# lambdaclass/AES_zero_knowledge_proof_circuit

Hardware: AMD Instinct MI355X
Metric: AES-ECB blocks proven/sec (Marlin), proof verifies (higher is better)
Workload: dtype u32 limbs (253-bit Fr / 377-bit Fq modular integers)

## Files before the change

aes_zero_knowledge_proof_circuit_amd/csrc/capi_kernels.hip:

```cpp
#include "../../include/zkaes.h"
#include <cstring>
#include <string>
#include <vector>
#include "hip_util.hpp"
#include "marlin.hpp"
#include "te28.cuh"
#include <algorithm>
#include <chrono>

typedef unsigned int v4u __attribute__((ext_vector_type(4)));
__global__ void __launch_bounds__(256) k_stream_copy(uint4 *__restrict__ dst_, const uint4 *__restrict__ src_, size_t n16) {
    v4u *dst = (v4u *)dst_; const v4u *src = (const v4u *)src_;
    size_t base = (size_t)blockIdx.x * 1024 + threadIdx.x;
    if (base + 768 < n16) {
        v4u v0 = __builtin_nontemporal_load(src + base), v1 = __builtin_nontemporal_load(src + base + 256);
        v4u v2 = __builtin_nontemporal_load(src + base + 512), v3 = __builtin_nontemporal_load(src + base + 768);
        __builtin_nontemporal_store(v0, dst + base); __builtin_nontemporal_store(v1, dst + base + 256);
        __builtin_nontemporal_store(v2, dst + base + 512); __builtin_nontemporal_store(v3, dst + base + 768);
    } else {
        for (size_t i = base; i < n16; i += 256) dst[i] = src[i];
    }
}


// ... 307 lines not shown
        DevPtr<PF> dv = upload(v, n, s);
        {
            zk::gpu::ThroughputWaits as_between_overlapping_proofs(throughput_variant != 0);
            zk::gpu::batch_inverse(dv, n, post_or_null ? &post : nullptr, s);
            zk::gpu::sync(s);
        }
        zk::gpu::d2h(v, dv, n * sizeof(PF), s);
    });
}
int zkaes_poly_lincomb(const uint8_t *const *polys, const size_t *lens, const uint8_t *scalars, int count, size_t n, uint8_t *out) {
    return guardk([&] {
        const char *who = "zkaes_poly_lincomb";
        need(count >= 1 && count <= 8, who, "1..8 terms"); need(polys && lens && scalars && (out || !n), who, "null argument"); need(n <= POLY_MAX, who, "polynomial too long");
        for (int i = 0; i < count; i++) { need(lens[i] <= n, who, "a term longer than the result"); need(!lens[i] || polys[i], who, "null polynomial"); }
        if (!n) return;
        zk::gpu::require_device();
        StreamGuard s;
        DevPtr<PF> dp[8], dout(n);
        const PF *ptr[8];
        PF sc[8];
        for (int i = 0; i < count; i++) { dp[i] = upload(polys[i], lens[i], s); ptr[i] = dp[i]; sc[i] = load_f(scalars + 32 * i, who); }
        zk::gpu::poly_lincomb_n(dout, n, ptr, lens, sc, count, s);
        zk::gpu::d2h(out, dout, n * sizeof(PF), s);
    });
}
int zkaes_vanishing_quotient_evals(int lg_n, const uint8_t *g, int ncosets, const uint8_t a[32], const uint32_t *idx_or_null, size_t nidx, uint8_t *out) {
    return guardk([&] {
        const char *who = "zkaes_vanishing_quotient_evals";
        need(lg_n >= 0 && lg_n <= 24, who, "lg_n must be in [0, 24]"); need(ncosets >= 1 && ncosets <= 3, who, "1..3 cosets"); need(g && out, who, "null argument");
        const size_t n = (size_t)1 << lg_n;
        for (size_t i = 0; idx_or_null && i < nidx; i++) need(idx_or_null[i] < n, who, "index out of range");
        const PF af = load_f(a, who);
        PF gs[3];
        for (int c = 0; c < ncosets; c++) gs[c] = load_f(g + 32 * c, who);
        zk::gpu::require_device();
        StreamGuard s;
        const PF *elems = zk::gpu::domain_elements<zk::Fr377>(lg_n);
        const size_t scratch_len = zk::gpu::vanishing_quotient_scratch(lg_n, ncosets);
        DevPtr<PF> tabs[3], scratch(scratch_len);
        PF *outs[3] = {nullptr, nullptr, nullptr};
        for (int c = 0; c < ncosets; c++) { tabs[c].alloc(n); outs[c] = tabs[c]; }
        zk::gpu::vanishing_quotient_evals(outs, gs, ncosets, af, elems, (uint32_t)n, lg_n, scratch, scratch_len, s);
        if (!idx_or_null) { for (int c = 0; c < ncosets; c++) zk::gpu::d2h(out + (size_t)c * n * sizeof(PF), tabs[c], n * sizeof(PF), s); return; }
        std::vector<PF> host(n);
        for (int c = 0; c < ncosets; c++) {
            zk::gpu::d2h(host.data(), tabs[c], n * sizeof(PF), s);
            for (size_t i = 0; i < nidx; i++) memcpy(out + ((size_t)c * nidx + i) * sizeof(PF), &host[idx_or_null[i]], sizeof(PF));
        }
    });
}
int zkaes_q1_coset_pointwise(const uint8_t *r, const uint8_t *za, const uint8_t *zb, const uint8_t *t, const uint8_t *z, const uint8_t consts[192], size_t n, uint8_t *out) {
    return guardk([&] {
        const char *who = "zkaes_q1_coset_pointwise";
        need(r && za && zb && t && z && consts && out, who, "null argument"); need(n >= 1 && n <= POLY_MAX, who, "n out of range");
        PF c[6];
        for (int i = 0; i < 6; i++) c[i] = load_f(consts + 32 * i, who);
        zk::gpu::require_device();
        StreamGuard s;
        DevPtr<PF> dr = upload(r, n, s), dza = upload(za, n, s), dzb = upload(zb, n, s), dt = upload(t, n, s), dz = upload(z, n, s), dout(n);
        zk::gpu::q1_coset_pointwise(dout, dr, dza, dzb, dt, dz, c[0], c[1], c[2], c[3], c[4], c[5], n, s);
        zk::gpu::d2h(out, dout, n * sizeof(PF), s);
    });
}
int zkaes_h2_coset(const uint8_t *const arrays[7], const uint8_t consts[224], size_t k, uint8_t *out) {
    return guardk([&] {
        const char *who = "zkaes_h2_coset";
        need(arrays && consts && out, who, "null argument"); need(k >= 1 && k <= POLY_MAX, who, "k out of range");
        for (int i = 0; i < 7; i++) need(arrays[i], who, "null array");
        PF c[7];
        for (int i = 0; i < 7; i++) c[i] = load_f(consts + 32 * i, who);
        zk::gpu::require_device();
        StreamGuard s;
        DevPtr<PF> d[7], dout(k);
        for (int i = 0; i < 7; i++) d[i] = upload(arrays[i], k, s);
        zk::gpu::h2_coset(dout, d[0], d[1], d[2], d[3], d[4], d[5], d[6], c[0], c[1], c[2], c[3], c[4], c[5], c[6], k, s);
        zk::gpu::d2h(out, dout, k * sizeof(PF), s);
    });
}
int zkaes_q1_combine(const uint8_t *q0, const uint8_t *q1, const uint8_t *q3, const uint8_t *mask, const uint8_t inv2[32], const uint8_t inv2zeta[32], size_t n, uint8_t *h1, uint8_t *g1) {
    return guardk([&] {
        const char *who = "zkaes_q1_combine";
        need(q0 && q1 && q3 && mask && h1 && (g1 || n < 2), who, "null argument"); need(n >= 1 && n <= POLY_MAX / 4, who, "n out of range");
        const PF i2 = load_f(inv2, who), i2z = load_f(inv2zeta, who);
        zk::gpu::require_device();
        StreamGuard s;
        DevPtr<PF> d0 = upload(q0, n, s), d1 = upload(q1, n, s), d3 = upload(q3, n, s), dm = upload(mask, 3 * n, s), dh(2 * n), dg(n);
        zk::gpu::q1_combine(dh, dg, d0, d1, d3, dm, i2, i2z, n, s);
        zk::gpu::d2h(h1, dh, 2 * n * sizeof(PF), s);
        zk::gpu::d2h(g1, dg, (n - 1) * sizeof(PF), s);
    });
}
int zkaes_coset_scale(const uint8_t *in, size_t in_len, const uint8_t g[32], size_t n, uint8_t *out) {
    return guardk([&] {
        const char *who = "zkaes_coset_scale";
        need((in || !in_len) && (out || !n), who, "null argument"); need(n <= POLY_MAX && in_len <= POLY_MAX, who, "polynomial too long");
        const PF gf = load_f(g, who);
        if (!n) return;
        zk::gpu::require_device();
        StreamGuard s;
        DevPtr<PF> din = upload(in, in_len, s), dout(n);
        zk::gpu::coset_scale(dout, din, gf, in_len, n, s);
        zk::gpu::d2h(out, dout, n * sizeof(PF), s);
    });
}
int zkaes_z_poly_from_w(const uint8_t *w, size_t wlen, const uint8_t *x_poly, uint32_t m, size_t n, uint8_t *zp) {
    return guardk([&] {
        const char *who = "zkaes_z_poly_from_w";
        need((w || !wlen) && (x_poly || !m) && zp, who, "null argument"); need(n < POLY_MAX && wlen <= POLY_MAX, who, "polynomial too long");
        zk::gpu::require_device();
        StreamGuard s;
        DevPtr<PF> dw = upload(w, wlen, s), dx = upload(x_poly, m, s), dz(n + 1);
        zk::gpu::z_poly_from_w(dz, dw, wlen, dx, m, n, s);
        zk::gpu::d2h(zp, dz, (n + 1) * sizeof(PF), s);
    });
}
int zkaes_ntt_padded(int field_id, const uint8_t *in, size_t in_len, size_t n, int inverse, int coset_c, int lg_big, uint8_t *out) {
    return guardk([&] {
        if (field_id == 381) run_ntt_padded<zk::Fr381>(in, in_len, n, inverse, coset_c, lg_big, out); else if (field_id == 377) run_ntt_padded<zk::Fr377>(in, in_len, n, inverse, coset_c, lg_big, out);
        else throw std::invalid_argument("field_id must be 377 or 381");
    });
}
int zkaes_ntt_scaled(const uint8_t g[32], const uint8_t *in, size_t in_len, size_t n, int inverse, uint8_t *out) {
    return guardk([&] {
        const char *who = "zkaes_ntt_scaled";
        const int lg = exact_log2(n, who);
        need(lg >= 1 && lg <= 28, who, "n must be in [2, 2^28]"); need(in_len <= n, who, "in_len must not exceed n"); need(out && (in || !in_len), who, "null argument");
        const PF gf = load_f(g, who);
        need(!gf.is_zero(), who, "the coset generator must not be zero");
        zk::gpu::require_device();
        StreamGuard s;
        DevPtr<void> table = zk::gpu::coset_power_table<PF>(inverse ? gf.inverse() : gf, n, s);
        DevPtr<PF> a = upload(in, in_len, s), b(n);
        zk::gpu::ntt_scaled<PF>(b, a, in_len, lg, inverse != 0, table, s);
        zk::gpu::d2h(out, b, n * sizeof(PF), s);
    });
}
int zkaes_msm(int curve_id, const uint8_t *bases, const uint8_t *scalars, size_t n, uint8_t *out_xy, int *out_inf) {
    return guardk([&] { if (curve_id == 381) run_msm<zk::Bls381>(bases, scalars, n, out_xy, out_inf, 0, nullptr, nullptr); else if (curve_id == 377) run_msm<zk::Bls377>(bases, scalars, n, out_xy, out_inf, 0, nullptr, nullptr); else throw std::invalid_argument("curve_id must be 377 or 381"); });
}
int zkaes_msm_bench(int curve_id, const uint8_t *bases, const uint8_t *scalars, size_t n, int reps, double *ms_total, double *ms_accumulate) {
    return guardk([&] { if (curve_id == 381) run_msm<zk::Bls381>(bases, scalars, n, nullptr, nullptr, reps, ms_total, ms_accumulate); else run_msm<zk::Bls377>(bases, scalars, n, nullptr, nullptr, reps, ms_total, ms_accumulate); });
}
int zkaes_msm_bench_synth(size_t n, int window_bits, int reps, double *ms_total, double *ms_accumulate, uint8_t *out_xy) {
    return guardk([&] {
        using Fq = zk::Fq377; using Fr = zk::Fr377;
        if (!ms_total || !ms_accumulate || reps < 1 || n == 0 || window_bits > 22) throw std::invalid_argument("zkaes_msm_bench_synth: bad arguments");
        zk::gpu::require_device();
        const size_t nt = window_bits > 0 ? (size_t)zk::gpu::table_windows<zk::Bls377>(window_bits) : 1;
        if ((uint64_t)nt * n >= (1ull << 30)) throw std::invalid_argument("zkaes_msm_bench_synth: n x table copies exceeds the 2^30 base indices of one MSM");
        StreamGuard s;
        DevPtr<zk::Affine<Fq>> tab(nt * n);
        zk::Affine<Fq> g; for (int i = 0; i < 12; i++) { g.x.l[i] = G1_377_X_MONT[i]; g.y.l[i] = G1_377_Y_MONT[i]; }
        Fr beta = Fr::from_u64(0x9e3779b97f4a7c15ull) * Fr::from_u64(0xc2b2ae3d27d4eb4full);
        zk::gpu::fixed_base_powers<zk::Bls377>(tab, g, beta, 1, n, s);
        if (window_bits > 0) zk::gpu::build_window_tables<zk::Bls377>(tab, n, window_bits, s);
        const bool edwards = window_bits != 0;
        DevPtr<zk::Affine28<zk::Fq377P>> tab28;
        DevPtr<zk::Niels28<zk::Fq377P>> tabte;
        if (edwards) { tabte.alloc(nt * n); zk::gpu::convert_bases_te<zk::Bls377>(tabte, tab, nt * n, s); }
        else { tab28.alloc(nt * n); zk::gpu::convert_bases<zk::Bls377>(tab28, tab, nt * n, s); }
        std::vector<Fr> sc(n);
        uint64_t x = 88172645463325252ull;
        for (size_t i = 0; i < n; i++) { for (int k = 0; k < 8; k += 2) { x ^= x << 13; x ^= x >> 7; x ^= x << 17; sc[i].l[k] = (uint32_t)x; sc[i].l[k + 1] = (uint32_t)(x >> 32); } sc[i].l[7] &= 0x0fffffffu; }
        DevPtr<Fr> ds(n);
        zk::gpu::h2d(ds, sc.data(), n * 32, s);
        zk::gpu::sync(s);
        WorkspaceGuard ws;
        auto run = [&]() -> zk::XYZZ<Fq> {
            if (edwards) return window_bits > 0 ? zk::gpu::msm_table<zk::Bls377>(ws, tabte, n, 0, window_bits, ds, n, s) : zk::gpu::msm<zk::Bls377>(ws, tabte.get(), ds.get(), n, s);
            return window_bits > 0 ? zk::gpu::msm_table<zk::Bls377>(ws, tab28, n, 0, window_bits, ds, n, s) : zk::gpu::msm<zk::Bls377>(ws, tab28.get(), ds.get(), n, s);
        };
        give_affine(run().to_affine(), out_xy, nullptr);
        zk::gpu::MsmStats before = zk::gpu::msm_stats(false);
        EventGuard e0, e1;
        zk::gpu::event_record(e0, s);
        for (int i = 0; i < reps; i++) run();
        zk::gpu::event_record(e1, s);
        float ms = zk::gpu::event_elapsed_ms(e0, e1);
        zk::gpu::MsmStats after = zk::gpu::msm_stats(false);
        *ms_total = ms / reps; *ms_accumulate = (after.accumulate_ms - before.accumulate_ms) / reps;
    });
}

int zkaes_stream_copy_bench(size_t bytes, int reps, double *gb_per_s) {
    return guardk([&] {
        if (bytes < 4096 || reps < 1 || !gb_per_s) throw std::invalid_argument("zkaes_stream_copy_bench: bytes >= 4096, reps >= 1");
        zk::gpu::require_device();
        StreamGuard s;
        const size_t n16 = bytes / 16;
        DevPtr<uint4> a(n16), b(n16);
        zk::gpu::dzero(a, n16 * 16, s);
        hipStream_t hs = (hipStream_t)s.h;
        k_stream_copy<<<(unsigned)((n16 + 1023) / 1024), 256, 0, hs>>>(b, a, n16);
        EventGuard e0, e1;
        zk::gpu::event_record(e0, s);
        for (int i = 0; i < reps; i++) k_stream_copy<<<(unsigned)((n16 + 1023) / 1024), 256, 0, hs>>>(i & 1 ? a.get() : b.get(), i & 1 ? b.get() : a.get(), n16);
        zk::gpu::event_record(e1, s);
        float ms = zk::gpu::event_elapsed_ms(e0, e1);
        *gb_per_s = 2.0 * (double)(n16 * 16) * reps / 1e9 / (ms / 1e3);
    });
}
int zkaes_int_rate_bench(double seconds, double out[8]) {
    return guardk([&] {
        if (!out || !(seconds > 0.0) || seconds > 30.0) throw std::invalid_argument("zkaes_int_rate_bench: 0 < seconds <= 30, out != NULL");
        zk::gpu::require_device();
        using P = zk::Fq377P; using G = zk::FpMsm<P>;
        StreamGuard s;
        hipStream_t hs = (hipStream_t)s.h;
        const int GRID_A = 4096, ITERS_A = 300, GRID_B = 8192, ITERS_B = 83;
        const uint32_t NREC = 4096;
        DevPtr<CalStamp> st(GRID_B);
        DevPtr<G> sink_a((size_t)GRID_A * 64);
        DevPtr<zk::AccTE<P>> sink_b((size_t)GRID_B * 64);
        DevPtr<zk::Niels28<P>> tab(NREC);
        k_cal_fill<<<NREC / 256, 256, 0, hs>>>(tab, NREC);
        G ga; for (int k = 0; k < 14; k++) ga.l[k] = 0x0123457u + 977u * k;
        std::vector<double> rate_a, mhz_a, rate_b, mhz_b, cyc_b;
        std::vector<CalStamp> h(GRID_B);
        auto median = [](std::vector<double> &v) { std::sort(v.begin(), v.end()); return v.empty() ? 0.0 : v[v.size() / 2]; };
        auto stamps = [&](int grid, double per_wave_units, double *mhz, double *cyc_per_unit) {
            zk::gpu::d2h(h.data(), st, (size_t)grid * sizeof(CalStamp), s);
            std::vector<double> m(grid), c(grid);
            for (int i = 0; i < grid; i++) { m[i] = (double)h[i].cyc / ((double)h[i].rt / 1e8) / 1e6; c[i] = (double)h[i].cyc / per_wave_units; }
            *mhz = median(m); *cyc_per_unit = median(c);
        };
        EventGuard e0, e1;
        const auto t_begin = std::chrono::steady_clock::now();
        int rounds = 0;
        while (rounds < 3 || std::chrono::duration<double>(std::chrono::steady_clock::now() - t_begin).count() < seconds) {
            double mhz, cyc;
            zk::gpu::event_record(e0, s);
            k_cal_fqmul<<<GRID_A, 64, 0, hs>>>(st, sink_a, ga, ITERS_A);
            zk::gpu::event_record(e1, s);
            stamps(GRID_A, 2.0 * ITERS_A, &mhz, &cyc);
            rate_a.push_back(2.0 * ITERS_A * 64.0 * GRID_A / (zk::gpu::event_elapsed_ms(e0, e1) * 1e-3)); mhz_a.push_back(mhz);
            zk::gpu::event_record(e0, s);
            k_cal_hot_loop<<<GRID_B, 64, 0, hs>>>(st, sink_b, tab, NREC - 1, ITERS_B);
            zk::gpu::event_record(e1, s);
            stamps(GRID_B, (double)ITERS_B, &mhz, &cyc);
            rate_b.push_back((double)ITERS_B * 64.0 * GRID_B / (zk::gpu::event_elapsed_ms(e0, e1) * 1e-3)); mhz_b.push_back(mhz); cyc_b.push_back(cyc);
            rounds++;
        }
        out[0] = median(rate_a); out[1] = median(mhz_a); out[2] = median(rate_b); out[3] = median(mhz_b); out[4] = median(cyc_b); out[5] = (double)rounds; out[6] = 0; out[7] = 0;
    });
}
int zkaes_mem_info(uint64_t *free_bytes, uint64_t *total_bytes) {
    return guardk([&] {
        zk::gpu::require_device();
        size_t f = 0, t = 0;
        HIP_CHECK(hipMemGetInfo(&f, &t));
        if (free_bytes) *free_bytes = f;
        if (total_bytes) *total_bytes = t;
    });
}
}
```

aes_zero_knowledge_proof_circuit_amd/csrc/gpu.hpp:

```cpp
#pragma once
#include <cstddef>
#include <cstdint>
#include <stdexcept>
#include <string>
#include <utility>
#include <vector>
#include "ec.cuh"
#include "te28.cuh"

namespace zk {
namespace gpu {

struct GpuError : std::runtime_error { using std::runtime_error::runtime_error; };
typedef void *stream_t;

int device_count();
void require_device();
int current_device();
void set_device(int ordinal);
void *dmalloc(size_t bytes);
#ifdef ZKAES_MEASURE
int knockin();
#endif
size_t mem_free_bytes();
void dfree(void *p);
void h2d(void *dst, const void *src, size_t bytes, stream_t s);
void d2h(void *dst, const void *src, size_t bytes, stream_t s);
void d2d(void *dst, const void *src, size_t bytes, stream_t s);
void dzero(void *dst, size_t bytes, stream_t s);
void sync(stream_t s);
bool throughput_mode();
struct ThroughputWaits { explicit ThroughputWaits(bool on); ~ThroughputWaits(); ThroughputWaits(const ThroughputWaits &) = delete; ThroughputWaits &operator=(const ThroughputWaits &) = delete; private: bool on_; };
stream_t stream_create();
stream_t stream_create_background();
void stream_destroy(stream_t s);
void *event_create();
void event_record(void *ev, stream_t s);
void stream_wait_event(stream_t s, void *ev);
float event_elapsed_ms(void *start, void *stop);
void event_destroy(void *ev);

void *pinned_alloc(size_t bytes);
void *pinned_device_address(void *host);
void pinned_free(void *host);

template <class T> struct DevElem { static constexpr size_t bytes = sizeof(T); };
template <> struct DevElem<void> { static constexpr size_t bytes = 1; };
template <class T> struct DevPtr {
    T *p = nullptr;
    size_t n = 0;
    DevPtr() = default;
    explicit DevPtr(size_t count) { alloc(count); }
    DevPtr(const DevPtr &) = delete; DevPtr &operator=(const DevPtr &) = delete;
    DevPtr(DevPtr &&o) noexcept : p(o.p), n(o.n) { o.p = nullptr; o.n = 0; }
    DevPtr &operator=(DevPtr &&o) noexcept { if (this != &o) { reset(); p = o.p; n = o.n; o.p = nullptr; o.n = 0; } return *this; }
    ~DevPtr() { dfree(p); }
    void reset() { dfree(p); p = nullptr; n = 0; }
    void alloc(size_t count) { reset(); p = (T *)dmalloc(count * DevElem<T>::bytes); n = count; }
    void grow(size_t count) { if (!p || count > n) alloc(count); }
    T *get() const { return p; }
    operator T *() const { return p; }
};
template <class... T> void grow_together(const size_t (&counts)[sizeof...(T)], DevPtr<T> &...bufs) {
    size_t i = 0;
    if (((bufs.p && counts[i++] <= bufs.n) && ...)) return;
    (bufs.reset(), ...);
    i = 0;
    try { (bufs.alloc(counts[i++]), ...); } catch (...) { (bufs.reset(), ...); throw; }
}
template <class H, H (*Create)(), void (*Destroy)(H)> struct Handle {
    H h = nullptr;
    Handle() : h(Create()) {}
    explicit Handle(H adopt) : h(adopt) {}
    Handle(const Handle &) = delete; Handle &operator=(const Handle &) = delete;
    Handle(Handle &&o) noexcept : h(o.h) { o.h = nullptr; }
    Handle &operator=(Handle &&o) noexcept { if (this != &o) { Destroy(h); h = o.h; o.h = nullptr; } return *this; }
    ~Handle() { Destroy(h); }
    operator H() const { return h; }
};
using StreamGuard = Handle<stream_t, stream_create, stream_destroy>;
using EventGuard = Handle<void *, event_create, event_destroy>;
struct PinnedPtr {
    void *host = nullptr, *dev = nullptr;
    PinnedPtr() = default;
    PinnedPtr(const PinnedPtr &) = delete; PinnedPtr &operator=(const PinnedPtr &) = delete;
    ~PinnedPtr() { pinned_free(host); }
    void alloc(size_t bytes) { pinned_free(host); host = dev = nullptr; host = pinned_alloc(bytes); dev = pinned_device_address(host); }
};

enum : int { OP_MSM_BUCKETS = 0, OP_MSM_SECOND_BASES = 1, OP_MSM_CLASS_SUM = 2 };
struct OpRecord { std::vector<std::pair<uint64_t, int>> ntt , msm ; };
void oplog_begin();
OpRecord oplog_end();
void oplog_ntt(uint64_t n, int count);
void oplog_msm(uint64_t points, int kind);

template <class Fr> void ntt(Fr *dst, const Fr *src, size_t in_len, int lg, bool inverse, stream_t s);
template <class Fr> void ntt_coset(Fr *dst, const Fr *src, size_t in_len, int lg, bool inverse, int coset_c, int lg_big, stream_t s);
template <class Fr> struct NttJob { Fr *dst; const Fr *src; int coset_c; };
template <class Fr> void ntt_batch(const NttJob<Fr> *jobs, int count, size_t in_len, int lg, bool inverse, int lg_big, stream_t s);
template <class Fr> DevPtr<void> coset_power_table(const Fr &g, size_t n, stream_t s);
template <class Fr> void ntt_scaled(Fr *dst, const Fr *src, size_t in_len, int lg, bool inverse, const void *table, stream_t s);
template <class Fr> const Fr *domain_elements(int lg);

struct MsmWorkspace;
MsmWorkspace *msm_workspace_create();
void msm_workspace_destroy(MsmWorkspace *ws);
using WorkspaceGuard = Handle<MsmWorkspace *, msm_workspace_create, msm_workspace_destroy>;
template <class Curve> void convert_bases(Affine28<typename Curve::FqP> *dst, const Affine<typename Curve::Fq> *src, size_t n, stream_t s);
template <class Curve>
XYZZ<typename Curve::Fq> msm(MsmWorkspace *ws, const Affine28<typename Curve::FqP> *bases, const typename Curve::Fr *scalars, size_t n, stream_t s);
template <class Curve>
void msm_prepare(MsmWorkspace *ws, const typename Curve::Fr *scal1, size_t n1, const typename Curve::Fr *scal2, size_t n2, size_t val_off2, stream_t s, int force_c = 0);
template <class Curve>
XYZZ<typename Curve::Fq> msm_finish(MsmWorkspace *ws, const Affine28<typename Curve::FqP> *bases, stream_t s);
template <class Curve> void convert_bases_te(Niels28<typename Curve::FqP> *dst, const Affine<typename Curve::Fq> *src, size_t n, stream_t s);
template <class Curve>
XYZZ<typename Curve::Fq> msm(MsmWorkspace *ws, const Niels28<typename Curve::FqP> *bases, const typename Curve::Fr *scalars, size_t n, stream_t s);
template <class Curve>
XYZZ<typename Curve::Fq> msm_finish(MsmWorkspace *ws, const Niels28<typename Curve::FqP> *bases, stream_t s);
template <class Curve>
void msm_finish2(MsmWorkspace *ws, const Niels28<typename Curve::FqP> *bases, const Niels28<typename Curve::FqP> *bases2, XYZZ<typename Curve::Fq> *out, stream_t s);
template <class Curve>
XYZZ<typename Curve::Fq> msm_table(MsmWorkspace *ws, const Niels28<typename Curve::FqP> *tables, size_t stride, size_t off, int c, const typename Curve::Fr *scalars, size_t n, stream_t s);
template <class Curve>
bool class_sum(MsmWorkspace *ws, const Niels28<typename Curve::FqP> *bases, const int8_t *vals, size_t n, XYZZ<typename Curve::Fq> *out, stream_t s);
template <class Curve> void msm_sharded_plan(size_t n_total, int *window_bits, int *n_windows);
template <class Curve>
void msm_window_sums_device(MsmWorkspace *ws, const Affine28<typename Curve::FqP> *bases, const typename Curve::Fr *scalars, size_t n_local, size_t n_total,
                            XYZZ<typename Curve::Fq> *dev_out, stream_t s);
template <class Curve>
XYZZ<typename Curve::Fq> msm_fold_window_sums_device(const XYZZ<typename Curve::Fq> *dev_in, int world, size_t n_total, stream_t s);
template <class Curve>
void msm_table_sum_device(MsmWorkspace *ws, const Niels28<typename Curve::FqP> *tables, size_t stride, size_t off, int c, const typename Curve::Fr *scalars, size_t n,
                          XYZZ<typename Curve::Fq> *dev_out, stream_t s);
template <class Curve>
XYZZ<typename Curve::Fq> msm_fold_points_device(const XYZZ<typename Curve::Fq> *dev_in, int world, stream_t s);
template <class Curve> int table_windows(int c);
template <class Curve> void build_window_tables(Affine<typename Curve::Fq> *tables, size_t stride, int c, stream_t s);
template <class Curve> void table_next(Affine<typename Curve::Fq> *next, const Affine<typename Curve::Fq> *prev, size_t count, int c, int j, stream_t s);
template <class Curve>
void msm_prepare_table(MsmWorkspace *ws, const typename Curve::Fr *scal1, size_t n1, size_t off1, const typename Curve::Fr *scal2, size_t n2, size_t off2, int c, size_t stride, stream_t s);
template <class Curve>
XYZZ<typename Curve::Fq> msm_table(MsmWorkspace *ws, const Affine28<typename Curve::FqP> *tables, size_t stride, size_t off, int c, const typename Curve::Fr *scalars, size_t n, stream_t s);
template <class Curve>
void fixed_base_powers(Affine<typename Curve::Fq> *out, const Affine<typename Curve::Fq> &base, const typename Curve::Fr &beta, size_t from, size_t count, stream_t s);
template <class Curve>
void fixed_base_scalars(Affine<typename Curve::Fq> *out, const Affine<typename Curve::Fq> &base, const typename Curve::Fr *scalars, size_t count, stream_t s);
template <class Curve>
bool class_sum(MsmWorkspace *ws, const Affine28<typename Curve::FqP> *bases, const int8_t *vals, size_t n, XYZZ<typename Curve::Fq> *out, stream_t s);
struct MsmStats { double accumulate_ms = 0; double total_ms = 0; uint64_t points = 0; uint64_t launches = 0; uint64_t pairs = 0; };
MsmStats msm_stats(bool reset);

}
}

namespace zk {
namespace gpu {
using F = Fr377;

void poly_set_at(F *p, size_t idx, const F &val, stream_t s);
void poly_add_at(F *p, size_t idx, const F &val, stream_t s);
void poly_scale(F *p, const F &sc, size_t n, stream_t s);
void poly_lincomb_n(F *out, size_t n, const F *const *polys, const size_t *lens, const F *scalars, int count, stream_t s);
size_t divide_by_vanishing_scratch(size_t len, size_t m);
void divide_by_vanishing(F *q, F *rem, const F *p, size_t len, size_t m, stream_t s, F *scratch = nullptr, size_t scratch_len = 0);
void divide_by_linear(F *q, const F *p, size_t len, const F &z, F *scratch, size_t scratch_elems, stream_t s);
size_t divide_by_linear_scratch(size_t len);
F poly_eval(const F *p, size_t len, const F &x, F *scratch, stream_t s);
size_t poly_eval_scratch(size_t len);
void poly_eval_multi(const F *const *p, const size_t *len, const F *x, int count, F *out, F *scratch, size_t scratch_elems, stream_t s);
void batch_inverse(F *v, size_t n, const F *post_or_null, stream_t s);
size_t vanishing_quotient_scratch(int lg_n, int ncosets);
void vanishing_quotient_evals(F *const *out, const F *g, int ncosets, const F &a, const F *elems, uint32_t n, int lg_n, F *scratch, size_t scratch_elems, stream_t s);
void f_evals_from_tables(F *out, const F *va, const F *vb, const F *vc, const F &ea, const F &eb, const F &ec, const F *ra, const F *rb, const uint32_t *ri, const uint32_t *ci, size_t k,
                         stream_t s);

void upload_sbox(const uint8_t table[256]);
void aes_trace(uint8_t *trace, size_t trace_stride, const uint8_t *msgs, const uint8_t *keys, uint32_t nproofs, uint32_t nblocks, stream_t s);
void aes_trace_cbc(uint8_t *trace, size_t trace_stride, const uint8_t *msgs, const uint8_t *keys, const uint8_t *ivs, uint32_t nproofs, uint32_t nblocks, stream_t s);
void aes_trace_ctr(uint8_t *trace, size_t trace_stride, const uint8_t *msgs, const uint8_t *keys, const uint8_t *icbs, uint32_t nproofs, uint32_t msg_len, stream_t s);
void aes_trace_gcm(uint8_t *trace, size_t trace_stride, const uint8_t *msgs, const uint8_t *keys, const uint8_t *hdrs, uint32_t nproofs, uint32_t msg_len, uint32_t aad_len, stream_t s);
void ghash_trace(uint8_t *trace, size_t trace_stride, uint32_t nproofs, uint32_t msg_len, uint32_t aad_len, stream_t s);
void witness_expand(uint8_t *z, const uint32_t *desc, uint32_t ncols, const uint8_t *trace, const uint32_t *sbox_in_off, const uint32_t *sbox_tmpl, stream_t s);
void spmv_bits(F *out, int8_t *small_out, size_t rows_out, const uint32_t *rowptr, const uint32_t *col, const int64_t *coeff, size_t rows, const uint8_t *z, stream_t s);
void w_classes(int8_t *out, const uint8_t *z, uint32_t n, uint32_t m, uint32_t num_witness, stream_t s);
void lagrange_scalars(F *lag, F *lag_w, const F *elems, const F &beta, uint32_t n, uint32_t m, stream_t s);
void w_evals(F *out, const uint8_t *z, const F *x_evals, uint32_t n, uint32_t m, uint32_t num_witness, stream_t s);
void bits_to_field(F *out, const uint8_t *z, size_t n, stream_t s);
constexpr uint32_t T_SEG = 32, T_HEAVY_SEGMENTS = 256;
void t_evals(F *out, uint32_t n, F *partial, uint32_t nseg, const uint32_t *col_seg_ptr, const uint32_t *seg_start, const uint32_t *seg_end, const uint32_t *heavy, uint32_t n_heavy,
             const uint32_t *row, const uint8_t *mat, const int64_t *coeff, const F *r_alpha, const F &eta_a, const F &eta_b, const F &eta_c, stream_t s);
uint64_t chacha_field_stream(F *out, size_t count, const uint32_t key[8], int rounds, uint64_t word_pos, void *scratch, size_t scratch_bytes, stream_t s);
void mask_fixup(F *p, size_t n, stream_t s);
void q1_coset_pointwise(F *out, const F *r, const F *za, const F *zb, const F *t, const F *z, const F &ca, const F &cb, const F &cz, const F &eta_a, const F &eta_b, const F &eta_c,
                        size_t n, stream_t s);
void z_evals_h(F *out, const uint8_t *z, uint32_t n, uint32_t m, uint32_t num_witness, stream_t s);
void q1_combine(F *h1, F *g1, const F *q0, const F *q1, const F *q3, const F *mask, const F &inv2, const F &inv2zeta, size_t n, stream_t s);
void coset_scale(F *out, const F *in, const F &g, size_t in_len, size_t n, stream_t s);
void h2_coset(F *out, const F *row, const F *col, const F *va, const F *vb, const F *vc, const F *rc, const F *f, const F &alpha, const F &beta, const F &alpha_beta,
              const F &ea, const F &eb, const F &ec, const F &vinv, size_t k, stream_t s);
void index_evals(F *row, F *col, F *rowcol, F *va, F *vb, F *vc, F *tmp, const uint32_t *ci, const uint32_t *ri, const int64_t *ca, const int64_t *cb, const int64_t *cc, size_t cnt,
                 size_t k, const F *elems, uint32_t n, stream_t s);
void z_poly_from_w(F *zp, const F *w, size_t wlen, const F *x_poly, uint32_t m, size_t n, stream_t s);

}
}
```

aes_zero_knowledge_proof_circuit_amd/csrc/kernels_msm.hip:

```cpp
#include <cstring>
#include <rocprim/device/device_radix_sort.hpp>
#include <rocprim/device/device_scan.hpp>
#include <chrono>
#include <cstdio>
#include <cstdlib>
#include <mutex>
#include <vector>
#include "hip_util.hpp"
#include "te28.cuh"

namespace zk {
namespace gpu {

template <class P> struct WeierLaw { using Params = P; using Base = Affine28<P>; using Acc = Acc28<P>; static constexpr bool edwards = false; };
template <class P> struct EdwardsLaw { using Params = P; using Base = Niels28<P>; using Acc = AccTE<P>; static constexpr bool edwards = true; };

static MsmStats g_stats;
static std::mutex g_stats_mu;
MsmStats msm_stats(bool reset) {
    std::lock_guard<std::mutex> g(g_stats_mu);
    MsmStats s = g_stats;
    if (reset) g_stats = MsmStats();
    return s;
}

constexpr uint32_t VAL_SKIP = 1u << 30, VAL_INDEX = VAL_SKIP - 1;
template <class Fr>
__global__ void k_digits(const Fr *__restrict__ scalars, uint32_t n, uint32_t i_off, uint32_t ntot, uint32_t val_off, int c, int nwin, uint32_t nb,
                         uint32_t *__restrict__ keys, uint32_t *__restrict__ vals) {
    uint32_t i = blockIdx.x * blockDim.x + threadIdx.x;
    if (i >= n) return;
    uint32_t raw[Fr::N + 1];
    scalars[i].to_raw(raw);
    raw[Fr::N] = 0;
    const uint32_t mask = (1u << c) - 1, half = 1u << (c - 1);
    uint32_t carry = 0;
    for (int w = 0; w < nwin; w++) {
        int bit = w * c, limb = bit >> 5, sh = bit & 31;
        uint64_t two = limb <= Fr::N - 1 ? ((uint64_t)raw[limb] | ((uint64_t)raw[limb + 1] << 32)) : 0;
        uint32_t v = ((uint32_t)(two >> sh) & mask) + carry;
        uint32_t neg = 0;
        carry = 0;
        if (v > half) { v = (1u << c) - v; neg = 1u << 31; carry = 1; }
        keys[(size_t)w * ntot + i_off + i] = ((uint32_t)w << (c - 1)) | (v ? v - 1 : 0u);
        vals[(size_t)w * ntot + i_off + i] = v ? ((val_off + i) | neg) : VAL_SKIP;
    }
}

struct TableLayout {
    int nwin, c_hi, n_hi;
    __host__ __device__ int width(int j) const { return j < n_hi ? c_hi : c_hi - 1; }
    __host__ __device__ int offset(int j) const { return j < n_hi ? j * c_hi : n_hi * c_hi + (j - n_hi) * (c_hi - 1); }
};
static TableLayout table_layout(int total_bits, int c) {
    TableLayout L;
    L.nwin = (total_bits + c - 1) / c;
    int base = total_bits / L.nwin, rem = total_bits % L.nwin;
    L.c_hi = base + (rem ? 1 : 0);
    L.n_hi = rem ? rem : L.nwin;
    return L;
}
template <class Fr>
__global__ void k_digits_table(const Fr *__restrict__ scalars, uint32_t n, uint32_t i_off, uint32_t ntot, uint32_t val_off, TableLayout L, uint32_t stride,
                               uint32_t *__restrict__ keys, uint32_t *__restrict__ vals) {
    uint32_t i = blockIdx.x * blockDim.x + threadIdx.x;
    if (i >= n) return;
    uint32_t raw[Fr::N + 1];
    scalars[i].to_raw(raw);
    raw[Fr::N] = 0;
    uint32_t carry = 0;
    for (int w = 0; w < L.nwin; w++) {
        const int c = L.width(w), bit = L.offset(w), limb = bit >> 5, sh = bit & 31;
        const uint32_t mask = (1u << c) - 1, half = 1u << (c - 1);
        uint64_t two = limb <= Fr::N - 1 ? ((uint64_t)raw[limb] | ((uint64_t)raw[limb + 1] << 32)) : 0;
        uint32_t v = ((uint32_t)(two >> sh) & mask) + carry;
        uint32_t neg = 0;
        carry = 0;
        if (v > half) { v = (1u << c) - v; neg = 1u << 31; carry = 1; }
        keys[(size_t)w * ntot + i_off + i] = v ? v - 1 : 0u;
        vals[(size_t)w * ntot + i_off + i] = v ? (((uint32_t)w * stride + val_off + i) | neg) : VAL_SKIP;
    }
}
template <class Fq>
__global__ void __launch_bounds__(64) k_table_next(const Affine<Fq> *__restrict__ prev, Affine<Fq> *__restrict__ next, uint32_t count, int c) {
    constexpr int B = 8;
    uint32_t t = blockIdx.x * blockDim.x + threadIdx.x;
    uint32_t s0 = t * B;
    if (s0 >= count) return;
    uint32_t e = s0 + B < count ? s0 + B : count;
    Fq xs[B], ys[B], zz[B], zzz[B], pre[B];
    Fq acc = Fq::one();
    for (uint32_t i = s0; i < e; i++) {
        XYZZ<Fq> p = XYZZ<Fq>::from_affine(prev[i]);
        for (int k = 0; k < c; k++) p = p.dbl();
        xs[i - s0] = p.x; ys[i - s0] = p.y; zz[i - s0] = p.zz; zzz[i - s0] = p.zzz;
        pre[i - s0] = acc;
        if (!p.zzz.is_zero()) acc = acc * p.zzz;
    }
    acc = acc.inverse();
    for (uint32_t i = e; i-- > s0;) {
        uint32_t q = i - s0;
        if (zzz[q].is_zero()) { next[i] = Affine<Fq>::inf(); continue; }
        Fq zi3 = acc * pre[q];
        acc = acc * zzz[q];
        Fq zi2 = (zi3 * zz[q]).sqr();
        Affine<Fq> a; a.x = xs[q] * zi2; a.y = ys[q] * zi3;
        next[i] = a;
    }
}

__device__ __forceinline__ uint32_t bounds_rank(uint32_t key, int cbits, uint32_t nwin) { return nwin == 1 ? key : (key & ((1u << cbits) - 1)) * nwin + (key >> cbits); }
__device__ __forceinline__ uint32_t bounds_key(uint32_t rank, int cbits, uint32_t nwin) { return nwin == 1 ? rank : ((rank % nwin) << cbits) | (rank / nwin); }
__global__ void k_bounds(const uint32_t *__restrict__ keys, size_t total, int cbits, uint32_t nwin, uint32_t *__restrict__ start, uint32_t *__restrict__ end) {
    size_t i0 = ((size_t)blockIdx.x * blockDim.x + threadIdx.x) * 4;
    if (i0 >= total) return;
    const uint32_t nb = nwin << cbits;
    uint32_t k[6];
    if (i0 + 4 <= total) { uint4 v = *reinterpret_cast<const uint4 *>(keys + i0); k[1] = v.x; k[2] = v.y; k[3] = v.z; k[4] = v.w; }
    else { for (int j = 0; j < 4; j++) k[1 + j] = i0 + j < total ? keys[i0 + j] : 0u; }
    k[0] = i0 ? keys[i0 - 1] : 0u;
    k[5] = i0 + 4 < total ? keys[i0 + 4] : 0u;
#pragma unroll
    for (int j = 0; j < 4; j++) {
        size_t i = i0 + j;
        if (i >= total) break;
        const uint32_t key = k[1 + j];
        if (i == 0 || k[j] != key) {
            const uint32_t r1 = bounds_rank(key, cbits, nwin);
            uint32_t r0 = 0;
            if (i != 0) { end[k[j]] = (uint32_t)i; r0 = bounds_rank(k[j], cbits, nwin) + 1; }
            for (uint32_t r = r0; r < r1; r++) { const uint32_t g = bounds_key(r, cbits, nwin); start[g] = (uint32_t)i; end[g] = (uint32_t)i; }
            start[key] = (uint32_t)i;
        }
        if (i + 1 == total) {
            end[key] = (uint32_t)total;
            for (uint32_t r = bounds_rank(key, cbits, nwin) + 1; r < nb; r++) { const uint32_t g = bounds_key(r, cbits, nwin); start[g] = (uint32_t)total; end[g] = (uint32_t)total; }
        }
    }
}

template <class P>
__global__ void k_convert_bases(const Affine<Fp<P>> *__restrict__ src, Affine28<P> *__restrict__ dst, size_t n) {
    size_t i = (size_t)blockIdx.x * blockDim.x + threadIdx.x;
    if (i < n) dst[i] = Affine28<P>::from_std(src[i]);
}

constexpr uint32_t BUCKET_CAP = 2048, BUCKET_CAP_TABLE = 512;
constexpr uint32_t NO_SLOT = 0xffffffffu;

constexpr int ORD_BINS = 1024, ORD_THREADS = 256, ORD_MAX_BLOCKS = 128;
__device__ __forceinline__ uint32_t order_key(uint32_t sz) { return (ORD_BINS - 1) - (sz > ORD_BINS - 1 ? ORD_BINS - 1 : sz); }
__global__ void __launch_bounds__(ORD_THREADS) k_order_hist(const uint32_t *__restrict__ start, const uint32_t *__restrict__ end, uint32_t nb, uint32_t per_block, uint32_t cap,
                                                             uint32_t *__restrict__ ovf_slot, uint32_t *__restrict__ ovf_bucket, uint32_t *__restrict__ ovf_nseg, uint32_t ovf_cap,
                                                             uint32_t *__restrict__ ctrl, uint32_t *__restrict__ hist) {
    __shared__ uint32_t h[ORD_BINS];
    for (int b = threadIdx.x; b < ORD_BINS; b += ORD_THREADS) h[b] = 0;
    __syncthreads();
    const uint32_t lo = blockIdx.x * per_block, hi = lo + per_block < nb ? lo + per_block : nb;
    for (uint32_t k = lo + threadIdx.x; k < hi; k += ORD_THREADS) {
        const uint32_t sz = end[k] - start[k];
        uint32_t slot = NO_SLOT;
        if (sz > cap) {
            slot = atomicAdd(&ctrl[0], 1u);
            if (slot < ovf_cap) { ovf_bucket[slot] = k; ovf_nseg[slot] = (sz - 1) / cap; } else slot = NO_SLOT;
        }
        ovf_slot[k] = slot;
        atomicAdd(&h[order_key(sz)], 1u);
    }
    __syncthreads();
    for (int b = threadIdx.x; b < ORD_BINS; b += ORD_THREADS) hist[(size_t)blockIdx.x * ORD_BINS + b] = h[b];
}
__global__ void __launch_bounds__(ORD_BINS) k_order_scan(const uint32_t *__restrict__ hist, uint32_t *__restrict__ offs, uint32_t nblk, uint32_t *__restrict__ ctrl,
                                                          const uint32_t *__restrict__ ovf_nseg, uint32_t *__restrict__ ovf_off, uint32_t ovf_cap) {
    __shared__ uint32_t part[ORD_BINS];
    const uint32_t t = threadIdx.x;
    auto block_exclusive = [&](uint32_t v) {
        part[t] = v;
        __syncthreads();
        for (int d = 1; d < ORD_BINS; d <<= 1) {
            uint32_t add = t >= (unsigned)d ? part[t - d] : 0;
            __syncthreads();
            part[t] += add;
            __syncthreads();
        }
        return part[t] - v;
    };
    uint32_t sum = 0;
    uint32_t i0 = 0;
    for (; i0 + 8 <= nblk; i0 += 8) {
        uint32_t c[8];
#pragma unroll
        for (int u = 0; u < 8; u++) c[u] = hist[(size_t)(i0 + u) * ORD_BINS + t];
#pragma unroll
        for (int u = 0; u < 8; u++) sum += c[u];
    }
    for (; i0 < nblk; i0++) sum += hist[(size_t)i0 * ORD_BINS + t];
    uint32_t run = block_exclusive(sum);
    for (i0 = 0; i0 + 8 <= nblk; i0 += 8) {
        uint32_t c[8];
#pragma unroll
        for (int u = 0; u < 8; u++) c[u] = hist[(size_t)(i0 + u) * ORD_BINS + t];
#pragma unroll
        for (int u = 0; u < 8; u++) { offs[(size_t)(i0 + u) * ORD_BINS + t] = run; run += c[u]; }
    }
    for (; i0 < nblk; i0++) { const uint32_t c = hist[(size_t)i0 * ORD_BINS + t]; offs[(size_t)i0 * ORD_BINS + t] = run; run += c; }
    uint32_t n = ctrl[0];
    if (n > ovf_cap) n = ovf_cap;
    uint32_t base = 0;
    for (uint32_t c0 = 0; c0 < n; c0 += ORD_BINS) {
        __syncthreads();
        const uint32_t v = c0 + t < n ? ovf_nseg[c0 + t] : 0;
        const uint32_t ex = block_exclusive(v);
        if (c0 + t < n) ovf_off[c0 + t] = base + ex;
        base += part[ORD_BINS - 1];
    }
    __syncthreads();
    if (t == 0) { ovf_off[n] = base; ctrl[1] = n; ctrl[2] = base; ctrl[0] = 0; }
}
__global__ void __launch_bounds__(ORD_THREADS) k_order_scatter(const uint32_t *__restrict__ start, const uint32_t *__restrict__ end, uint32_t nb, uint32_t per_block,
                                                                const uint32_t *__restrict__ offs, uint32_t *__restrict__ order) {
    __shared__ uint32_t h[ORD_BINS];
    for (int b = threadIdx.x; b < ORD_BINS; b += ORD_THREADS) h[b] = 0;
// ... 494 lines not shown
    const int nrep = bases2 ? 2 : 1, nsets = nsets_one * nrep;
    if (bases2 && !Law::edwards) throw GpuError("msm: two base arrays per prepared state need the Edwards law");
    if (nsets > MAX_WSUMS) throw GpuError("msm: too many windows");
    const size_t nb = (size_t)nsets_one << c;
    ensure_result(S, nb * nrep);
    if constexpr (!Law::edwards) HIP_CHECK(hipMemsetAsync(S.deferred_count, 0, 8, s));
#ifdef ZKAES_MEASURE
    if (knockin() & 8) {
        hipLaunchKernelGGL((k_accumulate<Law>), dim3((unsigned)((nb + 63) / 64)), dim3(64), 0, s, bases, S.sorted_vals, S.start, S.end, S.order, (uint32_t)nb, cap,
                           (A *)S.buckets.p, S.deferred, DEFERRED_CAP, S.deferred_count);
        if constexpr (!Law::edwards) HIP_CHECK(hipMemsetAsync(S.deferred_count, 0, 8, s));
    }
#endif
    uint32_t max_seg = (uint32_t)(pairs / cap + 1);
    for (int rep = 0; rep < nrep; rep++) {
        const typename Law::Base *src = rep ? bases2 : bases;
        HIP_CHECK(hipEventRecord((hipEvent_t)S.ev[2 * rep].h, s));
        hipLaunchKernelGGL((k_accumulate<Law>), dim3((unsigned)((nb + 63) / 64)), dim3(64), 0, s, src, S.sorted_vals, S.start, S.end, S.order, (uint32_t)nb, cap,
                           (A *)S.buckets.p + rep * nb, S.deferred, DEFERRED_CAP, S.deferred_count);
        HIP_LAUNCH_CHECK();
        HIP_CHECK(hipEventRecord((hipEvent_t)S.ev[2 * rep + 1].h, s));
        hipLaunchKernelGGL((k_accumulate_tail<Law>), dim3((max_seg + 63) / 64), dim3(64), 0, s, src, S.sorted_vals, S.start, S.end, S.ctrl, S.ovf_bucket, S.ovf_off, max_seg, cap,
                           (A *)S.ovf_partial.p + rep * S.ovf_bucket.n, (A *)S.buckets.p + rep * nb, S.deferred, DEFERRED_CAP, S.deferred_count);
        HIP_LAUNCH_CHECK();
    }
    if constexpr (!Law::edwards) for (int rep = 0; rep < nrep; rep++) {
        hipLaunchKernelGGL((k_fold_overflow<A>), dim3((max_seg + 63) / 64), dim3(64), 0, s, (A *)S.buckets.p + rep * nb, S.ctrl, S.ovf_bucket, S.ovf_off, max_seg, (const A *)S.ovf_partial.p + rep * S.ovf_bucket.n);
        HIP_LAUNCH_CHECK();
    }
    XYZZ<Fq> *res = (XYZZ<Fq> *)S.h_res.dev;
    uint32_t segs = (1u << c) / RED_L1, groups = (segs + RED_L2 - 1) / RED_L2;
    [[maybe_unused]] int te_lgR = 0, te_lgC = 0;
    [[maybe_unused]] bool te_host_tail = false;
#ifdef ZKAES_MEASURE
    for (int rep = (knockin() & 2) ? 0 : 1; rep < 2; rep++)
#endif
    {
    if constexpr (Law::edwards)
        hipLaunchKernelGGL((k_reduce_l1_pair<A>), dim3((unsigned)((2 * segs * nsets + 63) / 64)), dim3(64), 0, s, (const A *)S.buckets.p, c, nsets, (A *)S.seg_s.p, (A *)S.seg_w.p);
    else
        hipLaunchKernelGGL((k_reduce_l1<A>), dim3((unsigned)((segs * nsets + 63) / 64)), dim3(64), 0, s, (const A *)S.buckets.p, c, nsets, (A *)S.seg_s.p, (A *)S.seg_w.p);
    HIP_LAUNCH_CHECK();
    if constexpr (Law::edwards) {
        const int lgG = c - 3 > 0 ? c - 3 : 0, lgC = (lgG + 1) / 2, lgR = lgG - lgC;
        if (lgC > 8) throw GpuError("msm: more than 2^19 buckets per set");
        const unsigned jobs = 2u * (1u << lgR) + (1u << lgC);
        A *rc = (A *)S.partial.p, *part = rc + (size_t)nsets * jobs;
        hipLaunchKernelGGL((k_reduce_rc<P>), dim3((unsigned)nsets * jobs), dim3(RQ_THREADS), 0, s, (const A *)S.seg_s.p, (const A *)S.seg_w.p, lgR, lgC, rc);
        HIP_LAUNCH_CHECK();
        te_host_tail = !dev_wsum_out && nsets <= 4;
        hipLaunchKernelGGL((k_reduce_terms<P>), dim3((unsigned)(RF_OUT * nsets)), dim3(RT_THREADS), 0, s, (const A *)rc, lgR, lgC, part, res, te_host_tail);
        HIP_LAUNCH_CHECK();
        if (!te_host_tail) {
            hipLaunchKernelGGL((k_reduce_combine<P>), dim3((unsigned)nsets), dim3(64), 0, s, (const A *)part, lgR, lgC, res, dev_wsum_out);
            HIP_LAUNCH_CHECK();
        }
        te_lgR = lgR; te_lgC = lgC;
    } else {
    hipLaunchKernelGGL((k_reduce_l2<A>), dim3(2u * (unsigned)((groups * nsets + 63) / 64)), dim3(64), 0, s, (const A *)S.seg_s.p, (const A *)S.seg_w.p, c, nsets, (A *)S.partial.p);
    HIP_LAUNCH_CHECK();
    const uint32_t parts = 2 * groups;
    if (nsets == 1 && parts > 2048) {
        uint32_t mid = (parts + 255) / 256;
        hipLaunchKernelGGL((k_sum_tree<A>), dim3(mid), dim3(256), 0, s, (const A *)S.partial.p, parts, 256u, (A *)S.seg_s.p, 0u, 0u);
        HIP_LAUNCH_CHECK();
        hipLaunchKernelGGL((k_reduce_window<A>), dim3(1), dim3(256), 0, s, (const A *)S.seg_s.p, mid, res, dev_wsum_out);
    } else {
        hipLaunchKernelGGL((k_reduce_window<A>), dim3((unsigned)nsets), dim3(256), 0, s, (const A *)S.partial.p, parts, res, dev_wsum_out);
    }
    HIP_LAUNCH_CHECK();
    }
    }
    std::vector<XYZZ<Fq>> ws(nsets);
    uint32_t n_deferred = 0;
    sync((stream_t)s);
    if (Law::edwards && te_host_tail) {
        std::vector<XYZZ<Fq>> terms((size_t)nsets * RF_OUT);
        memcpy(terms.data(), S.h_res.host, sizeof(XYZZ<Fq>) * terms.size());
        for (int i = 0; i < nsets; i++) ws[i] = reduce_host_tail<Fq>(terms.data() + (size_t)i * RF_OUT, te_lgR, te_lgC);
    } else memcpy(ws.data(), S.h_res.host, sizeof(XYZZ<Fq>) * nsets);
    if constexpr (!Law::edwards) {
        HIP_CHECK(hipMemcpyAsync(&n_deferred, S.deferred_count, 4, hipMemcpyDeviceToHost, s));
        sync((stream_t)s);
        if (n_deferred > DEFERRED_CAP) throw GpuError("msm: more than 2^20 degenerate additions (repeated base points); refusing to return a wrong sum");
    }
    for (int rep = 0; rep < nrep; rep++) HIP_CHECK(hipEventElapsedTime(acc_ms + rep, (hipEvent_t)S.ev[2 * rep].h, (hipEvent_t)S.ev[2 * rep + 1].h));
    (void)n_points;
    return ws;
}
static void add_stats(const float *acc_ms, int launches, size_t n, size_t pairs, std::chrono::steady_clock::time_point t_begin) {
    std::lock_guard<std::mutex> g(g_stats_mu);
    for (int i = 0; i < launches; i++) g_stats.accumulate_ms += acc_ms[i];
    g_stats.points += n * (size_t)launches;
    g_stats.pairs += pairs * (size_t)launches;
    g_stats.launches += (uint64_t)launches;
    g_stats.total_ms += std::chrono::duration<double, std::milli>(std::chrono::steady_clock::now() - t_begin).count();
}

__global__ void __launch_bounds__(64) k_convert_bases_te(const Affine<Fq377> *__restrict__ src, Niels28<Fq377P> *__restrict__ dst, size_t n, uint32_t *__restrict__ bad) {
    constexpr int B = 8;
    size_t s0 = ((size_t)blockIdx.x * blockDim.x + threadIdx.x) * B;
    if (s0 >= n) return;
    size_t e = s0 + B < n ? s0 + B : n;
    TeMapParts m[B];
    Fq377 pre[B];
    bool skip[B];
    Fq377 acc = Fq377::one();
    for (size_t i = s0; i < e; i++) {
        Affine<Fq377> p = src[i];
        int q = (int)(i - s0);
        skip[q] = p.is_inf();
        if (!skip[q]) {
            m[q] = te_map_parts(p);
            if (m[q].den.is_zero()) { skip[q] = true; atomicOr(bad, 1u); }
        }
        pre[q] = acc;
        if (!skip[q]) acc = acc * m[q].den;
    }
    acc = acc.inverse();
    for (size_t i = e; i-- > s0;) {
        int q = (int)(i - s0);
        if (skip[q]) { dst[i] = niels_identity<Fq377P>(); continue; }
        Fq377 inv = acc * pre[q];
        acc = acc * m[q].den;
        dst[i] = te_niels_finish(m[q], inv);
    }
}
template <class Curve>
void convert_bases_te(Niels28<typename Curve::FqP> *dst, const Affine<typename Curve::Fq> *src, size_t n, stream_t s_) {
    static_assert(Curve::ID == 377, "only BLS12-377's G1 has a twisted Edwards model");
    if (!n) return;
    hipStream_t s = (hipStream_t)s_;
    DevPtr<uint32_t> d_bad(1);
    uint32_t h_bad = 0;
    HIP_CHECK(hipMemsetAsync(d_bad, 0, 4, s));
    size_t lanes = (n + 7) / 8;
    hipLaunchKernelGGL(k_convert_bases_te, dim3((unsigned)((lanes + 63) / 64)), dim3(64), 0, s, src, dst, n, d_bad.get());
    HIP_LAUNCH_CHECK();
    sync((stream_t)s);
    HIP_CHECK(hipMemcpyAsync(&h_bad, d_bad, 4, hipMemcpyDeviceToHost, s));
    sync((stream_t)s);
    if (h_bad) throw GpuError("convert_bases_te: a base point has order 2 or 4 -- the Edwards path needs points of the prime-order subgroup");
}
template void convert_bases_te<Bls377>(Niels28<Fq377P> *, const Affine<Fq377> *, size_t, stream_t);

template <class Curve>
void convert_bases(Affine28<typename Curve::FqP> *dst, const Affine<typename Curve::Fq> *src, size_t n, stream_t s_) {
    if (!n) return;
    hipLaunchKernelGGL((k_convert_bases<typename Curve::FqP>), dim3((unsigned)((n + 255) / 256)), dim3(256), 0, (hipStream_t)s_, src, dst, n);
    HIP_LAUNCH_CHECK();
}

template <class Curve>
void msm_prepare(MsmWorkspace *ws_, const typename Curve::Fr *scal1, size_t n1, const typename Curve::Fr *scal2, size_t n2, size_t val_off2, stream_t s_, int force_c) {
    using Fr = typename Curve::Fr;
    hipStream_t s = (hipStream_t)s_;
    if (!ws_) throw GpuError("msm: null workspace");
    MsmWorkspace &S = *ws_;
    size_t n = n1 + n2;
    S.plan_n = n;
    if (n == 0) return;
    if (n >= (1u << 30) || val_off2 + n2 >= (1u << 30)) throw GpuError("msm: too many points");
    int lg = 0;
    while (((size_t)1 << lg) < n) lg++;
    int c = lg - 2;
    if (c < 7) c = 7;
    if (c > 17) c = 17;
    if (force_c >= 4 && force_c <= 22) c = force_c;
    const int nwin = (Fr::BITS + 1 + c - 1) / c;
    size_t pairs = n * (size_t)nwin;
    if (pairs >= ((size_t)1 << 31)) throw GpuError("msm: n x windows exceeds the 2^31 pairs the sort indexes with int");
    const size_t nb = (size_t)nwin << (c - 1);
    S.plan_c = c; S.plan_nwin = nwin; S.plan_pairs = pairs; S.plan_table = false; S.plan_cap = BUCKET_CAP;
    ensure_scratch(S, pairs, nb, BUCKET_CAP);
    if (n1) { hipLaunchKernelGGL((k_digits<Fr>), dim3((unsigned)((n1 + 255) / 256)), dim3(256), 0, s, scal1, (uint32_t)n1, 0u, (uint32_t)n, 0u, c, nwin, (uint32_t)nb, S.keys_a, S.vals_a); HIP_LAUNCH_CHECK(); }
    if (n2) { hipLaunchKernelGGL((k_digits<Fr>), dim3((unsigned)((n2 + 255) / 256)), dim3(256), 0, s, scal2, (uint32_t)n2, (uint32_t)n1, (uint32_t)n, (uint32_t)val_off2, c, nwin, (uint32_t)nb, S.keys_a, S.vals_a); HIP_LAUNCH_CHECK(); }
    prepare_buckets<typename Curve::FqP>(S, pairs, c - 1, nwin, c - 1, BUCKET_CAP, s);
}
template <class Curve, class Law>
static XYZZ<typename Curve::Fq> msm_finish_impl(MsmWorkspace *ws_, const typename Law::Base *bases, stream_t s_, const typename Law::Base *bases2 = nullptr,
                                                XYZZ<typename Curve::Fq> *out2 = nullptr) {
    using Fq = typename Curve::Fq;
    static_assert(sizeof(XYZZ<Fq>) == 192, "XYZZ layout");
    hipStream_t s = (hipStream_t)s_;
    if (!ws_) throw GpuError("msm: null workspace");
    MsmWorkspace &S = *ws_;
    if (out2) *out2 = XYZZ<Fq>::inf();
    if (S.plan_n == 0) return XYZZ<Fq>::inf();
    auto t_begin = std::chrono::steady_clock::now();
    const int c = S.plan_c, nwin = S.plan_nwin;
    oplog_msm(S.plan_n, OP_MSM_BUCKETS);
    if (bases2) oplog_msm(S.plan_n, OP_MSM_SECOND_BASES);
    float ms[2] = {0, 0};
    if (S.plan_table) {
        std::vector<XYZZ<Fq>> one = run_buckets<Law>(S, bases, S.plan_pairs, c - 1, 1, S.plan_n, S.plan_cap, s, ms, nullptr, bases2);
        add_stats(ms, bases2 ? 2 : 1, S.plan_n, S.plan_pairs, t_begin);
        if (bases2) *out2 = one[1];
        return one[0];
    }
    if (bases2 && 2 * nwin > MAX_WSUMS) {
        *out2 = msm_finish_impl<Curve, Law>(ws_, bases2, s_);
        bases2 = nullptr;
    }
    std::vector<XYZZ<Fq>> ws = run_buckets<Law>(S, bases, S.plan_pairs, c - 1, nwin, S.plan_n, S.plan_cap, s, ms, nullptr, bases2);
    static const bool msm_debug = getenv("ZKAES_MSM_DEBUG") != nullptr;
    if (msm_debug) {
        for (int w = 0; w < nwin; w++) {
            Affine<Fq> a = ws[w].to_affine();
            fprintf(stderr, "window %d inf=%d x0=%08x y0=%08x\n", w, (int)a.is_inf(), a.x.l[0], a.y.l[0]);
        }
    }
    XYZZ<Fq> total[2];
    for (int rep = 0; rep < (bases2 ? 2 : 1); rep++) {
        XYZZ<Fq> t = XYZZ<Fq>::inf();
        for (int w = nwin - 1; w >= 1; w--) {
            t.add(ws[rep * nwin + w]);
            for (int k = 0; k < c; k++) t = t.dbl();
        }
        t.add(ws[rep * nwin]);
        total[rep] = t;
    }
    if (bases2) *out2 = total[1];
    add_stats(ms, bases2 ? 2 : 1, S.plan_n, S.plan_pairs, t_begin);
    return total[0];
}
template <class Curve>
void msm_finish2(MsmWorkspace *ws_, const Niels28<typename Curve::FqP> *bases, const Niels28<typename Curve::FqP> *bases2, XYZZ<typename Curve::Fq> *out, stream_t s_) {
    out[0] = msm_finish_impl<Curve, EdwardsLaw<typename Curve::FqP>>(ws_, bases, s_, bases2, out + 1);
}
template <class Curve>
XYZZ<typename Curve::Fq> msm_finish(MsmWorkspace *ws_, const Affine28<typename Curve::FqP> *bases, stream_t s_) { return msm_finish_impl<Curve, WeierLaw<typename Curve::FqP>>(ws_, bases, s_); }
template <class Curve>
XYZZ<typename Curve::Fq> msm(MsmWorkspace *ws_, const Affine28<typename Curve::FqP> *bases, const typename Curve::Fr *scalars, size_t n, stream_t s_) {
    if (n == 0) return XYZZ<typename Curve::Fq>::inf();
    msm_prepare<Curve>(ws_, scalars, n, nullptr, 0, 0, s_);
    return msm_finish<Curve>(ws_, bases, s_);
}
template <class Curve>
XYZZ<typename Curve::Fq> msm_finish(MsmWorkspace *ws_, const Niels28<typename Curve::FqP> *bases, stream_t s_) { return msm_finish_impl<Curve, EdwardsLaw<typename Curve::FqP>>(ws_, bases, s_); }
template <class Curve>
XYZZ<typename Curve::Fq> msm(MsmWorkspace *ws_, const Niels28<typename Curve::FqP> *bases, const typename Curve::Fr *scalars, size_t n, stream_t s_) {
    if (n == 0) return XYZZ<typename Curve::Fq>::inf();
    msm_prepare<Curve>(ws_, scalars, n, nullptr, 0, 0, s_);
    return msm_finish<Curve>(ws_, bases, s_);
}

template <class Curve>
void msm_sharded_plan(size_t n_total, int *c_out, int *nwin_out) {
    int lg = 0;
    while (((size_t)1 << lg) < n_total) lg++;
    int c = lg - 2;
    if (c < 7) c = 7;
    if (c > 17) c = 17;
    *c_out = c;
    *nwin_out = (Curve::Fr::BITS + 1 + c - 1) / c;
}
template <class Curve>
void msm_window_sums_device(MsmWorkspace *ws_, const Affine28<typename Curve::FqP> *bases, const typename Curve::Fr *scalars, size_t n_local, size_t n_total,
                            XYZZ<typename Curve::Fq> *dev_out, stream_t s_) {
    using Fq = typename Curve::Fq;
    hipStream_t s = (hipStream_t)s_;
    int c, nwin;
    msm_sharded_plan<Curve>(n_total, &c, &nwin);
    if (n_local == 0) {
        HIP_CHECK(hipMemsetAsync(dev_out, 0, sizeof(XYZZ<Fq>) * nwin, s));
        sync((stream_t)s);
        return;
    }
    msm_prepare<Curve>(ws_, scalars, n_local, nullptr, 0, 0, s_, c);
    MsmWorkspace &S = *ws_;
    if (S.plan_nwin != nwin) throw GpuError("msm_window_sums_device: window plan mismatch");
    float ms = 0;
    auto t_begin = std::chrono::steady_clock::now();
    oplog_msm(n_local, OP_MSM_BUCKETS);
    run_buckets<WeierLaw<typename Curve::FqP>>(S, bases, S.plan_pairs, c - 1, nwin, n_local, S.plan_cap, s, &ms, dev_out);
    add_stats(&ms, 1, n_local, S.plan_pairs, t_begin);
}
template <class Fq>
__global__ void k_fold_ranks(const XYZZ<Fq> *__restrict__ in, int world, int nwin, XYZZ<Fq> *__restrict__ out) {
    int w = blockIdx.x * blockDim.x + threadIdx.x;
    if (w >= nwin) return;
    XYZZ<Fq> acc = in[w];
    for (int r = 1; r < world; r++) acc.add(in[(size_t)r * nwin + w]);
    out[w] = acc;
}
template <class Curve>
XYZZ<typename Curve::Fq> msm_fold_window_sums_device(const XYZZ<typename Curve::Fq> *dev_in, int world, size_t n_total, stream_t s_) {
    using Fq = typename Curve::Fq;
    hipStream_t s = (hipStream_t)s_;
    int c, nwin;
    msm_sharded_plan<Curve>(n_total, &c, &nwin);
    DevPtr<XYZZ<Fq>> d_out((size_t)nwin);
    hipLaunchKernelGGL((k_fold_ranks<Fq>), dim3(1), dim3(64), 0, s, dev_in, world, nwin, d_out.get());
    HIP_LAUNCH_CHECK();
    std::vector<XYZZ<Fq>> ws(nwin);
    sync((stream_t)s);
    HIP_CHECK(hipMemcpyAsync(ws.data(), d_out, sizeof(XYZZ<Fq>) * nwin, hipMemcpyDeviceToHost, s));
    sync((stream_t)s);
    XYZZ<Fq> total = XYZZ<Fq>::inf();
    for (int w = nwin - 1; w >= 1; w--) {
        total.add(ws[w]);
        for (int k = 0; k < c; k++) total = total.dbl();
    }
    total.add(ws[0]);
    return total;
}

template <class Curve>
void msm_table_sum_device(MsmWorkspace *ws_, const Niels28<typename Curve::FqP> *tables, size_t stride, size_t off, int c, const typename Curve::Fr *scalars, size_t n,
                          XYZZ<typename Curve::Fq> *dev_out, stream_t s_) {
    using Fq = typename Curve::Fq;
    hipStream_t s = (hipStream_t)s_;
    if (n == 0) {
        HIP_CHECK(hipMemsetAsync(dev_out, 0, sizeof(XYZZ<Fq>), s));
        sync((stream_t)s);
        return;
    }
    msm_prepare_table<Curve>(ws_, scalars, n, off, nullptr, 0, 0, c, stride, s_);
    MsmWorkspace &S = *ws_;
    float ms = 0;
    auto t_begin = std::chrono::steady_clock::now();
    oplog_msm(n, OP_MSM_BUCKETS);
    run_buckets<EdwardsLaw<typename Curve::FqP>>(S, tables, S.plan_pairs, S.plan_c - 1, 1, n, S.plan_cap, s, &ms, dev_out);
    add_stats(&ms, 1, n, S.plan_pairs, t_begin);
}
template <class Curve>
XYZZ<typename Curve::Fq> msm_fold_points_device(const XYZZ<typename Curve::Fq> *dev_in, int world, stream_t s_) {
    using Fq = typename Curve::Fq;
    hipStream_t s = (hipStream_t)s_;
    DevPtr<XYZZ<Fq>> d_out(1);
    hipLaunchKernelGGL((k_fold_ranks<Fq>), dim3(1), dim3(64), 0, s, dev_in, world, 1, d_out.get());
    HIP_LAUNCH_CHECK();
    XYZZ<Fq> r;
    sync((stream_t)s);
    HIP_CHECK(hipMemcpyAsync(&r, d_out, sizeof r, hipMemcpyDeviceToHost, s));
    sync((stream_t)s);
    return r;
}

template <class Curve>
int table_windows(int c) { return table_layout(Curve::Fr::BITS + 1, c).nwin; }

template <class Curve>
void build_window_tables(Affine<typename Curve::Fq> *tables, size_t stride, int c, stream_t s_) {
    using Fq = typename Curve::Fq;
    hipStream_t s = (hipStream_t)s_;
    const TableLayout L = table_layout(Curve::Fr::BITS + 1, c);
    for (int j = 1; j < L.nwin; j++) {
        uint32_t lanes = (uint32_t)((stride + 7) / 8);
        hipLaunchKernelGGL((k_table_next<Fq>), dim3((lanes + 63) / 64), dim3(64), 0, s, tables + (size_t)(j - 1) * stride, tables + (size_t)j * stride, (uint32_t)stride, L.width(j - 1));
        HIP_LAUNCH_CHECK();
    }
    sync((stream_t)s);
}

template <class Curve>
void table_next(Affine<typename Curve::Fq> *next, const Affine<typename Curve::Fq> *prev, size_t count, int c, int j, stream_t s_) {
    const TableLayout L = table_layout(Curve::Fr::BITS + 1, c);
    if (j < 1 || j >= L.nwin) throw GpuError("table_next: window index out of range");
    uint32_t lanes = (uint32_t)((count + 7) / 8);
    hipLaunchKernelGGL((k_table_next<typename Curve::Fq>), dim3((lanes + 63) / 64), dim3(64), 0, (hipStream_t)s_, prev, next, (uint32_t)count, L.width(j - 1));
    HIP_LAUNCH_CHECK();
}

constexpr int PART_FINE_BITS = 9, PART_FINE = 1 << PART_FINE_BITS, PART_WBITS = 4, PART_KEYS = PART_FINE << PART_WBITS;
constexpr int PART_THREADS = 512, PART_SPT = 2, PART_TILE = PART_THREADS * PART_SPT;
constexpr int PART_MAXW = 1 << PART_WBITS;
constexpr int PART_STAGE = PART_TILE * PART_MAXW;
constexpr uint32_t PART_NBIN_MAX = 1024;
constexpr uint32_t PART_GRID = 512, PART_NONE = 0xffffffffu;
constexpr int PART_FINE_THREADS = 1024, PART_FINE_UNROLL = 8;

template <int NW>
__device__ __forceinline__ void part_digits(const uint32_t (&raw)[NW + 1], const TableLayout &L, uint32_t d[PART_MAXW]) {
    uint32_t carry = 0;
#pragma unroll
    for (int w = 0; w < PART_MAXW; w++) {
        d[w] = PART_NONE;
        if (w < L.nwin) {
            const int c = L.width(w), bit = L.offset(w), limb = bit >> 5, sh = bit & 31;
            const uint32_t mask = (1u << c) - 1, half = 1u << (c - 1);
            uint64_t two = limb <= NW - 1 ? ((uint64_t)raw[limb] | ((uint64_t)raw[limb + 1] << 32)) : 0;
            uint32_t v = ((uint32_t)(two >> sh) & mask) + carry;
            uint32_t neg = 0;
            carry = 0;
            if (v > half) { v = (1u << c) - v; neg = 1u << 31; carry = 1; }
            if (v) d[w] = (v - 1) | neg;
        }
    }
}
template <int THREADS>
__device__ __forceinline__ void part_block_scan(uint32_t *cnt, uint32_t len, uint32_t *wave_sums, uint32_t *total_out) {
    const uint32_t per = len / THREADS, t = threadIdx.x, base = t * per;
    uint32_t sum = 0;
    for (uint32_t i = 0; i < per; i++) sum += cnt[base + i];
    uint32_t incl = sum;
    for (int d = 1; d < 64; d <<= 1) { uint32_t v = __shfl_up(incl, d, 64); if ((int)(t & 63) >= d) incl += v; }
    if ((t & 63) == 63) wave_sums[t >> 6] = incl;
    __syncthreads();
    uint32_t run = incl - sum;
    for (uint32_t w = 0; w < (t >> 6); w++) run += wave_sums[w];
    for (uint32_t i = 0; i < per; i++) { const uint32_t c = cnt[base + i]; cnt[base + i] = run; run += c; }
    if (t == THREADS - 1) *total_out = run;
    __syncthreads();
}
template <class Fr>
__global__ void __launch_bounds__(PART_THREADS) k_part_hist(const Fr *__restrict__ s1, uint32_t n1, const Fr *__restrict__ s2, uint32_t n2, TableLayout L, uint32_t nbin,
                                                            uint32_t *__restrict__ canon, uint32_t *__restrict__ hist) {
    __shared__ uint32_t sh[PART_NBIN_MAX];
    for (uint32_t b = threadIdx.x; b < nbin; b += PART_THREADS) sh[b] = 0;
    __syncthreads();
    const uint32_t n = n1 + n2, ntiles = (n + PART_TILE - 1) / PART_TILE, per_wg = (ntiles + gridDim.x - 1) / gridDim.x;
    const uint32_t tile_lo = blockIdx.x * per_wg, tile_hi = tile_lo + per_wg < ntiles ? tile_lo + per_wg : ntiles;
    for (uint32_t tile = tile_lo; tile < tile_hi; tile++)
        for (int q = 0; q < PART_SPT; q++) {
            const uint32_t g = tile * PART_TILE + q * PART_THREADS + threadIdx.x;
            if (g >= n) continue;
            uint32_t d[PART_MAXW], raw[Fr::N + 1];
            (g < n1 ? s1[g] : s2[g - n1]).to_raw(raw);
            raw[Fr::N] = 0;
            part_digits<Fr::N>(raw, L, d);
#pragma unroll
            for (int w = 0; w < PART_MAXW; w++) if (d[w] != PART_NONE) atomicAdd(&sh[(d[w] & 0x7fffffffu) >> PART_FINE_BITS], 1u);
            static_assert(Fr::N == 8, "the canonical scalar is stored as two 16-byte words");
            uint4 *dst = reinterpret_cast<uint4 *>(canon + (size_t)g * Fr::N);
            dst[0] = make_uint4(raw[0], raw[1], raw[2], raw[3]); dst[1] = make_uint4(raw[4], raw[5], raw[6], raw[7]);
        }
    __syncthreads();
    for (uint32_t b = threadIdx.x; b < nbin; b += PART_THREADS) hist[(size_t)b * gridDim.x + blockIdx.x] = sh[b];
    if (blockIdx.x == 0 && threadIdx.x == 0) hist[(size_t)nbin * gridDim.x] = 0;
}
template <int NW>
__global__ void __launch_bounds__(PART_THREADS) k_part_scatter(const uint32_t *__restrict__ canon, uint32_t n, uint32_t n1, TableLayout L, uint32_t off1, uint32_t off2, uint32_t stride,
                                                               uint32_t nbin, const uint32_t *__restrict__ offs, uint32_t *__restrict__ out_val, uint16_t *__restrict__ out_key) {
    __shared__ uint32_t cursor[PART_NBIN_MAX], cnt[PART_NBIN_MAX], fill[PART_NBIN_MAX], st_val[PART_STAGE], st_key[PART_STAGE];
    __shared__ uint32_t wave_sums[PART_THREADS / 64], total;
    for (uint32_t b = threadIdx.x; b < nbin; b += PART_THREADS) cursor[b] = offs[(size_t)b * gridDim.x + blockIdx.x];
    const uint32_t ntiles = (n + PART_TILE - 1) / PART_TILE, per_wg = (ntiles + gridDim.x - 1) / gridDim.x;
    const uint32_t tile_lo = blockIdx.x * per_wg, tile_hi = tile_lo + per_wg < ntiles ? tile_lo + per_wg : ntiles;
    for (uint32_t tile = tile_lo; tile < tile_hi; tile++) {
        for (uint32_t b = threadIdx.x; b < PART_NBIN_MAX; b += PART_THREADS) { cnt[b] = 0; fill[b] = 0; }
        __syncthreads();
        uint32_t d[PART_SPT][PART_MAXW];
#pragma unroll
        for (int q = 0; q < PART_SPT; q++) {
            const uint32_t g = tile * PART_TILE + q * PART_THREADS + threadIdx.x;
            if (g < n) {
                uint32_t raw[NW + 1];
                const uint4 *src = reinterpret_cast<const uint4 *>(canon + (size_t)g * NW);
                const uint4 a = src[0], b = src[1];
                raw[0] = a.x; raw[1] = a.y; raw[2] = a.z; raw[3] = a.w; raw[4] = b.x; raw[5] = b.y; raw[6] = b.z; raw[7] = b.w; raw[NW] = 0;
                part_digits<NW>(raw, L, d[q]);
            } else {
#pragma unroll
                for (int w = 0; w < PART_MAXW; w++) d[q][w] = PART_NONE;
            }
#pragma unroll
            for (int w = 0; w < PART_MAXW; w++) if (d[q][w] != PART_NONE) atomicAdd(&cnt[(d[q][w] & 0x7fffffffu) >> PART_FINE_BITS], 1u);
        }
        __syncthreads();
        part_block_scan<PART_THREADS>(cnt, PART_NBIN_MAX, wave_sums, &total);
#pragma unroll
        for (int q = 0; q < PART_SPT; q++) {
            const uint32_t g = tile * PART_TILE + q * PART_THREADS + threadIdx.x;
            const uint32_t base = g < n1 ? off1 + g : off2 + (g - n1);
#pragma unroll
            for (int w = 0; w < PART_MAXW; w++) {
                if (d[q][w] == PART_NONE) continue;
                const uint32_t bucket = d[q][w] & 0x7fffffffu, bin = bucket >> PART_FINE_BITS;
                const uint32_t e = cnt[bin] + atomicAdd(&fill[bin], 1u);
                st_val[e] = ((uint32_t)w * stride + base) | (d[q][w] & 0x80000000u);
                st_key[e] = bucket | ((uint32_t)w << 20);
            }
        }
        __syncthreads();
        const uint32_t tot = total;
        for (uint32_t e = threadIdx.x; e < tot; e += PART_THREADS) {
            const uint32_t key = st_key[e], bucket = key & 0xfffffu, bin = bucket >> PART_FINE_BITS, dst = cursor[bin] + (e - cnt[bin]);
            out_val[dst] = st_val[e];
            out_key[dst] = (uint16_t)(((bucket & (PART_FINE - 1)) << PART_WBITS) | (key >> 20));
        }
        __syncthreads();
        for (uint32_t b = threadIdx.x; b < nbin; b += PART_THREADS) cursor[b] += fill[b];
        __syncthreads();
    }
}
constexpr uint32_t PART_FINE_STAGE = 30720;
__global__ void __launch_bounds__(PART_FINE_THREADS) k_part_fine(const uint32_t *__restrict__ offs, uint32_t grid_a, const uint32_t *__restrict__ in_val, const uint16_t *__restrict__ in_key,
                                                                 uint32_t *__restrict__ out_val, uint32_t *__restrict__ start, uint32_t *__restrict__ end) {
    __shared__ uint32_t cur[PART_KEYS], stage[PART_FINE_STAGE], wave_sums[PART_FINE_THREADS / 64], total, split_key;
    const uint32_t bin = blockIdx.x, t = threadIdx.x;
    const uint32_t lo = offs[(size_t)bin * grid_a], hi = offs[(size_t)(bin + 1) * grid_a];
    for (uint32_t f = t; f < PART_KEYS; f += PART_FINE_THREADS) cur[f] = 0;
    __syncthreads();
    for (uint32_t e0 = lo + t; e0 < hi; e0 += PART_FINE_THREADS * PART_FINE_UNROLL) {
        uint32_t key[PART_FINE_UNROLL];
#pragma unroll
        for (int u = 0; u < PART_FINE_UNROLL; u++) { const uint32_t e = e0 + u * PART_FINE_THREADS; key[u] = e < hi ? in_key[e] : PART_NONE; }
#pragma unroll
        for (int u = 0; u < PART_FINE_UNROLL; u++) if (key[u] != PART_NONE) atomicAdd(&cur[key[u]], 1u);
    }
    __syncthreads();
    part_block_scan<PART_FINE_THREADS>(cur, PART_KEYS, wave_sums, &total);
    for (uint32_t f = t; f < PART_FINE; f += PART_FINE_THREADS) {
        const uint32_t k = bin * PART_FINE + f;
        start[k] = lo + cur[f << PART_WBITS];
        end[k] = lo + (f + 1 < PART_FINE ? cur[(f + 1) << PART_WBITS] : total);
    }
    __syncthreads();
    const uint32_t tot = total;
    uint32_t k_lo = 0, base = 0;
    while (base < tot) {
        const uint32_t lim = base + PART_FINE_STAGE;
        if (tot <= lim) { if (t == 0) split_key = PART_KEYS; }
        else for (uint32_t f = k_lo + t; f < PART_KEYS; f += PART_FINE_THREADS) {
            const uint32_t e_f = f + 1 < PART_KEYS ? cur[f + 1] : tot;
            if (cur[f] <= lim && e_f > lim) split_key = f;
        }
        __syncthreads();
        uint32_t k_hi = split_key;
        const bool direct = k_hi == k_lo;
        if (direct) k_hi = k_lo + 1;
        const uint32_t stop = k_hi < PART_KEYS ? cur[k_hi] : tot;
        __syncthreads();
        for (uint32_t e0 = lo + t; e0 < hi; e0 += PART_FINE_THREADS * PART_FINE_UNROLL) {
            uint32_t key[PART_FINE_UNROLL], val[PART_FINE_UNROLL];
#pragma unroll
            for (int u = 0; u < PART_FINE_UNROLL; u++) {
                const uint32_t e = e0 + u * PART_FINE_THREADS;
                key[u] = PART_NONE;
                if (e < hi) { key[u] = in_key[e]; val[u] = in_val[e]; }
            }
#pragma unroll
            for (int u = 0; u < PART_FINE_UNROLL; u++) if (key[u] >= k_lo && key[u] < k_hi) {
                const uint32_t pos = atomicAdd(&cur[key[u]], 1u);
                if (direct) out_val[lo + pos] = val[u]; else stage[pos - base] = val[u];
            }
        }
        __syncthreads();
        if (!direct) for (uint32_t i = t; i < stop - base; i += PART_FINE_THREADS) out_val[lo + base + i] = stage[i];
        __syncthreads();
        base = stop; k_lo = k_hi;
    }
}
template <class Fr>
static void partition_buckets(MsmWorkspace &S, const Fr *scal1, size_t n1, size_t off1, const Fr *scal2, size_t n2, size_t off2, const TableLayout &L, size_t stride, uint32_t cap, hipStream_t s) {
    const int B = L.c_hi - 1;
    const uint32_t nbin = 1u << (B - PART_FINE_BITS), G = PART_GRID;
    const size_t n = n1 + n2, nb = (size_t)1 << B, nh = (size_t)nbin * G + 1;
    S.canon.grow(n * Fr::N);
    grow_together({nh, nh}, S.part_hist, S.part_offs);
#ifdef ZKAES_MEASURE
    for (int rep = (knockin() & 1) ? 0 : 1; rep < 2; rep++)
#endif
    {
    hipLaunchKernelGGL((k_part_hist<Fr>), dim3(G), dim3(PART_THREADS), 0, s, scal1, (uint32_t)n1, scal2, (uint32_t)n2, L, nbin, S.canon, S.part_hist);
    HIP_LAUNCH_CHECK();
    size_t tb = 0;
    HIP_CHECK(rocprim::exclusive_scan(nullptr, tb, S.part_hist.p, S.part_offs.p, 0u, nh, rocprim::plus<uint32_t>(), s));
    S.tmp.grow(tb);
    HIP_CHECK(rocprim::exclusive_scan(S.tmp.p, tb, S.part_hist.p, S.part_offs.p, 0u, nh, rocprim::plus<uint32_t>(), s));
    hipLaunchKernelGGL((k_part_scatter<Fr::N>), dim3(G), dim3(PART_THREADS), 0, s, (const uint32_t *)S.canon, (uint32_t)n, (uint32_t)n1, L, (uint32_t)off1, (uint32_t)off2, (uint32_t)stride, nbin,
                       (const uint32_t *)S.part_offs, S.vals_a, (uint16_t *)S.keys_a.p);
    HIP_LAUNCH_CHECK();
    hipLaunchKernelGGL(k_part_fine, dim3(nbin), dim3(PART_FINE_THREADS), 0, s, (const uint32_t *)S.part_offs, G, (const uint32_t *)S.vals_a, (const uint16_t *)S.keys_a.p, S.vals_b, S.start, S.end);
    HIP_LAUNCH_CHECK();
    }
    S.sorted_vals = S.vals_b; S.sorted_keys = nullptr;
    order_buckets(S, nb, cap, s);
}

template <class Curve>
void msm_prepare_table(MsmWorkspace *ws_, const typename Curve::Fr *scal1, size_t n1, size_t off1, const typename Curve::Fr *scal2, size_t n2, size_t off2, int c, size_t stride,
                       stream_t s_) {
    using Fr = typename Curve::Fr;
    hipStream_t s = (hipStream_t)s_;
    if (!ws_) throw GpuError("msm: null workspace");
    MsmWorkspace &S = *ws_;
    size_t n = n1 + n2;
    S.plan_n = n;
    if (n == 0) return;
    if (c < 4 || c > 24) throw GpuError("msm_table: window bits out of range");
    const TableLayout L = table_layout(Fr::BITS + 1, c);
    const int nwin = L.nwin;
    if (off1 + n1 > stride || off2 + n2 > stride) throw GpuError("msm_table: range exceeds the table");
    if ((uint64_t)nwin * stride >= (1ull << 30) || (uint64_t)n * nwin >= (1ull << 31)) throw GpuError("msm_table: index range too large");
    size_t pairs = n * (size_t)nwin;
    const size_t nb = (size_t)1 << (L.c_hi - 1);
    uint32_t cap = BUCKET_CAP_TABLE;
    while ((uint64_t)cap < 2 * (pairs / nb) + 64) cap <<= 1;
    S.plan_c = L.c_hi; S.plan_nwin = nwin; S.plan_pairs = pairs; S.plan_table = true; S.plan_cap = cap;
    ensure_scratch(S, pairs, nb, cap);
    const int B = L.c_hi - 1;
    if (B > PART_FINE_BITS && (1u << (B - PART_FINE_BITS)) <= PART_NBIN_MAX && nwin <= PART_MAXW && pairs >= ((size_t)1 << 16)) {
        partition_buckets<Fr>(S, scal1, n1, off1, scal2, n2, off2, L, stride, cap, s);
        return;
    }
    if (n1) { hipLaunchKernelGGL((k_digits_table<Fr>), dim3((unsigned)((n1 + 255) / 256)), dim3(256), 0, s, scal1, (uint32_t)n1, 0u, (uint32_t)n, (uint32_t)off1, L, (uint32_t)stride, S.keys_a, S.vals_a); HIP_LAUNCH_CHECK(); }
    if (n2) { hipLaunchKernelGGL((k_digits_table<Fr>), dim3((unsigned)((n2 + 255) / 256)), dim3(256), 0, s, scal2, (uint32_t)n2, (uint32_t)n1, (uint32_t)n, (uint32_t)off2, L, (uint32_t)stride, S.keys_a, S.vals_a); HIP_LAUNCH_CHECK(); }
    prepare_buckets<typename Curve::FqP>(S, pairs, L.c_hi - 1, 1, L.c_hi - 1, cap, s);
}
template <class Curve>
XYZZ<typename Curve::Fq> msm_table(MsmWorkspace *ws_, const Affine28<typename Curve::FqP> *tables, size_t stride, size_t off, int c, const typename Curve::Fr *scalars, size_t n, stream_t s_) {
    if (n == 0) return XYZZ<typename Curve::Fq>::inf();
    msm_prepare_table<Curve>(ws_, scalars, n, off, nullptr, 0, 0, c, stride, s_);
    return msm_finish<Curve>(ws_, tables, s_);
}
template <class Curve>
XYZZ<typename Curve::Fq> msm_table(MsmWorkspace *ws_, const Niels28<typename Curve::FqP> *tables, size_t stride, size_t off, int c, const typename Curve::Fr *scalars, size_t n, stream_t s_) {
    if (n == 0) return XYZZ<typename Curve::Fq>::inf();
    msm_prepare_table<Curve>(ws_, scalars, n, off, nullptr, 0, 0, c, stride, s_);
    return msm_finish<Curve>(ws_, tables, s_);
}

template <class Fr>
__global__ void k_power_scalars(Fr beta, uint64_t from, uint32_t count, Fr *__restrict__ out) {
    uint32_t i = blockIdx.x * blockDim.x + threadIdx.x;
    if (i >= count) return;
    out[i] = beta.pow_u64(from + i);
}
template <class Fq, class Fr>
__global__ void __launch_bounds__(64) k_fixed_base(const Affine<Fq> *__restrict__ table, const Fr *__restrict__ scalars, uint32_t count, Affine<Fq> *__restrict__ out) {
    uint32_t i = blockIdx.x * blockDim.x + threadIdx.x;
    if (i >= count) return;
    uint32_t raw[Fr::N];
    scalars[i].to_raw(raw);
    XYZZ<Fq> acc = XYZZ<Fq>::inf();
    for (int w = 0; w < Fr::N * 4; w++) {
        uint32_t d = (raw[w >> 2] >> ((w & 3) * 8)) & 0xff;
        if (d) acc.madd(table[w * 255 + d - 1]);
    }
    out[i] = acc.to_affine();
}

namespace {
template <class Curve>
DevPtr<Affine<typename Curve::Fq>> upload_fixed_base_table(const Affine<typename Curve::Fq> &base, hipStream_t s) {
    using Fq = typename Curve::Fq;
    const int NW = Curve::Fr::N * 4;
    std::vector<Affine<Fq>> table((size_t)NW * 255);
    XYZZ<Fq> wb = XYZZ<Fq>::from_affine(base);
    for (int w = 0; w < NW; w++) {
        XYZZ<Fq> acc = wb;
        for (int d = 1; d <= 255; d++) { table[(size_t)w * 255 + d - 1] = acc.to_affine(); acc.add(wb); }
        for (int k = 0; k < 8; k++) wb = wb.dbl();
    }
    DevPtr<Affine<Fq>> d_table(table.size());
    HIP_CHECK(hipMemcpyAsync(d_table, table.data(), table.size() * sizeof(Affine<Fq>), hipMemcpyHostToDevice, s));
    sync((stream_t)s);
    return d_table;
}
}

template <class Curve>
void fixed_base_powers(Affine<typename Curve::Fq> *out, const Affine<typename Curve::Fq> &base, const typename Curve::Fr &beta, size_t from, size_t count, stream_t s_) {
    using Fq = typename Curve::Fq;
    using Fr = typename Curve::Fr;
    hipStream_t s = (hipStream_t)s_;
    if (!count) return;
    DevPtr<Affine<Fq>> d_table = upload_fixed_base_table<Curve>(base, s);
    const size_t CH = 1 << 20;
    DevPtr<Fr> d_sc(CH);
    for (size_t off = 0; off < count; off += CH) {
        uint32_t m = (uint32_t)((count - off) < CH ? (count - off) : CH);
        hipLaunchKernelGGL((k_power_scalars<Fr>), dim3((m + 255) / 256), dim3(256), 0, s, beta, (uint64_t)(from + off), m, d_sc.get());
        HIP_LAUNCH_CHECK();
        hipLaunchKernelGGL((k_fixed_base<Fq, Fr>), dim3((m + 63) / 64), dim3(64), 0, s, (const Affine<Fq> *)d_table.get(), (const Fr *)d_sc.get(), m, out + off);
        HIP_LAUNCH_CHECK();
    }
    sync((stream_t)s);
}
template <class Curve>
void fixed_base_scalars(Affine<typename Curve::Fq> *out, const Affine<typename Curve::Fq> &base, const typename Curve::Fr *scalars, size_t count, stream_t s_) {
    using Fq = typename Curve::Fq;
    using Fr = typename Curve::Fr;
    hipStream_t s = (hipStream_t)s_;
    if (!count) return;
    DevPtr<Affine<Fq>> d_table = upload_fixed_base_table<Curve>(base, s);
    const size_t CH = 1 << 20;
    for (size_t off = 0; off < count; off += CH) {
        uint32_t m = (uint32_t)((count - off) < CH ? (count - off) : CH);
        hipLaunchKernelGGL((k_fixed_base<Fq, Fr>), dim3((m + 63) / 64), dim3(64), 0, s, (const Affine<Fq> *)d_table.get(), scalars + off, m, out + off);
        HIP_LAUNCH_CHECK();
    }
    sync((stream_t)s);
}

constexpr int CLS_CHUNK = 16;
template <class Law>
__global__ void __launch_bounds__(64, 2) k_class_partials(const typename Law::Base *__restrict__ bases, const int8_t *__restrict__ vals, uint32_t n, typename Law::Acc *__restrict__ part1,
                                                           typename Law::Acc *__restrict__ part2, uint32_t *__restrict__ flags) {
    using P = typename Law::Params;
    using G = FpMsm<P>;
    uint32_t t = blockIdx.x * blockDim.x + threadIdx.x;
    uint32_t s0 = t * CLS_CHUNK;
    if (s0 >= n) return;
    uint32_t e = s0 + CLS_CHUNK < n ? s0 + CLS_CHUNK : n;
    if constexpr (Law::edwards) {
#pragma unroll 1
        for (int cls = 1; cls <= 2; cls++) {
            AccTE<P> a = te_identity<P>();
            for (uint32_t i = s0; i < e; i++) {
                const int v = vals[i], m = v < 0 ? -v : v;
                if (m != cls) { if (m > 2 && cls == 1) atomicOr(flags, 2u); continue; }
                Niels28<P> p = bases[i];
                if (v < 0) p = niels_neg<P>(p);
                te_madd<P>(a, p);
            }
            (cls == 1 ? part1 : part2)[t] = a;
        }
        return;
    } else
    {
    Acc28<P> a1, a2;
    bool inf1 = true, inf2 = true;
    for (uint32_t i = s0; i < e; i++) {
        int v = vals[i];
        if (v == 0) continue;
        Affine28<P> p = bases[i];
        if (p.is_inf()) continue;
        if (v < 0) { p.y = G::zero().template sub<2>(p.y); v = -v; }
        if (v == 1) {
            if (inf1) { a1.x = p.x; a1.y = p.y; a1.zz = G::k_one(); a1.zzz = a1.zz; inf1 = false; }
            else if (!madd28(a1, p)) atomicOr(flags, 1u);
        } else if (v == 2) {
            if (inf2) { a2.x = p.x; a2.y = p.y; a2.zz = G::k_one(); a2.zzz = a2.zz; inf2 = false; }
            else if (!madd28(a2, p)) atomicOr(flags, 1u);
        } else atomicOr(flags, 2u);
    }
    part1[t] = inf1 ? inf28<P>() : a1;
    part2[t] = inf2 ? inf28<P>() : a2;
    }
}
template <class A>
__global__ void __launch_bounds__(256) k_sum_tree(const A *__restrict__ in, uint32_t total, uint32_t per, A *__restrict__ out, uint32_t in_stride, uint32_t out_stride) {
    __shared__ A sh[256];
    in += (size_t)blockIdx.y * in_stride; out += (size_t)blockIdx.y * out_stride;
    uint32_t b = blockIdx.x, t = threadIdx.x;
    uint32_t lo = b * per, hi = lo + per < total ? lo + per : total;
    A acc = PtOps<A>::identity();
    for (uint32_t i = lo + t; i < hi; i += 256) PtOps<A>::add(acc, in[i]);
    sh[t] = acc;
    __syncthreads();
    int width = 256;
    while (width > 2 && (uint32_t)(width >> 1) >= hi - lo) width >>= 1;
    for (int s = width >> 1; s > 0; s >>= 1) {
        if ((int)t < s) { A a = sh[t]; PtOps<A>::add(a, sh[t + s]); sh[t] = a; }
        __syncthreads();
    }
    if (t == 0) out[b] = sh[0];
}
template <class P>
__global__ void __launch_bounds__(RQ_THREADS) k_quad_sum(const AccTE<P> *__restrict__ in, uint32_t total, uint32_t per, AccTE<P> *__restrict__ out, uint32_t in_stride, uint32_t out_stride) {
    __shared__ uint32_t pt[RQ_QUADS * PT_WORDS];
    in += (size_t)blockIdx.y * in_stride; out += (size_t)blockIdx.y * out_stride;
    const uint32_t b = blockIdx.x, quad = threadIdx.x >> 2;
    const int q = threadIdx.x & 3;
    const uint32_t lo = b * per, hi = lo + per < total ? lo + per : total;
    FpMsm<P> acc = te_identity_quad<P>(q);
    for (uint32_t i = lo + quad; i < hi; i += RQ_QUADS) acc = te_add_quad<P>(acc, quad_load<P>(reinterpret_cast<const uint32_t *>(in + i), q), q);
    quad_store<P>(pt + quad * PT_WORDS, q, acc);
    __syncthreads();
    quad_tree_sum<P>(pt, RQ_QUADS, quad, q);
    if (quad == 0) quad_store<P>(reinterpret_cast<uint32_t *>(out + b), q, quad_load<P>(pt, q));
}
template <class A>
__global__ void __launch_bounds__(64) k_class_result(const A *__restrict__ in, uint32_t *__restrict__ flags, XYZZ<Fp<typename PtOps<A>::Params>> *__restrict__ out) {
    uint32_t i = threadIdx.x;
    if (i < 2) out[i] = PtOps<A>::to_std(in[i]);
    if (i == 2) { *reinterpret_cast<uint32_t *>(out + 2) = *flags; *flags = 0; }
}

template <class Curve, class Law>
static bool class_sum_impl(MsmWorkspace *ws_, const typename Law::Base *bases, const int8_t *vals, size_t n, XYZZ<typename Curve::Fq> *out, stream_t s_) {
    using A = typename Law::Acc;
    using Fq = typename Curve::Fq;
    hipStream_t s = (hipStream_t)s_;
    *out = XYZZ<Fq>::inf();
    if (n == 0) return true;
    if (!ws_) throw GpuError("class_sum: null workspace");
    MsmWorkspace &S = *ws_;
    uint32_t chunks = (uint32_t)((n + CLS_CHUNK - 1) / CLS_CHUNK), mid = (chunks + 255) / 256;
    size_t need_buckets = 2 * (size_t)chunks + 2 * mid + 8;
    ensure_scratch(S, 1, need_buckets, 0);
    A *p1 = (A *)S.buckets.p, *p2 = p1 + chunks, *m1 = p2 + chunks, *m2 = m1 + mid, *fin = m2 + mid;
    hipLaunchKernelGGL((k_class_partials<Law>), dim3((chunks + 63) / 64), dim3(64), 0, s, bases, vals, (uint32_t)n, p1, p2, S.ctrl + 3);
    HIP_LAUNCH_CHECK();
    (void)p2; (void)m2;
    if constexpr (Law::edwards) {
        hipLaunchKernelGGL((k_quad_sum<typename Law::Params>), dim3(mid, 2), dim3(RQ_THREADS), 0, s, (const A *)p1, chunks, 256u, m1, chunks, mid); HIP_LAUNCH_CHECK();
        hipLaunchKernelGGL((k_quad_sum<typename Law::Params>), dim3(1, 2), dim3(RQ_THREADS), 0, s, (const A *)m1, mid, mid, fin, mid, 1u); HIP_LAUNCH_CHECK();
    } else {
        hipLaunchKernelGGL((k_sum_tree<A>), dim3(mid, 2), dim3(256), 0, s, (const A *)p1, chunks, 256u, m1, chunks, mid); HIP_LAUNCH_CHECK();
        hipLaunchKernelGGL((k_sum_tree<A>), dim3(1, 2), dim3(256), 0, s, (const A *)m1, mid, mid, fin, mid, 1u); HIP_LAUNCH_CHECK();
    }
    hipLaunchKernelGGL((k_class_result<A>), dim3(1), dim3(64), 0, s, (const A *)fin, S.ctrl + 3, (XYZZ<Fq> *)S.h_res.dev); HIP_LAUNCH_CHECK();
    XYZZ<Fq> r[2];
    uint32_t flags = 0;
    sync((stream_t)s);
    memcpy(r, S.h_res.host, sizeof r);
    memcpy(&flags, (const char *)S.h_res.host + sizeof r, 4);
    if (flags) return false;
    oplog_msm(n, OP_MSM_CLASS_SUM);
    XYZZ<Fq> t = r[1].dbl();
    t.add(r[0]);
    *out = t;
    return true;
}
template <class Curve>
bool class_sum(MsmWorkspace *ws_, const Affine28<typename Curve::FqP> *bases, const int8_t *vals, size_t n, XYZZ<typename Curve::Fq> *out, stream_t s_) {
    return class_sum_impl<Curve, WeierLaw<typename Curve::FqP>>(ws_, bases, vals, n, out, s_);
}
template <class Curve>
bool class_sum(MsmWorkspace *ws_, const Niels28<typename Curve::FqP> *bases, const int8_t *vals, size_t n, XYZZ<typename Curve::Fq> *out, stream_t s_) {
    return class_sum_impl<Curve, EdwardsLaw<typename Curve::FqP>>(ws_, bases, vals, n, out, s_);
}
template XYZZ<Fq377> msm_finish<Bls377>(MsmWorkspace *, const Niels28<Fq377P> *, stream_t);
template void msm_finish2<Bls377>(MsmWorkspace *, const Niels28<Fq377P> *, const Niels28<Fq377P> *, XYZZ<Fq377> *, stream_t);
template XYZZ<Fq377> msm<Bls377>(MsmWorkspace *, const Niels28<Fq377P> *, const Fr377 *, size_t, stream_t);
template XYZZ<Fq377> msm_table<Bls377>(MsmWorkspace *, const Niels28<Fq377P> *, size_t, size_t, int, const Fr377 *, size_t, stream_t);
template bool class_sum<Bls377>(MsmWorkspace *, const Niels28<Fq377P> *, const int8_t *, size_t, XYZZ<Fq377> *, stream_t);

template void msm_table_sum_device<Bls377>(MsmWorkspace *, const Niels28<Fq377P> *, size_t, size_t, int, const Fr377 *, size_t, XYZZ<Fq377> *, stream_t);
template XYZZ<Fq377> msm_fold_points_device<Bls377>(const XYZZ<Fq377> *, int, stream_t);
template XYZZ<Fq381> msm_fold_points_device<Bls381>(const XYZZ<Fq381> *, int, stream_t);
template void msm_sharded_plan<Bls377>(size_t, int *, int *);
template void msm_sharded_plan<Bls381>(size_t, int *, int *);
template void msm_window_sums_device<Bls377>(MsmWorkspace *, const Affine28<Fq377P> *, const Fr377 *, size_t, size_t, XYZZ<Fq377> *, stream_t);
template void msm_window_sums_device<Bls381>(MsmWorkspace *, const Affine28<Fq381P> *, const Fr381 *, size_t, size_t, XYZZ<Fq381> *, stream_t);
template XYZZ<Fq377> msm_fold_window_sums_device<Bls377>(const XYZZ<Fq377> *, int, size_t, stream_t);
template XYZZ<Fq381> msm_fold_window_sums_device<Bls381>(const XYZZ<Fq381> *, int, size_t, stream_t);
template void msm_prepare_table<Bls377>(MsmWorkspace *, const Fr377 *, size_t, size_t, const Fr377 *, size_t, size_t, int, size_t, stream_t);
template void msm_prepare_table<Bls381>(MsmWorkspace *, const Fr381 *, size_t, size_t, const Fr381 *, size_t, size_t, int, size_t, stream_t);
template XYZZ<Fq377> msm_table<Bls377>(MsmWorkspace *, const Affine28<Fq377P> *, size_t, size_t, int, const Fr377 *, size_t, stream_t);
template XYZZ<Fq381> msm_table<Bls381>(MsmWorkspace *, const Affine28<Fq381P> *, size_t, size_t, int, const Fr381 *, size_t, stream_t);
template void convert_bases<Bls377>(Affine28<Fq377P> *, const Affine<Fq377> *, size_t, stream_t);
template void convert_bases<Bls381>(Affine28<Fq381P> *, const Affine<Fq381> *, size_t, stream_t);
template void build_window_tables<Bls377>(Affine<Fq377> *, size_t, int, stream_t);
template void table_next<Bls377>(Affine<Fq377> *, const Affine<Fq377> *, size_t, int, int, stream_t);
template void table_next<Bls381>(Affine<Fq381> *, const Affine<Fq381> *, size_t, int, int, stream_t);
template void build_window_tables<Bls381>(Affine<Fq381> *, size_t, int, stream_t);
template int table_windows<Bls377>(int);
template int table_windows<Bls381>(int);
template void msm_prepare<Bls377>(MsmWorkspace *, const Fr377 *, size_t, const Fr377 *, size_t, size_t, stream_t, int);
template void msm_prepare<Bls381>(MsmWorkspace *, const Fr381 *, size_t, const Fr381 *, size_t, size_t, stream_t, int);
template XYZZ<Fq377> msm_finish<Bls377>(MsmWorkspace *, const Affine28<Fq377P> *, stream_t);
template XYZZ<Fq381> msm_finish<Bls381>(MsmWorkspace *, const Affine28<Fq381P> *, stream_t);
template XYZZ<Fq377> msm<Bls377>(MsmWorkspace *, const Affine28<Fq377P> *, const Fr377 *, size_t, stream_t);
template XYZZ<Fq381> msm<Bls381>(MsmWorkspace *, const Affine28<Fq381P> *, const Fr381 *, size_t, stream_t);
template void fixed_base_scalars<Bls377>(Affine<Fq377> *, const Affine<Fq377> &, const Fr377 *, size_t, stream_t);
template bool class_sum<Bls377>(MsmWorkspace *, const Affine28<Fq377P> *, const int8_t *, size_t, XYZZ<Fq377> *, stream_t);
template void fixed_base_powers<Bls377>(Affine<Fq377> *, const Affine<Fq377> &, const Fr377 &, size_t, size_t, stream_t);
template void fixed_base_powers<Bls381>(Affine<Fq381> *, const Affine<Fq381> &, const Fr381 &, size_t, size_t, stream_t);

}
}
```

aes_zero_knowledge_proof_circuit_amd/csrc/marlin.cpp:

```cpp
#include "marlin.hpp"
#include "../../include/zkaes.h"
#include <algorithm>
#include <cstdio>
#include <chrono>
#include <cstdlib>
#include <cstring>
#include <atomic>
#include <map>
#include <mutex>
#include <future>
#include <deque>
#include <condition_variable>
#include <thread>
#include <functional>
#include <stdexcept>
#include <cerrno>
#include <sys/random.h>
#include "gpu.hpp"
#include "trace_layout.h"
#include "transcript.hpp"
#include "marlin_host.hpp"

namespace zk {
namespace {

using namespace hostx;
using gpu::F;
using Clock = std::chrono::steady_clock;
double ms_since(Clock::time_point t0) { return std::chrono::duration<double, std::milli>(Clock::now() - t0).count(); }

}

using SrsPoint = Niels28<Fq377P>;
static void srs_convert(SrsPoint *dst, const G1A *src, size_t n, gpu::stream_t s) { gpu::convert_bases_te<Bls377>(dst, src, n, s); }

struct DeviceScope {
    int prev = -1;
    explicit DeviceScope(int device) noexcept { try { prev = gpu::current_device(); if (prev != device) gpu::set_device(device); else prev = -1; } catch (...) { prev = -1; } }
    ~DeviceScope() { if (prev >= 0) { try { gpu::set_device(prev); } catch (...) {} } }
};
using gpu::DevPtr;
struct KzgRand { bool hiding = false; Fr b[3]; };

struct UniversalSrs {
    int device = 0;
    size_t max_degree = 0, stride = 0;
    int table_c = 20;
    size_t n_tab = 1;
    Fr beta;
    G1A g, gamma_g;
    pairing::G2Affine h, beta_h;
    G1A gamma_powers[3];
    FixedBaseHost gamma_tab[3];
    DevPtr<SrsPoint> d_points;
    double build_s = 0;
    bool tables() const { return n_tab > 1; }
    uint64_t bytes() const { return (uint64_t)n_tab * stride * sizeof(SrsPoint); }
    ~UniversalSrs() { DeviceScope on(device); d_points.reset(); }
};
struct LagrangeSrs {
    int device = 0;
    size_t n = 0, m = 0;
    DevPtr<SrsPoint> d_lag_h, d_lag_w;
    std::vector<G1A> lag_pj;
    G1A lag_vh, lag_vw;
    FixedBaseHost lag_vh_tab, lag_vw_tab;
    ~LagrangeSrs() { DeviceScope on(device); d_lag_h.reset(); d_lag_w.reset(); }
};
namespace {
std::mutex g_srs_mu;
std::map<std::pair<int, size_t>, std::weak_ptr<UniversalSrs>> g_srs_cache[2];
std::map<std::tuple<int, size_t, size_t>, std::weak_ptr<LagrangeSrs>> g_lag_cache;
bool g_srs_hold = false;
std::vector<std::shared_ptr<UniversalSrs>> g_srs_held;
std::vector<std::shared_ptr<LagrangeSrs>> g_lag_held;
std::atomic<size_t> g_default_contexts{0};
}
size_t default_contexts() {
    size_t v = g_default_contexts.load();
    if (v) return v;
    v = ZKAES_DEFAULT_CONTEXTS;
    if (const char *e = getenv("ZKAES_CONTEXTS")) v = (size_t)std::min(64, std::max(1, atoi(e)));
    g_default_contexts.store(v);
    return v;
}
void set_default_contexts(size_t n) { g_default_contexts.store(n > 64 ? 64 : n); }
static std::shared_ptr<UniversalSrs> acquire_srs(size_t max_degree, bool want_tables, size_t reserve_bytes, gpu::stream_t stream) {
    std::lock_guard<std::mutex> lock(g_srs_mu);
    const int device = gpu::current_device();
    const auto key = std::make_pair(device, max_degree);
    if (auto sp = g_srs_cache[1][key].lock()) return sp;
    if (!want_tables) if (auto sp = g_srs_cache[0][key].lock()) return sp;
    auto t0 = Clock::now();
    std::shared_ptr<UniversalSrs> S(new UniversalSrs());
    S->device = device; S->max_degree = max_degree; S->stride = max_degree + 1;
    kzg_setup_points(S->beta, S->g, S->gamma_g, S->h);
    S->table_c = 20;
    size_t n_tab = want_tables ? (size_t)gpu::table_windows<Bls377>(S->table_c) : 1;
    if (n_tab > 1 && (uint64_t)n_tab * S->stride >= (1ull << 30)) n_tab = 1;
    if (n_tab > 1) {
        const size_t need = n_tab * S->stride * sizeof(SrsPoint) + 2 * S->stride * sizeof(G1A) + reserve_bytes + ((size_t)2 << 30);
        if (gpu::mem_free_bytes() < need) n_tab = 1;
    }
    if (n_tab == 1) if (auto sp = g_srs_cache[0][key].lock()) return sp;
    S->n_tab = n_tab;
    {
        DevPtr<G1A> stage[2];
        stage[0].alloc(S->stride);
        if (n_tab > 1) stage[1].alloc(S->stride);
        gpu::fixed_base_powers<Bls377>(stage[0], S->g, S->beta, 0, S->stride, stream);
        S->d_points.alloc(n_tab * S->stride);
        srs_convert(S->d_points, stage[0], S->stride, stream);
        for (size_t j = 1; j < n_tab; j++) {
            gpu::table_next<Bls377>(stage[j & 1], stage[(j - 1) & 1], S->stride, S->table_c, (int)j, stream);
            srs_convert(S->d_points + j * S->stride, stage[j & 1], S->stride, stream);
        }
        gpu::sync(stream);
    }
    { Fr bp = Fr::one(); for (int i = 0; i < 3; i++) { S->gamma_powers[i] = mul_affine(S->gamma_g, bp); bp = bp * S->beta; S->gamma_tab[i].build(S->gamma_powers[i]); } }
    { uint32_t raw[8]; S->beta.to_raw(raw); S->beta_h = pairing::g2_mul_raw(S->h, raw, 8); }
    S->build_s = ms_since(t0) / 1e3;
    g_srs_cache[n_tab > 1 ? 1 : 0][key] = S;
    if (g_srs_hold) g_srs_held.push_back(S);
    return S;
}
static std::shared_ptr<LagrangeSrs> acquire_lagrange(const UniversalSrs &U, size_t n, int lg_n, size_t m, int lg_m, gpu::stream_t stream) {
    std::lock_guard<std::mutex> lock(g_srs_mu);
    const int device = gpu::current_device();
    const auto key = std::make_tuple(device, n, m);
    if (auto sp = g_lag_cache[key].lock()) return sp;
    std::shared_ptr<LagrangeSrs> Lg(new LagrangeSrs());
    Lg->device = device; Lg->n = n; Lg->m = m;
    DevPtr<F> d_lag(n), d_lagw(n);
    gpu::lagrange_scalars(d_lag, d_lagw, gpu::domain_elements<F>(lg_n), U.beta, (uint32_t)n, (uint32_t)m, stream);
    DevPtr<G1A> pts(n);
    auto to28 = [&](const F *sc, DevPtr<SrsPoint> &dst) {
        gpu::fixed_base_scalars<Bls377>(pts, U.g, sc, n, stream);
        dst.alloc(n);
        srs_convert(dst, pts, n, stream);
        gpu::sync(stream);
    };
    to28(d_lag, Lg->d_lag_h);
    to28(d_lagw, Lg->d_lag_w);
    Fr vh = eval_vanishing(n, U.beta), vx = eval_vanishing(m, U.beta), vx_inv = vx.inverse();
    Fr cm = vx * Fr::from_u64(m).inverse(), cn = vh * Fr::from_u64(n).inverse();
    std::vector<Fr> pj(m), den(m);
    Fr gx = domain_gen(lg_m), e = Fr::one();
    for (size_t j = 0; j < m; j++) { den[j] = U.beta - e; pj[j] = e; e = e * gx; }
    { std::vector<Fr> pre(m); Fr acc = Fr::one(); for (size_t j = 0; j < m; j++) { pre[j] = acc; acc = acc * den[j]; } Fr inv = acc.inverse(); for (size_t j = m; j-- > 0;) { Fr d = den[j]; den[j] = inv * pre[j]; inv = inv * d; } }
    for (size_t j = 0; j < m; j++) pj[j] = pj[j] * den[j] * (cm - cn) * vx_inv;
    DevPtr<F> d_pj(m);
    gpu::h2d(d_pj, pj.data(), m * sizeof(F), stream);
    gpu::fixed_base_scalars<Bls377>(pts, U.g, d_pj, m, stream);
    Lg->lag_pj.resize(m);
    gpu::d2h(Lg->lag_pj.data(), pts, m * sizeof(G1A), stream);
    Lg->lag_vh = mul_affine(U.g, vh);
    Lg->lag_vw = mul_affine(U.g, vh * vx_inv);
    Lg->lag_vh_tab.build(Lg->lag_vh); Lg->lag_vw_tab.build(Lg->lag_vw);
    g_lag_cache[key] = Lg;
    if (g_srs_hold) g_lag_held.push_back(Lg);
    return Lg;
}
void srs_hold(bool hold) {
    std::vector<std::shared_ptr<UniversalSrs>> drop_u;
    std::vector<std::shared_ptr<LagrangeSrs>> drop_l;
    {
        std::lock_guard<std::mutex> lock(g_srs_mu);
        g_srs_hold = hold;
        if (hold) {
            for (auto &cache : g_srs_cache) for (auto &kv : cache) if (auto sp = kv.second.lock()) if (std::find(g_srs_held.begin(), g_srs_held.end(), sp) == g_srs_held.end()) g_srs_held.push_back(sp);
            for (auto &kv : g_lag_cache) if (auto sp = kv.second.lock()) if (std::find(g_lag_held.begin(), g_lag_held.end(), sp) == g_lag_held.end()) g_lag_held.push_back(sp);
        } else { drop_u.swap(g_srs_held); drop_l.swap(g_lag_held); }
    }
}


struct LaneWorker {
    std::thread th;
    std::mutex mu;
    std::condition_variable cv;
    std::deque<std::function<void()>> q;
    bool stop = false;
    LaneWorker() { th = std::thread([this] { run(); }); }
    ~LaneWorker() { { std::lock_guard<std::mutex> g(mu); stop = true; } cv.notify_one(); if (th.joinable()) th.join(); }
    void run() {
        for (;;) {
            std::function<void()> t;
            { std::unique_lock<std::mutex> lk(mu); cv.wait(lk, [&] { return stop || !q.empty(); }); if (q.empty()) return; t = std::move(q.front()); q.pop_front(); }
            t();
        }
    }
    void submit(std::function<void()> f) { { std::lock_guard<std::mutex> g(mu); q.push_back(std::move(f)); } cv.notify_one(); }
};
struct ProverContext {
    std::mutex in_use;
    gpu::StreamGuard stream;
    gpu::WorkspaceGuard msm_ws;
    DevPtr<uint8_t> d_trace, d_z, d_msg, d_key, d_iv;
    DevPtr<void> d_rng;
    DevPtr<int8_t> d_cls[3];
    DevPtr<F> za_ev, zb_ev, x_poly, x_tmp, x_evals, tmp_n, ra_ev, ra_poly, zpoly, t_partial;
    DevPtr<F> poly[9];
    size_t poly_len[9] = {0};
    DevPtr<F> e[5], f_poly, acc, wit, wit2, scratch;
    ProverTimings timings;
    DevPtr<F> acc_b, wit_b, wit2_b, scratch_b;
    DevPtr<F> scratch_c; gpu::EventGuard ev_aux{nullptr};
    bool throughput = false;
    static constexpr int N_LANES = 5;
    struct Lane {
        gpu::stream_t stream = nullptr; gpu::MsmWorkspace *ws = nullptr;
        gpu::StreamGuard own_stream{nullptr}; gpu::WorkspaceGuard own_ws{nullptr};
        gpu::EventGuard ready{nullptr};
        std::unique_ptr<LaneWorker> worker;
    };
    Lane lane[N_LANES];
    ProverContext() { lane[0].stream = stream; lane[0].ws = msm_ws; }
    void ensure_lanes() {
        for (int i = 1; i < N_LANES; i++) if (!lane[i].worker) {
            Lane &L = lane[i];
            L.own_stream = gpu::StreamGuard(i == 3 ? gpu::stream_create_background() : gpu::stream_create()); L.own_ws = gpu::WorkspaceGuard(); L.ready = gpu::EventGuard();
            L.stream = L.own_stream; L.ws = L.own_ws;
            L.worker.reset(new LaneWorker());
        }
    }
};

class ProvingKeyImpl {
  public:
    VerifyingKey vk;
    Circuit circuit;
    size_t message_len = 0;
    size_t n = 0, k = 0, m = 0;
    int lg_n = 0, lg_k = 0, lg_m = 0;
    size_t max_degree = 0, supported_degree = 0, lowest_shift = 0, bounds[2] = {0, 0};
    int device = 0;
    std::shared_ptr<UniversalSrs> srs;
    std::shared_ptr<LagrangeSrs> lag;
    SrsPoint *d_powers = nullptr, *d_shifted = nullptr;
    size_t srs_stride = 0;
#ifndef ZKAES_TABLE_MIN_N
#define ZKAES_TABLE_MIN_N 100000
#endif
    size_t table_min_n = ZKAES_TABLE_MIN_N;
    bool use_lagrange = true;
    int table_c = 20;
    bool use_tables = false;
    std::atomic<size_t> n_contexts{0};
    double setup_srs_s = 0, setup_total_s = 0;
    DevPtr<uint32_t> d_desc, d_sbox_in, d_sbox_tmpl;
    DevPtr<uint32_t> d_a_rowptr, d_a_col, d_b_rowptr, d_b_col;
    DevPtr<int64_t> d_a_coeff, d_b_coeff;
    DevPtr<uint32_t> d_t_colptr, d_t_seg_start, d_t_seg_end, d_t_row; DevPtr<uint8_t> d_t_mat; DevPtr<int64_t> d_t_coeff;
    uint32_t t_nseg = 0, t_nheavy = 0;
    DevPtr<uint32_t> d_t_heavy;
    DevPtr<uint32_t> d_ix_ci, d_ix_ri;
    DevPtr<F> ix_ev[6], ix_co[6], ix_cs[6];
    Fr coset_g, coset_g_inv, coset_vk_inv;
    DevPtr<void> coset_tab, coset_tab_inv;
    ProverTimings last_timings;

    std::mutex ctx_mu;
    std::vector<std::unique_ptr<ProverContext>> ctxs;

    ProverContext &context(size_t i) {
        gpu::set_device(device);
        std::lock_guard<std::mutex> g(ctx_mu);
        while (ctxs.size() <= i) {
            std::unique_ptr<ProverContext> c(new ProverContext());
            alloc_workspace(*c);
            ctxs.push_back(std::move(c));
        }
        return *ctxs[i];
    }
    void alloc_workspace(ProverContext &cx) {
        const Circuit &c = circuit;
        size_t n4 = next_pow2(3 * n + 1);
        cx.d_trace.alloc(c.trace_bytes + 64); cx.d_z.alloc(c.num_variables() + 64);
        cx.d_msg.alloc(std::max<size_t>(message_len, 16)); cx.d_key.alloc(16); cx.d_iv.alloc(std::max<size_t>(16, 12 + c.aad_bytes));
        for (auto &p : cx.d_cls) p.alloc(n + 64);
        { size_t ncand = (size_t)(3.0 * n / 0.58 * 1.02) + 8192; cx.d_rng.alloc((ncand * 8 / 16 + 2) * 64 + ncand * 8 + (4u << 20)); }
        cx.za_ev.alloc(n); cx.zb_ev.alloc(n); cx.x_poly.alloc(m); cx.x_tmp.alloc(m); cx.x_evals.alloc(n); cx.tmp_n.alloc(n + 1); cx.ra_ev.alloc(n); cx.ra_poly.alloc(n);
        cx.zpoly.alloc(n + 1); cx.t_partial.alloc(t_nseg + 1);
        size_t caps[9] = {n + 1, n + 1, n + 1, 3 * n, n, n, 3 * n, k, k + 1};
        for (int i = 0; i < 9; i++) cx.poly[i].alloc(caps[i]);
        size_t big = std::max(n4, k);
        for (auto &b : cx.e) b.alloc(big);
        cx.f_poly.alloc(k);
        cx.acc.alloc(std::max(3 * n, k) + 1); cx.wit.alloc(std::max(3 * n, k) + 1); cx.wit2.alloc(std::max(n, k) + 1); cx.scratch.alloc(std::max(8 + 3 * gpu::poly_eval_scratch(n + 1) + gpu::poly_eval_scratch(k), gpu::divide_by_linear_scratch(std::max(3 * n, k) + 1)));
    }

    template <class T> static DevPtr<T> upload(const std::vector<T> &v, gpu::stream_t s) {
        DevPtr<T> d(v.size());
        gpu::h2d(d, v.data(), v.size() * sizeof(T), s);
        return d;
    }

    bool table_ok(const ProverContext &, size_t len) const { return use_tables && len >= table_min_n; }
    using Lane = ProverContext::Lane;
    XYZZ<Fq377> msm_powers(ProverContext &cx, Lane &ln, bool shifted, size_t off, const F *scalars, size_t len) {
        if (len == 0) return XYZZ<Fq377>::inf();
        size_t avail = shifted ? (bounds[1] + 1) : (supported_degree + 1);
        if (off + len > avail) throw std::runtime_error("KZG10: polynomial degree exceeds the committer key");
        if (table_ok(cx, len)) return gpu::msm_table<Bls377>(ln.ws, d_powers, srs_stride, (shifted ? lowest_shift : 0) + off, table_c, scalars, len, ln.stream);
        return gpu::msm<Bls377>(ln.ws, (shifted ? d_shifted : d_powers) + off, scalars, len, ln.stream);
    }
    struct Labeled { int idx; long bound; bool hiding; KzgRand rand, shifted_rand; Commitment comm; };
    static void draw_rand(Labeled &lp, ChaChaRng &zk) {
        auto draw = [&](KzgRand &r) { r.hiding = lp.hiding; for (auto &x : r.b) x = Fr::zero(); if (lp.hiding) for (int i = 0; i < 3; i++) r.b[i] = zk.rand_field<Fr>(); };
        draw(lp.rand);
        if (lp.bound >= 0) draw(lp.shifted_rand);
    }
    void hide(XYZZ<Fq377> &c, const KzgRand &rnd) const { if (rnd.hiding) for (int i = 0; i < 3; i++) c.add(srs->gamma_tab[i].mul(rnd.b[i])); }
    bool lagrange_commit(ProverContext &cx, Lane &ln, int which, const std::vector<uint8_t> &inst, const Fr &rho, const KzgRand &rnd, G1A &out) {
        XYZZ<Fq377> c;
        if (!gpu::class_sum<Bls377>(ln.ws, which == 0 ? lag->d_lag_w : lag->d_lag_h, cx.d_cls[which], n, &c, ln.stream)) return false;
        if (which == 0) for (size_t j = 0; j < m; j++) if (inst[j]) c.madd(lag->lag_pj[j].neg());
        c.add((which == 0 ? lag->lag_vw_tab : lag->lag_vh_tab).mul(rho));
        hide(c, rnd);
        out = c.to_affine();
        return true;
    }
    void mpc_commit(ProverContext &cx, Lane &ln, Labeled &lp) {
        const F *coeffs = cx.poly[lp.idx].p;
        size_t len = cx.poly_len[lp.idx];
        lp.comm.has_shifted = false;
        const bool bounded = lp.bound >= 0;
        const size_t off = bounded ? (max_degree - (size_t)lp.bound) - lowest_shift : 0;
        if (len > supported_degree + 1 || (bounded && off + len > bounds[1] + 1)) throw std::runtime_error("KZG10: polynomial degree exceeds the committer key");
        if (len) {
            if (table_ok(cx, len)) gpu::msm_prepare_table<Bls377>(ln.ws, coeffs, len, 0, nullptr, 0, 0, table_c, srs_stride, ln.stream);
            else gpu::msm_prepare<Bls377>(ln.ws, coeffs, len, nullptr, 0, 0, ln.stream);
        }
        XYZZ<Fq377> c12[2] = {XYZZ<Fq377>::inf(), XYZZ<Fq377>::inf()}, h12[2] = {XYZZ<Fq377>::inf(), XYZZ<Fq377>::inf()};
        hide(h12[0], lp.rand);
        if (bounded) hide(h12[1], lp.shifted_rand);
        if (len) {
            if (bounded) gpu::msm_finish2<Bls377>(ln.ws, d_powers, d_shifted + off, c12, ln.stream);
            else c12[0] = gpu::msm_finish<Bls377>(ln.ws, d_powers, ln.stream);
        }
        c12[0].add(h12[0]);
        lp.comm.comm = c12[0].to_affine();
        if (bounded) { c12[1].add(h12[1]); lp.comm.shifted = c12[1].to_affine(); lp.comm.has_shifted = true; }
    }
    void msm_opening_prepare(ProverContext &cx, Lane &ln, const F *wit, size_t wlen, const F *swit, size_t slen, size_t shift_off) {
        if (wlen > supported_degree + 1 || shift_off + slen > bounds[1] + 1) throw std::runtime_error("KZG10: polynomial degree exceeds the committer key");
        if (table_ok(cx, wlen + slen)) gpu::msm_prepare_table<Bls377>(ln.ws, wit, wlen, 0, swit, slen, lowest_shift + shift_off, table_c, srs_stride, ln.stream);
        else gpu::msm_prepare<Bls377>(ln.ws, wit, wlen, swit, slen, lowest_shift + shift_off, ln.stream);
    }
    XYZZ<Fq377> msm_opening_finish(Lane &ln) { return gpu::msm_finish<Bls377>(ln.ws, d_powers, ln.stream); }
    bool use_lanes = true;
    struct RoundJobs {
        ProvingKeyImpl &K; ProverContext &cx;
        const bool async;
        struct Slot { std::string err; std::function<void(Lane &)> fn; std::promise<void> done; std::future<void> fut; bool queued = false; };
        std::vector<std::unique_ptr<Slot>> slots;
        RoundJobs(ProvingKeyImpl &k, ProverContext &c) : K(k), cx(c), async(!c.throughput && k.use_lanes) { if (async) cx.ensure_lanes(); }
        void start(int lane_i, std::function<void(Lane &)> fn, bool gate) {
            std::unique_ptr<Slot> sl(new Slot());
            sl->fn = std::move(fn);
            Slot *p = sl.get();
            slots.push_back(std::move(sl));
            if (!async) return;
            if (lane_i < 1 || lane_i >= ProverContext::N_LANES) throw std::logic_error("RoundJobs: bad lane");
            Lane &ln = cx.lane[lane_i];
            if (gate) { gpu::event_record(ln.ready, cx.stream); gpu::stream_wait_event(ln.stream, ln.ready); }
            const int dev = K.device;
            p->fut = p->done.get_future(); p->queued = true;
            ln.worker->submit([p, &ln, dev] {
                try { gpu::set_device(dev); p->fn(ln); } catch (const std::exception &e) { p->err = e.what(); if (p->err.empty()) p->err = "error"; } catch (...) { p->err = "error"; }
                p->done.set_value();
            });
        }
        void join() {
            std::string first;
            for (auto &sl : slots) {
                if (async) { if (sl->queued) { sl->fut.wait(); sl->queued = false; } }
                else { try { sl->fn(cx.lane[0]); } catch (const std::exception &e) { sl->err = e.what(); if (sl->err.empty()) sl->err = "error"; } }
                if (first.empty() && !sl->err.empty()) first = sl->err;
            }
            slots.clear();
            if (!first.empty()) throw std::runtime_error(first);
        }
        void wait_all() noexcept { for (auto &sl : slots) if (sl->queued) sl->fut.wait(); }
        ~RoundJobs() { wait_all(); }
    };

    struct ProofRun {
        ProverContext &cx;
        const uint8_t *host_trace, *msg; size_t len; const uint8_t *key, *iv;
        Clock::time_point t_all, t0;
        ChaChaRng zk;
        FiatShamirRng fs;
        Labeled r1[4], r2[3], r3[2];
        Fr rhos[3];
        std::vector<uint8_t> inst;
        bool declined[3] = {false, false, false};
        Fr alpha, eta_a, eta_b, eta_c, vh_alpha, beta, vh_beta, ea_vv, eb_vv, ec_vv, alpha_beta, gamma;
        Proof pf;
        bool early_evals = false;
        std::atomic<bool> g2_quotient_queued{false};
        RoundJobs jobs;
        ProofRun(ProvingKeyImpl &K, ProverContext &c, const uint8_t *trace, const uint8_t *msg_, size_t len_, const uint8_t *key_, const uint8_t *iv_, const uint8_t *zk_seed)
            : cx(c), host_trace(trace), msg(msg_), len(len_), key(key_), iv(iv_), t_all(Clock::now()), t0(t_all), zk(zk_seed ? zk_seed : ark_test_rng_seed(), 12),
              r1{{0, -1, true}, {1, -1, true}, {2, -1, true}, {3, -1, false}}, r2{{4, -1, false}, {5, (long)(K.n - 2), true}, {6, -1, false}},
              r3{{7, (long)(K.k - 2), false}, {8, -1, false}}, jobs(K, c) {}
    };
    Fr sample_outside_h(FiatShamirRng &fs) const;

    void setup(int kind, size_t message_len, const SrsLiterals &lits, unsigned flags, size_t aad_len);
    Proof prove(ProverContext &cx, const uint8_t *trace_or_null, const uint8_t *msg, size_t len, const uint8_t *key, const uint8_t *zk_seed, bool throughput = false, const uint8_t *iv = nullptr);
    void launch_trace(ProverContext &cx, const uint8_t *msg, size_t len, const uint8_t *key, const uint8_t *iv);
    void prove_round1(ProofRun &R);
    void prove_round2(ProofRun &R);
    void prove_round3(ProofRun &R);
    void prove_open(ProofRun &R);
};

void ProvingKeyImpl::setup(int kind, size_t message_len_, const SrsLiterals &lits, unsigned flags, size_t aad_len) {
    auto t_setup = Clock::now();
    gpu::require_device();
    device = gpu::current_device();
    message_len = message_len_;
    std::unique_ptr<ProverContext> cx0(new ProverContext());
    gpu::stream_t stream = cx0->stream;
    circuit = compile_circuit(kind, message_len, aad_len);
    const Circuit &c = circuit;
    size_t rows = c.num_constraints;
    std::vector<uint32_t> j_ci, j_ri;
    std::vector<int64_t> j_a, j_b, j_c;
    m = c.num_instance; n = next_pow2(c.num_constraints);
    for (size_t r = 0; r < rows; r++) {
        uint32_t ia = c.A.rowptr[r], ib = c.B.rowptr[r], ic = c.C.rowptr[r];
        const uint32_t ea = c.A.rowptr[r + 1], eb = c.B.rowptr[r + 1], ec = c.C.rowptr[r + 1];
        for (;;) {
            uint32_t best = 0xffffffffu;
            if (ia < ea) best = std::min(best, c.A.col[ia]);
            if (ib < eb) best = std::min(best, c.B.col[ib]);
            if (ic < ec) best = std::min(best, c.C.col[ic]);
            if (best == 0xffffffffu) break;
            j_ci.push_back((uint32_t)reindex_by_subdomain(n, m, best));
            j_ri.push_back((uint32_t)r);
            j_a.push_back(ia < ea && c.A.col[ia] == best ? c.A.coeff[ia++] : 0);
            j_b.push_back(ib < eb && c.B.col[ib] == best ? c.B.coeff[ib++] : 0);
            j_c.push_back(ic < ec && c.C.col[ic] == best ? c.C.coeff[ic++] : 0);
        }
    }
    size_t nnz = j_ci.size();
    k = next_pow2(nnz);
    lg_n = log2_exact(n); lg_k = log2_exact(k); lg_m = log2_exact(m);
    vk.num_variables = c.num_variables(); vk.num_constraints = c.num_constraints; vk.num_non_zero = nnz; vk.num_instance = c.num_instance;
    vk.num_public_inputs = c.raw_instance - 1;
    if (vk.num_variables != vk.num_constraints) throw std::logic_error("index: matrices are not square after padding");
    max_degree = ahp_max_degree(lits.num_constraints, lits.num_variables, lits.num_non_zero);
    supported_degree = ahp_max_degree(vk.num_constraints, vk.num_variables, vk.num_non_zero);
    if (supported_degree > max_degree) throw std::runtime_error("IndexTooLarge: the circuit needs degree " + std::to_string(supported_degree) + " but the universal SRS supports " + std::to_string(max_degree));
    bounds[0] = std::min(n - 2, k - 2); bounds[1] = std::max(n - 2, k - 2);
    lowest_shift = max_degree - bounds[1];
    {
        const bool want_tables = lg_k >= 20 && !(flags & KEY_NO_TABLES);
        const size_t big = std::max(4 * n, 2 * k), ebuf = std::max(4 * n, k);
        const size_t per_context = (18 * n + 6 * k + 5 * ebuf) * sizeof(F) + 13 * big * 16 + ((size_t)256 << 20);
        auto t_srs = Clock::now();
        srs = acquire_srs(max_degree, want_tables, default_contexts() * per_context, stream);
        setup_srs_s = ms_since(t_srs) / 1e3;
        use_tables = want_tables && srs->tables();
        table_c = srs->table_c;
        srs_stride = srs->stride;
        d_powers = srs->d_points;
        d_shifted = d_powers + lowest_shift;
    }
    static const bool lanes_default = [] { const char *e = getenv("ZKAES_LANES"); return !e || atoi(e) != 0; }();
    use_lanes = lanes_default;
    if (use_lagrange) lag = acquire_lagrange(*srs, n, lg_n, m, lg_m, stream);
    const G1A &g = srs->g;
    vk.g = srs->g; vk.gamma_g = srs->gamma_g;
    vk.h = srs->h; vk.beta_h = srs->beta_h;
    vk.degree_bounds[0] = bounds[0]; vk.degree_bounds[1] = bounds[1];
    for (int i = 0; i < 2; i++) vk.shift_powers[i] = mul_affine(g, srs->beta.pow_u64(max_degree - bounds[i]));
    vk.supported_degree = supported_degree; vk.max_degree = max_degree;
    {
        uint8_t sb[256];
        for (int i = 0; i < 256; i++) sb[i] = aes_sbox_value((uint8_t)i);
        gpu::upload_sbox(sb);
    }
    d_desc = upload(c.desc, stream);
    d_sbox_in = upload(c.sbox_in_off.empty() ? std::vector<uint32_t>{0} : c.sbox_in_off, stream);
    d_sbox_tmpl = upload(c.sbox_tmpl.empty() ? std::vector<uint32_t>{0} : c.sbox_tmpl, stream);
    d_a_rowptr = upload(c.A.rowptr, stream); d_a_col = upload(c.A.col.empty() ? std::vector<uint32_t>{0} : c.A.col, stream);
    d_a_coeff = upload(c.A.coeff.empty() ? std::vector<int64_t>{0} : c.A.coeff, stream);
    d_b_rowptr = upload(c.B.rowptr, stream); d_b_col = upload(c.B.col.empty() ? std::vector<uint32_t>{0} : c.B.col, stream);
    d_b_coeff = upload(c.B.coeff.empty() ? std::vector<int64_t>{0} : c.B.coeff, stream);
    {
        std::vector<uint32_t> colptr(n + 1, 0), trow;
        std::vector<uint8_t> tmat;
        std::vector<int64_t> tcoef;
        const CsrMatrix *M[3] = {&c.A, &c.B, &c.C};
        for (int q = 0; q < 3; q++) for (uint32_t col : M[q]->col) colptr[reindex_by_subdomain(n, m, col) + 1]++;
        for (size_t i = 0; i < n; i++) colptr[i + 1] += colptr[i];
        size_t total = colptr[n];
        trow.resize(total ? total : 1); tmat.resize(total ? total : 1); tcoef.resize(total ? total : 1);
// ... 221 lines not shown
        const size_t ls[3] = {cx.poly_len[5], cx.poly_len[4], cx.poly_len[2]};
        const Fr at[3] = {R.beta, R.beta, R.beta};
        Fr ev[3];
        gpu::poly_eval_multi(ps, ls, at, 3, ev, cx.scratch.p, cx.scratch.n, s);
        R.pf.evals[0] = ev[0]; R.pf.evals[2] = ev[1]; R.pf.evals[3] = ev[2];
        gpu::divide_by_linear(cx.wit2.p, cx.poly[5].p, cx.poly_len[5], R.beta, cx.scratch.p, cx.scratch.n, s);
    }
    R.jobs.join();
    { Bytes o; for (auto &lp : R.r3) o.commitment_tobytes(lp.comm); R.fs.absorb(o.b); }
    R.gamma = R.fs.rng().rand_field<Fr>();
    cx.timings.round3_ms = ms_since(R.t0); R.t0 = Clock::now();
}

void ProvingKeyImpl::prove_open(ProofRun &R) {
    ProverContext &cx = R.cx;
    gpu::stream_t s = cx.stream;
    if (R.early_evals) {
        const F *ps[1] = {cx.poly[7].p};
        const size_t ls[1] = {cx.poly_len[7]};
        gpu::poly_eval_multi(ps, ls, &R.gamma, 1, &R.pf.evals[1], cx.scratch.p, cx.scratch.n, s);
    } else {
        const F *ps[4] = {cx.poly[5].p, cx.poly[7].p, cx.poly[4].p, cx.poly[2].p};
        const size_t ls[4] = {cx.poly_len[5], cx.poly_len[7], cx.poly_len[4], cx.poly_len[2]};
        const Fr at[4] = {R.beta, R.gamma, R.beta, R.beta};
        gpu::poly_eval_multi(ps, ls, at, 4, R.pf.evals, cx.scratch.p, cx.scratch.n, s);
    }
    const Fr g2_g = R.pf.evals[1], t_b = R.pf.evals[2], zb_b = R.pf.evals[3];
    { Bytes o; for (auto &v : R.pf.evals) o.field(v); R.fs.absorb(o.b); }
    Fr ch;
    { uint64_t lo = R.fs.rng().next_u64(), hi = R.fs.rng().next_u64(); uint32_t raw[8] = {(uint32_t)lo, (uint32_t)(lo >> 32), (uint32_t)hi, (uint32_t)(hi >> 32), 0, 0, 0, 0}; ch = Fr::from_raw(raw); }
    Fr r_alpha_at_beta = (R.vh_alpha - R.vh_beta) * (R.alpha - R.beta).inverse();
    Fr vx_beta = eval_vanishing(m, R.beta);
    Fr c_za = r_alpha_at_beta * (R.eta_a + R.eta_c * zb_b), c_w = (t_b * vx_beta).neg(), c_h1 = R.vh_beta.neg();
    Fr vk_gamma = eval_vanishing(k, R.gamma);
    Fr bmul = R.gamma * g2_g + t_b * Fr::from_u64(k).inverse();
    Fr c_row = R.alpha * bmul, c_col = R.beta * bmul, c_rc = bmul.neg(), c_h2 = vk_gamma.neg();
    Fr chp[5]; chp[0] = Fr::one(); for (int i = 1; i < 5; i++) chp[i] = chp[i - 1] * ch;
    auto rand_axpy = [](Fr out[3], const Fr &sc, const KzgRand &r) { if (r.hiding) for (int i = 0; i < 3; i++) out[i] = out[i] + sc * r.b[i]; };
    auto host_divide_by_linear = [](Fr q[2], const Fr p[3], const Fr &z) { q[1] = p[2]; q[0] = p[1] + z * p[2]; };
    auto host_eval3 = [](const Fr p[3], const Fr &z) { return p[0] + z * (p[1] + z * p[2]); };
    if (R.jobs.async && !cx.ev_aux) {
        cx.acc_b.alloc(cx.acc.n); cx.wit_b.alloc(cx.wit.n); cx.wit2_b.alloc(cx.wit2.n); cx.scratch_b.alloc(cx.scratch.n);
        cx.scratch_c.alloc(gpu::divide_by_linear_scratch(std::max(n, k) + 1)); cx.ev_aux = gpu::EventGuard();
    }
    const bool two_sets = cx.ev_aux != nullptr && R.jobs.async;
    if (R.jobs.async) gpu::sync(s);
    struct WaitJobs { RoundJobs &j; ~WaitJobs() { j.wait_all(); } } wait_jobs{R.jobs};
    R.jobs.start(1, [&](Lane &ln) {
        gpu::stream_t ls_ = ln.stream;
        size_t plen = 3 * n;
        Fr rb[3] = {Fr::zero(), Fr::zero(), Fr::zero()};
        {
            const F *ps[7] = {cx.poly[5].p, cx.poly[3].p, cx.poly[1].p, cx.poly[0].p, cx.poly[6].p, cx.poly[4].p, cx.poly[2].p};
            size_t ls[7] = {cx.poly_len[5], cx.poly_len[3], cx.poly_len[1], cx.poly_len[0], cx.poly_len[6], cx.poly_len[4], cx.poly_len[2]};
            Fr sc[7] = {chp[0], chp[2], chp[2] * c_za, chp[2] * c_w, chp[2] * c_h1, chp[3], chp[4]};
            gpu::poly_lincomb_n(cx.acc.p, plen, ps, ls, sc, 7, ls_);
        }
        rand_axpy(rb, chp[0], R.r2[1].rand); rand_axpy(rb, chp[2] * c_za, R.r1[1].rand); rand_axpy(rb, chp[2] * c_w, R.r1[0].rand); rand_axpy(rb, chp[4], R.r1[2].rand);
        if (!R.early_evals) gpu::divide_by_linear(cx.wit2.p, cx.poly[5].p, cx.poly_len[5], R.beta, cx.scratch.p, cx.scratch.n, ls_);
        gpu::divide_by_linear(cx.wit.p, cx.acc.p, plen, R.beta, cx.scratch.p, cx.scratch.n, ls_);
        gpu::poly_scale(cx.wit2.p, chp[1], cx.poly_len[5] - 1, ls_);
        msm_opening_prepare(cx, ln, cx.wit.p, plen - 1, cx.wit2.p, cx.poly_len[5] - 1, bounds[1] - (n - 2));
        XYZZ<Fq377> hw = XYZZ<Fq377>::inf();
        Fr rq[2]; host_divide_by_linear(rq, rb, R.beta);
        for (int i = 0; i < 2; i++) hw.add(srs->gamma_tab[i].mul(rq[i]));
        Fr rv = host_eval3(rb, R.beta);
        Fr srb[3]; for (int i = 0; i < 3; i++) srb[i] = chp[1] * R.r2[1].shifted_rand.b[i];
        host_divide_by_linear(rq, srb, R.beta);
        for (int i = 0; i < 2; i++) hw.add(srs->gamma_tab[i].mul(rq[i]));
        rv = rv + host_eval3(srb, R.beta);
        XYZZ<Fq377> w = msm_opening_finish(ln);
        w.add(hw);
        R.pf.w_beta = w.to_affine(); R.pf.random_v_beta = rv;
    }, false);
    R.jobs.start(2, [&](Lane &ln) {
        gpu::stream_t ls_ = ln.stream;
        DevPtr<F> &acc_ = two_sets ? cx.acc_b : cx.acc, &wit_ = two_sets ? cx.wit_b : cx.wit, &wit2_ = two_sets ? cx.wit2_b : cx.wit2, &scr_ = two_sets ? cx.scratch_b : cx.scratch;
        size_t plen = k;
        {
            const F *ps[8] = {cx.poly[7].p, ix_co[2].p, ix_co[3].p, ix_co[4].p, ix_co[0].p, ix_co[1].p, ix_co[5].p, cx.poly[8].p};
            size_t ls[8] = {cx.poly_len[7], k, k, k, k, k, k, cx.poly_len[8]};
            Fr sc[8] = {chp[0], chp[2] * R.ea_vv, chp[2] * R.eb_vv, chp[2] * R.ec_vv, chp[2] * c_row, chp[2] * c_col, chp[2] * c_rc, chp[2] * c_h2};
            gpu::poly_lincomb_n(acc_.p, plen, ps, ls, sc, 8, ls_);
        }
        gpu::divide_by_linear(wit_.p, acc_.p, plen, R.gamma, scr_.p, scr_.n, ls_);
        if (R.jobs.async) {
            while (!R.g2_quotient_queued.load(std::memory_order_acquire)) std::this_thread::yield();
            gpu::stream_wait_event(ls_, cx.ev_aux);
        } else {
            gpu::divide_by_linear(wit2_.p, cx.poly[7].p, cx.poly_len[7], R.gamma, scr_.p, scr_.n, ls_);
            gpu::poly_scale(wit2_.p, chp[1], cx.poly_len[7] - 1, ls_);
        }
        msm_opening_prepare(cx, ln, wit_.p, plen - 1, wit2_.p, cx.poly_len[7] - 1, bounds[1] - (k - 2));
        XYZZ<Fq377> w = msm_opening_finish(ln);
        R.pf.w_gamma = w.to_affine();
    }, false);
    if (R.jobs.async) {
        try {
            gpu::divide_by_linear(cx.wit2_b.p, cx.poly[7].p, cx.poly_len[7], R.gamma, cx.scratch_c.p, cx.scratch_c.n, s);
            gpu::poly_scale(cx.wit2_b.p, chp[1], cx.poly_len[7] - 1, s);
            gpu::event_record(cx.ev_aux, s);
        } catch (...) { R.g2_quotient_queued.store(true, std::memory_order_release); throw; }
        R.g2_quotient_queued.store(true, std::memory_order_release);
    }
    R.jobs.join();
}

Proof ProvingKeyImpl::prove(ProverContext &cx, const uint8_t *host_trace, const uint8_t *msg, size_t len, const uint8_t *key, const uint8_t *zk_seed, bool throughput, const uint8_t *iv) {
    gpu::set_device(device);
    std::lock_guard<std::mutex> busy(cx.in_use);
    cx.throughput = throughput;
    ProofRun R(*this, cx, host_trace, msg, len, key, iv, zk_seed);
    prove_round1(R);
    prove_round2(R);
    prove_round3(R);
    prove_open(R);
    for (int i = 0; i < 4; i++) R.pf.comms[i] = R.r1[i].comm;
    for (int i = 0; i < 3; i++) R.pf.comms[4 + i] = R.r2[i].comm;
    for (int i = 0; i < 2; i++) R.pf.comms[7 + i] = R.r3[i].comm;
    cx.timings.open_ms = ms_since(R.t0);
    cx.timings.total_ms = ms_since(R.t_all);
    { std::lock_guard<std::mutex> g(ctx_mu); last_timings = cx.timings; }
    return R.pf;
}

ProvingKey::~ProvingKey() { if (impl) { DeviceScope on(impl->device); delete impl; } }
const VerifyingKey &ProvingKey::vk() const { return impl->vk; }
const Circuit &ProvingKey::circuit() const { return impl->circuit; }
const ProverTimings &ProvingKey::last_timings() const { return impl->last_timings; }
bool ProvingKey::tables_built(uint64_t *bytes) const {
    if (bytes) *bytes = impl->use_tables ? impl->srs->bytes() : 0;
    return impl->use_tables;
}
void ProvingKey::srs_info(uint64_t out[6], double secs[2]) const {
    const UniversalSrs &U = *impl->srs;
    out[0] = U.max_degree; out[1] = U.stride; out[2] = U.n_tab; out[3] = U.bytes();
    out[4] = (uint64_t)impl->srs.use_count();
    out[5] = impl->lag ? 2 * (uint64_t)impl->lag->n * sizeof(SrsPoint) : 0;
    if (secs) { secs[0] = impl->setup_srs_s; secs[1] = impl->setup_total_s; }
}
size_t ProvingKey::contexts() const { size_t v = impl->n_contexts.load(); return v ? v : default_contexts(); }
void ProvingKey::set_contexts(size_t n) {
    if (n > 64) throw std::invalid_argument("set_contexts: at most 64 prover contexts per key");
    impl->n_contexts.store(n);
}
void ProvingKey::msm_powers_partial_device(const uint8_t *scalars, size_t n_local, size_t offset, void *dev_out) {
    gpu::set_device(impl->device);
    if (!impl->use_tables) throw std::runtime_error("msm_powers_partial_device: this key has no window tables (KEY_NO_TABLES, or the device was short of memory)");
    if (offset + n_local > impl->supported_degree + 1) throw std::runtime_error("msm_powers_partial_device: range exceeds the committer key");
    ProverContext &cx = impl->context(0);
    std::lock_guard<std::mutex> busy(cx.in_use);
    if (n_local > cx.acc.n) throw std::runtime_error("msm_powers_partial_device: more scalars than a prover context holds");
    if (n_local) gpu::h2d(cx.acc.p, scalars, n_local * sizeof(F), cx.stream);
    gpu::msm_table_sum_device<Bls377>(cx.msm_ws, impl->d_powers, impl->srs_stride, offset, impl->table_c, cx.acc.p, n_local, (XYZZ<Fq377> *)dev_out, cx.stream);
}
Proof ProvingKey::prove_aes(const uint8_t *message, size_t len, const uint8_t key[16], const uint8_t *zk_seed) {
    if (impl->circuit.kind != CIRCUIT_AES) throw std::invalid_argument("proving key was not synthesized for the AES circuit");
    if (len % 16) throw std::invalid_argument("Input must be 16 bytes length when adding round key");
    if (len != impl->circuit.n_blocks * 16) throw std::invalid_argument("InstanceDoesNotMatchIndex: proving key was synthesized for " + std::to_string(impl->circuit.n_blocks * 16) + " bytes");
    return impl->prove(impl->context(0), nullptr, message, len, key, zk_seed);
}
std::string ProvingKey::op_lists_json(const uint8_t *message, size_t len, const uint8_t key[16], bool throughput_path) {
    if (impl->circuit.kind != CIRCUIT_AES) throw std::invalid_argument("proving key was not synthesized for the AES circuit");
    if (len != impl->circuit.n_blocks * 16) throw std::invalid_argument("InstanceDoesNotMatchIndex: proving key was synthesized for " + std::to_string(impl->circuit.n_blocks * 16) + " bytes");
    gpu::OpRecord rec;
    gpu::oplog_begin();
    try { impl->prove(impl->context(0), nullptr, message, len, key, nullptr, throughput_path); }
    catch (...) { gpu::oplog_end(); throw; }
    rec = gpu::oplog_end();
    const Circuit &c = impl->circuit;
    std::string o = "{\"h\":" + std::to_string(impl->n) + ",\"k\":" + std::to_string(impl->k) + ",\"x\":" + std::to_string(impl->m) + ",\"variables\":" + std::to_string(c.num_variables()) +
                    ",\"constraints\":" + std::to_string(c.num_constraints) + ",\"nnz\":[" + std::to_string(c.A.nnz()) + "," + std::to_string(c.B.nnz()) + "," + std::to_string(c.C.nnz()) + "]" +
                    ",\"blocks\":" + std::to_string(c.n_blocks) + ",\"path\":\"" + (throughput_path ? "throughput" : "lone") + "\",\"ntt\":[";
    for (size_t i = 0; i < rec.ntt.size(); i++) o += (i ? "," : "") + std::string("[") + std::to_string(rec.ntt[i].first) + "," + std::to_string(rec.ntt[i].second) + "]";
    o += "],\"msm\":[";
    static const char *kinds[3] = {"buckets", "second_bases", "class_sum"};
    for (size_t i = 0; i < rec.msm.size(); i++) o += (i ? "," : "") + std::string("[") + std::to_string(rec.msm[i].first) + ",\"" + kinds[rec.msm[i].second % 3] + "\"]";
    o += "]}";
    return o;
}
static std::vector<uint8_t> witness_of(ProvingKeyImpl *impl, const uint8_t *message, size_t len, const uint8_t *key, const uint8_t *iv) {
    const Circuit &c = impl->circuit;
    ProverContext &cx = impl->context(0);
    std::lock_guard<std::mutex> busy(cx.in_use);
    gpu::stream_t s = cx.stream;
    impl->launch_trace(cx, message, len, key, iv);
    gpu::witness_expand(cx.d_z, impl->d_desc, (uint32_t)c.num_variables(), cx.d_trace, impl->d_sbox_in, impl->d_sbox_tmpl, s);
    std::vector<uint8_t> z(c.num_variables());
    gpu::d2h(z.data(), cx.d_z, z.size(), s);
    return z;
}
std::vector<uint8_t> ProvingKey::aes_witness(const uint8_t *message, size_t len, const uint8_t key[16]) {
    if (impl->circuit.kind != CIRCUIT_AES) throw std::invalid_argument("proving key was not synthesized for the AES circuit");
    if (len % 16) throw std::invalid_argument("Input must be 16 bytes length when adding round key");
    if (len != impl->circuit.n_blocks * 16) throw std::invalid_argument("InstanceDoesNotMatchIndex: proving key was synthesized for " + std::to_string(impl->circuit.n_blocks * 16) + " bytes");
    return witness_of(impl, message, len, key, nullptr);
}
static void require_cbc_key(const Circuit &c, size_t len) {
    if (c.kind != CIRCUIT_AES_CBC) throw std::invalid_argument("proving key was not synthesized for the AES-CBC circuit");
    if (len == 0 || len % 16) throw std::invalid_argument("CBC: the message must be a non-zero multiple of 16 bytes");
}
std::vector<uint8_t> ProvingKey::aes_witness_cbc(const uint8_t *message, size_t len, const uint8_t key[16], const uint8_t iv[16]) {
    require_cbc_key(impl->circuit, len);
    if (!message || !key || !iv) throw std::invalid_argument("null argument");
    if (len != impl->circuit.n_blocks * 16) throw std::invalid_argument("InstanceDoesNotMatchIndex: proving key was synthesized for " + std::to_string(impl->circuit.n_blocks * 16) + " bytes");
    return witness_of(impl, message, len, key, iv);
}
Proof ProvingKey::prove_aes_cbc(const uint8_t *message, size_t len, const uint8_t key[16], const uint8_t iv[16], const uint8_t *zk_seed, uint8_t *ciphertext_or_null) {
    require_cbc_key(impl->circuit, len);
    if (!message || !key || !iv) throw std::invalid_argument("null argument");
    if (len != impl->circuit.n_blocks * 16) throw std::invalid_argument("InstanceDoesNotMatchIndex: proving key was synthesized for " + std::to_string(impl->circuit.n_blocks * 16) + " bytes");
    if (ciphertext_or_null) aes128_cbc_encrypt_host(message, len, key, iv, ciphertext_or_null);
    return impl->prove(impl->context(0), nullptr, message, len, key, zk_seed, false, iv);
}
static void require_ctr_key(const Circuit &c, const uint8_t *message, const uint8_t *key, const uint8_t *icb) {
    if (c.kind != CIRCUIT_AES_CTR) throw std::invalid_argument("proving key was not synthesized for the AES-CTR circuit");
    if (!message || !key || !icb) throw std::invalid_argument("null argument");
}
std::vector<uint8_t> ProvingKey::aes_witness_ctr(const uint8_t *message, size_t len, const uint8_t key[16], const uint8_t icb[16]) {
    const Circuit &c = impl->circuit;
    require_ctr_key(c, message, key, icb);
    if (len != c.message_bytes) throw std::invalid_argument("InstanceDoesNotMatchIndex: proving key was synthesized for " + std::to_string(c.message_bytes) + " bytes");
    return witness_of(impl, message, len, key, icb);
}
Proof ProvingKey::prove_aes_ctr(const uint8_t *message, size_t len, const uint8_t key[16], const uint8_t icb[16], const uint8_t *zk_seed, uint8_t *ciphertext_or_null) {
    const Circuit &c = impl->circuit;
    require_ctr_key(c, message, key, icb);
    if (len != c.message_bytes) throw std::invalid_argument("InstanceDoesNotMatchIndex: proving key was synthesized for " + std::to_string(c.message_bytes) + " bytes");
    if (ciphertext_or_null) aes128_ctr_crypt_host(message, len, key, icb, ciphertext_or_null);
    return impl->prove(impl->context(0), nullptr, message, len, key, zk_seed, false, icb);
}
void os_random_seed(uint8_t out[32]) {
    size_t got = 0;
    while (got < 32) {
        ssize_t r = getrandom(out + got, 32 - got, 0);
        if (r < 0) { if (errno == EINTR) continue; throw std::runtime_error("getrandom failed: no entropy for the prover's zero-knowledge seed"); }
        got += (size_t)r;
    }
}
static void derive_zk_seed(uint8_t out[32], const uint8_t *seed32, uint64_t index) {
    uint8_t buf[40];
    memcpy(buf, seed32, 32);
    for (int i = 0; i < 8; i++) buf[32 + i] = (uint8_t)(index >> (8 * i));
    Blake2s::digest(out, buf, sizeof buf);
}
static std::vector<Proof> prove_many(ProvingKeyImpl *impl, const uint8_t *messages, const uint8_t *keys, size_t key_stride, size_t n_chunks, size_t n_contexts, const uint8_t *zk_seed, uint64_t index_offset,
                                     const uint8_t *ivs, size_t iv_stride = 16) {
    size_t chunk = impl->circuit.message_bytes;
    if (n_contexts == 0) n_contexts = 1;
    n_contexts = std::min(n_contexts, std::max<size_t>(n_chunks, 1));
    std::vector<Proof> proofs(n_chunks);
    for (size_t i = 0; i < n_contexts; i++) impl->context(i);
    std::atomic<size_t> next{0};
    std::vector<std::string> errors(n_contexts);
    const int device = impl->device;
    auto worker = [&](size_t ci) {
        try {
            gpu::set_device(device);
            ProverContext &cx = impl->context(ci);
            for (;;) {
                size_t i = next.fetch_add(1);
                if (i >= n_chunks) break;
                uint8_t seed_i[32];
                if (zk_seed) derive_zk_seed(seed_i, zk_seed, index_offset + (uint64_t)i);
                proofs[i] = impl->prove(cx, nullptr, messages + i * chunk, chunk, keys + i * key_stride, zk_seed ? seed_i : nullptr, n_chunks > 1, ivs ? ivs + iv_stride * i : nullptr);
            }
        } catch (const std::exception &e) { errors[ci] = e.what(); }
    };
    gpu::ThroughputWaits waits(n_contexts > 1);
    std::vector<std::thread> threads;
    for (size_t ci = 1; ci < n_contexts; ci++) threads.emplace_back(worker, ci);
    worker(0);
    for (auto &t : threads) t.join();
    for (auto &e : errors) if (!e.empty()) throw std::runtime_error(e);
    return proofs;
}
std::vector<Proof> ProvingKey::prove_aes_chunked(const uint8_t *message, size_t len, const uint8_t key[16], size_t n_contexts, const uint8_t *zk_seed, uint64_t index_offset) {
    if (impl->circuit.kind != CIRCUIT_AES) throw std::invalid_argument("proving key was not synthesized for the AES circuit");
    size_t chunk = impl->circuit.n_blocks * 16;
    if (chunk == 0 || len % chunk) throw std::invalid_argument("message length must be a multiple of the key's plaintext length (" + std::to_string(chunk) + " bytes)");
    return prove_many(impl, message, key, 0, len / chunk, n_contexts, zk_seed, index_offset, nullptr);
}
std::vector<Proof> ProvingKey::prove_aes_batch(const uint8_t *messages, const uint8_t *keys, size_t n, size_t n_contexts, const uint8_t *zk_seed, uint64_t index_offset) {
    if (impl->circuit.kind != CIRCUIT_AES) throw std::invalid_argument("proving key was not synthesized for the AES circuit");
    if (impl->circuit.n_blocks == 0) throw std::invalid_argument("proving key has an empty plaintext");
    return prove_many(impl, messages, keys, 16, n, n_contexts, zk_seed, index_offset, nullptr);
}
std::vector<Proof> ProvingKey::prove_aes_cbc_chunked(const uint8_t *message, size_t len, const uint8_t key[16], const uint8_t iv[16], size_t n_contexts, const uint8_t *zk_seed, uint64_t index_offset,
                                                     uint8_t *ciphertext_or_null) {
    require_cbc_key(impl->circuit, len);
    if (!message || !key || !iv) throw std::invalid_argument("null argument");
    size_t chunk = impl->circuit.n_blocks * 16;
    if (len % chunk) throw std::invalid_argument("message length must be a multiple of the key's plaintext length (" + std::to_string(chunk) + " bytes)");
    std::vector<uint8_t> ct(len);
    aes128_cbc_encrypt_host(message, len, key, iv, ct.data());
    size_t n_chunks = len / chunk;
    std::vector<uint8_t> ivs(16 * n_chunks);
    for (size_t j = 0; j < n_chunks; j++) memcpy(&ivs[16 * j], j ? &ct[chunk * j - 16] : iv, 16);
    std::vector<Proof> proofs = prove_many(impl, message, key, 0, n_chunks, n_contexts, zk_seed, index_offset, ivs.data());
    if (ciphertext_or_null) memcpy(ciphertext_or_null, ct.data(), len);
    return proofs;
}
std::vector<Proof> ProvingKey::prove_aes_ctr_chunked(const uint8_t *message, size_t len, const uint8_t key[16], const uint8_t icb[16], size_t n_contexts, const uint8_t *zk_seed, uint64_t index_offset,
                                                     uint8_t *ciphertext_or_null) {
    const Circuit &c = impl->circuit;
    require_ctr_key(c, message, key, icb);
    size_t chunk = c.message_bytes;
// ... 159 lines not shown
```

Before: 97.76.

## Fold Montgomery R^-1 into SRS bases so MSM digits skip scalar conversion

Result: no change. 98.04 (median of 6 runs) (+0.3%).

```diff
diff --git a/aes_zero_knowledge_proof_circuit_amd/csrc/capi_kernels.hip b/aes_zero_knowledge_proof_circuit_amd/csrc/capi_kernels.hip
--- a/aes_zero_knowledge_proof_circuit_amd/csrc/capi_kernels.hip
+++ b/aes_zero_knowledge_proof_circuit_amd/csrc/capi_kernels.hip
@@ -483,9 +483,11 @@
         DevPtr<zk::Affine<Fq>> tab(nt * n);
         zk::Affine<Fq> g; for (int i = 0; i < 12; i++) { g.x.l[i] = G1_377_X_MONT[i]; g.y.l[i] = G1_377_Y_MONT[i]; }
         Fr beta = Fr::from_u64(0x9e3779b97f4a7c15ull) * Fr::from_u64(0xc2b2ae3d27d4eb4full);
-        zk::gpu::fixed_base_powers<zk::Bls377>(tab, g, beta, 1, n, s);
+        const bool edwards = window_bits != 0;
+        const zk::gpu::Digits digits = edwards ? zk::gpu::Digits::stored : zk::gpu::Digits::canonical;
+        const Fr r_inv = zk::gpu::montgomery_r_inverse<Fr>();
+        zk::gpu::fixed_base_powers<zk::Bls377>(tab, g, beta, 1, n, s, edwards ? &r_inv : nullptr);
         if (window_bits > 0) zk::gpu::build_window_tables<zk::Bls377>(tab, n, window_bits, s);
-        const bool edwards = window_bits != 0;
         DevPtr<zk::Affine28<zk::Fq377P>> tab28;
         DevPtr<zk::Niels28<zk::Fq377P>> tabte;
         if (edwards) { tabte.alloc(nt * n); zk::gpu::convert_bases_te<zk::Bls377>(tabte, tab, nt * n, s); }
@@ -498,7 +500,7 @@
         zk::gpu::sync(s);
         WorkspaceGuard ws;
         auto run = [&]() -> zk::XYZZ<Fq> {
-            if (edwards) return window_bits > 0 ? zk::gpu::msm_table<zk::Bls377>(ws, tabte, n, 0, window_bits, ds, n, s) : zk::gpu::msm<zk::Bls377>(ws, tabte.get(), ds.get(), n, s);
+            if (edwards) return window_bits > 0 ? zk::gpu::msm_table<zk::Bls377>(ws, tabte, n, 0, window_bits, ds, n, s, digits) : zk::gpu::msm<zk::Bls377>(ws, tabte.get(), ds.get(), n, s, digits);
             return window_bits > 0 ? zk::gpu::msm_table<zk::Bls377>(ws, tab28, n, 0, window_bits, ds, n, s) : zk::gpu::msm<zk::Bls377>(ws, tab28.get(), ds.get(), n, s);
         };
         give_affine(run().to_affine(), out_xy, nullptr);
diff --git a/aes_zero_knowledge_proof_circuit_amd/csrc/gpu.hpp b/aes_zero_knowledge_proof_circuit_amd/csrc/gpu.hpp
--- a/aes_zero_knowledge_proof_circuit_amd/csrc/gpu.hpp
+++ b/aes_zero_knowledge_proof_circuit_amd/csrc/gpu.hpp
@@ -104,6 +104,8 @@
 template <class Fr> const Fr *domain_elements(int lg);
 
 struct MsmWorkspace;
+enum class Digits { canonical, stored };
+template <class Fr> inline Fr montgomery_r_inverse() { Fr x = Fr::zero(); x.l[0] = 1; return x; }
 MsmWorkspace *msm_workspace_create();
 void msm_workspace_destroy(MsmWorkspace *ws);
 using WorkspaceGuard = Handle<MsmWorkspace *, msm_workspace_create, msm_workspace_destroy>;
@@ -111,18 +113,20 @@
 template <class Curve>
 XYZZ<typename Curve::Fq> msm(MsmWorkspace *ws, const Affine28<typename Curve::FqP> *bases, const typename Curve::Fr *scalars, size_t n, stream_t s);
 template <class Curve>
-void msm_prepare(MsmWorkspace *ws, const typename Curve::Fr *scal1, size_t n1, const typename Curve::Fr *scal2, size_t n2, size_t val_off2, stream_t s, int force_c = 0);
+void msm_prepare(MsmWorkspace *ws, const typename Curve::Fr *scal1, size_t n1, const typename Curve::Fr *scal2, size_t n2, size_t val_off2, stream_t s, int force_c = 0,
+                 Digits digits = Digits::canonical);
 template <class Curve>
 XYZZ<typename Curve::Fq> msm_finish(MsmWorkspace *ws, const Affine28<typename Curve::FqP> *bases, stream_t s);
 template <class Curve> void convert_bases_te(Niels28<typename Curve::FqP> *dst, const Affine<typename Curve::Fq> *src, size_t n, stream_t s);
 template <class Curve>
-XYZZ<typename Curve::Fq> msm(MsmWorkspace *ws, const Niels28<typename Curve::FqP> *bases, const typename Curve::Fr *scalars, size_t n, stream_t s);
+XYZZ<typename Curve::Fq> msm(MsmWorkspace *ws, const Niels28<typename Curve::FqP> *bases, const typename Curve::Fr *scalars, size_t n, stream_t s, Digits digits = Digits::canonical);
 template <class Curve>
 XYZZ<typename Curve::Fq> msm_finish(MsmWorkspace *ws, const Niels28<typename Curve::FqP> *bases, stream_t s);
 template <class Curve>
 void msm_finish2(MsmWorkspace *ws, const Niels28<typename Curve::FqP> *bases, const Niels28<typename Curve::FqP> *bases2, XYZZ<typename Curve::Fq> *out, stream_t s);
 template <class Curve>
-XYZZ<typename Curve::Fq> msm_table(MsmWorkspace *ws, const Niels28<typename Curve::FqP> *tables, size_t stride, size_t off, int c, const typename Curve::Fr *scalars, size_t n, stream_t s);
+XYZZ<typename Curve::Fq> msm_table(MsmWorkspace *ws, const Niels28<typename Curve::FqP> *tables, size_t stride, size_t off, int c, const typename Curve::Fr *scalars, size_t n, stream_t s,
+                                   Digits digits = Digits::canonical);
 template <class Curve>
 bool class_sum(MsmWorkspace *ws, const Niels28<typename Curve::FqP> *bases, const int8_t *vals, size_t n, XYZZ<typename Curve::Fq> *out, stream_t s);
 template <class Curve> void msm_sharded_plan(size_t n_total, int *window_bits, int *n_windows);
@@ -133,18 +137,20 @@
 XYZZ<typename Curve::Fq> msm_fold_window_sums_device(const XYZZ<typename Curve::Fq> *dev_in, int world, size_t n_total, stream_t s);
 template <class Curve>
 void msm_table_sum_device(MsmWorkspace *ws, const Niels28<typename Curve::FqP> *tables, size_t stride, size_t off, int c, const typename Curve::Fr *scalars, size_t n,
-                          XYZZ<typename Curve::Fq> *dev_out, stream_t s);
+                          XYZZ<typename Curve::Fq> *dev_out, stream_t s, Digits digits = Digits::canonical);
 template <class Curve>
 XYZZ<typename Curve::Fq> msm_fold_points_device(const XYZZ<typename Curve::Fq> *dev_in, int world, stream_t s);
 template <class Curve> int table_windows(int c);
 template <class Curve> void build_window_tables(Affine<typename Curve::Fq> *tables, size_t stride, int c, stream_t s);
 template <class Curve> void table_next(Affine<typename Curve::Fq> *next, const Affine<typename Curve::Fq> *prev, size_t count, int c, int j, stream_t s);
 template <class Curve>
-void msm_prepare_table(MsmWorkspace *ws, const typename Curve::Fr *scal1, size_t n1, size_t off1, const typename Curve::Fr *scal2, size_t n2, size_t off2, int c, size_t stride, stream_t s);
+void msm_prepare_table(MsmWorkspace *ws, const typename Curve::Fr *scal1, size_t n1, size_t off1, const typename Curve::Fr *scal2, size_t n2, size_t off2, int c, size_t stride, stream_t s,
+                       Digits digits = Digits::canonical);
 template <class Curve>
 XYZZ<typename Curve::Fq> msm_table(MsmWorkspace *ws, const Affine28<typename Curve::FqP> *tables, size_t stride, size_t off, int c, const typename Curve::Fr *scalars, size_t n, stream_t s);
 template <class Curve>
-void fixed_base_powers(Affine<typename Curve::Fq> *out, const Affine<typename Curve::Fq> &base, const typename Curve::Fr &beta, size_t from, size_t count, stream_t s);
+void fixed_base_powers(Affine<typename Curve::Fq> *out, const Affine<typename Curve::Fq> &base, const typename Curve::Fr &beta, size_t from, size_t count, stream_t s,
+                       const typename Curve::Fr *scale = nullptr);
 template <class Curve>
 void fixed_base_scalars(Affine<typename Curve::Fq> *out, const Affine<typename Curve::Fq> &base, const typename Curve::Fr *scalars, size_t count, stream_t s);
 template <class Curve>
diff --git a/aes_zero_knowledge_proof_circuit_amd/csrc/kernels_msm.hip b/aes_zero_knowledge_proof_circuit_amd/csrc/kernels_msm.hip
--- a/aes_zero_knowledge_proof_circuit_amd/csrc/kernels_msm.hip
+++ b/aes_zero_knowledge_proof_circuit_amd/csrc/kernels_msm.hip
@@ -25,14 +25,21 @@
 }
 
 constexpr uint32_t VAL_SKIP = 1u << 30, VAL_INDEX = VAL_SKIP - 1;
-template <class Fr>
+template <bool STORED, class Fr>
+__device__ __forceinline__ void digit_source(const Fr &x, uint32_t (&raw)[Fr::N + 1]) {
+    if constexpr (STORED) {
+#pragma unroll
+        for (int i = 0; i < Fr::N; i++) raw[i] = x.l[i];
+    } else x.to_raw(raw);
+    raw[Fr::N] = 0;
+}
+template <class Fr, bool STORED>
 __global__ void k_digits(const Fr *__restrict__ scalars, uint32_t n, uint32_t i_off, uint32_t ntot, uint32_t val_off, int c, int nwin, uint32_t nb,
                          uint32_t *__restrict__ keys, uint32_t *__restrict__ vals) {
     uint32_t i = blockIdx.x * blockDim.x + threadIdx.x;
     if (i >= n) return;
     uint32_t raw[Fr::N + 1];
-    scalars[i].to_raw(raw);
-    raw[Fr::N] = 0;
+    digit_source<STORED>(scalars[i], raw);
     const uint32_t mask = (1u << c) - 1, half = 1u << (c - 1);
     uint32_t carry = 0;
     for (int w = 0; w < nwin; w++) {
@@ -60,14 +67,13 @@
     L.n_hi = rem ? rem : L.nwin;
     return L;
 }
-template <class Fr>
+template <class Fr, bool STORED>
 __global__ void k_digits_table(const Fr *__restrict__ scalars, uint32_t n, uint32_t i_off, uint32_t ntot, uint32_t val_off, TableLayout L, uint32_t stride,
                                uint32_t *__restrict__ keys, uint32_t *__restrict__ vals) {
     uint32_t i = blockIdx.x * blockDim.x + threadIdx.x;
     if (i >= n) return;
     uint32_t raw[Fr::N + 1];
-    scalars[i].to_raw(raw);
-    raw[Fr::N] = 0;
+    digit_source<STORED>(scalars[i], raw);
     uint32_t carry = 0;
     for (int w = 0; w < L.nwin; w++) {
         const int c = L.width(w), bit = L.offset(w), limb = bit >> 5, sh = bit & 31;
@@ -868,7 +874,7 @@
 }
 
 template <class Curve>
-void msm_prepare(MsmWorkspace *ws_, const typename Curve::Fr *scal1, size_t n1, const typename Curve::Fr *scal2, size_t n2, size_t val_off2, stream_t s_, int force_c) {
+void msm_prepare(MsmWorkspace *ws_, const typename Curve::Fr *scal1, size_t n1, const typename Curve::Fr *scal2, size_t n2, size_t val_off2, stream_t s_, int force_c, Digits digits) {
     using Fr = typename Curve::Fr;
     hipStream_t s = (hipStream_t)s_;
     if (!ws_) throw GpuError("msm: null workspace");
@@ -889,8 +895,9 @@
     const size_t nb = (size_t)nwin << (c - 1);
     S.plan_c = c; S.plan_nwin = nwin; S.plan_pairs = pairs; S.plan_table = false; S.plan_cap = BUCKET_CAP;
     ensure_scratch(S, pairs, nb, BUCKET_CAP);
-    if (n1) { hipLaunchKernelGGL((k_digits<Fr>), dim3((unsigned)((n1 + 255) / 256)), dim3(256), 0, s, scal1, (uint32_t)n1, 0u, (uint32_t)n, 0u, c, nwin, (uint32_t)nb, S.keys_a, S.vals_a); HIP_LAUNCH_CHECK(); }
-    if (n2) { hipLaunchKernelGGL((k_digits<Fr>), dim3((unsigned)((n2 + 255) / 256)), dim3(256), 0, s, scal2, (uint32_t)n2, (uint32_t)n1, (uint32_t)n, (uint32_t)val_off2, c, nwin, (uint32_t)nb, S.keys_a, S.vals_a); HIP_LAUNCH_CHECK(); }
+    const auto digits_kernel = digits == Digits::stored ? k_digits<Fr, true> : k_digits<Fr, false>;
+    if (n1) { hipLaunchKernelGGL(digits_kernel, dim3((unsigned)((n1 + 255) / 256)), dim3(256), 0, s, scal1, (uint32_t)n1, 0u, (uint32_t)n, 0u, c, nwin, (uint32_t)nb, S.keys_a, S.vals_a); HIP_LAUNCH_CHECK(); }
+    if (n2) { hipLaunchKernelGGL(digits_kernel, dim3((unsigned)((n2 + 255) / 256)), dim3(256), 0, s, scal2, (uint32_t)n2, (uint32_t)n1, (uint32_t)n, (uint32_t)val_off2, c, nwin, (uint32_t)nb, S.keys_a, S.vals_a); HIP_LAUNCH_CHECK(); }
     prepare_buckets<typename Curve::FqP>(S, pairs, c - 1, nwin, c - 1, BUCKET_CAP, s);
 }
 template <class Curve, class Law>
@@ -955,9 +962,9 @@
 template <class Curve>
 XYZZ<typename Curve::Fq> msm_finish(MsmWorkspace *ws_, const Niels28<typename Curve::FqP> *bases, stream_t s_) { return msm_finish_impl<Curve, EdwardsLaw<typename Curve::FqP>>(ws_, bases, s_); }
 template <class Curve>
-XYZZ<typename Curve::Fq> msm(MsmWorkspace *ws_, const Niels28<typename Curve::FqP> *bases, const typename Curve::Fr *scalars, size_t n, stream_t s_) {
+XYZZ<typename Curve::Fq> msm(MsmWorkspace *ws_, const Niels28<typename Curve::FqP> *bases, const typename Curve::Fr *scalars, size_t n, stream_t s_, Digits digits) {
     if (n == 0) return XYZZ<typename Curve::Fq>::inf();
-    msm_prepare<Curve>(ws_, scalars, n, nullptr, 0, 0, s_);
+    msm_prepare<Curve>(ws_, scalars, n, nullptr, 0, 0, s_, 0, digits);
     return msm_finish<Curve>(ws_, bases, s_);
 }
 
@@ -983,7 +990,7 @@
         sync((stream_t)s);
         return;
     }
-    msm_prepare<Curve>(ws_, scalars, n_local, nullptr, 0, 0, s_, c);
+    msm_prepare<Curve>(ws_, scalars, n_local, nullptr, 0, 0, s_, c, Digits::canonical);
     MsmWorkspace &S = *ws_;
     if (S.plan_nwin != nwin) throw GpuError("msm_window_sums_device: window plan mismatch");
     float ms = 0;
@@ -1024,7 +1031,7 @@
 
 template <class Curve>
 void msm_table_sum_device(MsmWorkspace *ws_, const Niels28<typename Curve::FqP> *tables, size_t stride, size_t off, int c, const typename Curve::Fr *scalars, size_t n,
-                          XYZZ<typename Curve::Fq> *dev_out, stream_t s_) {
+                          XYZZ<typename Curve::Fq> *dev_out, stream_t s_, Digits digits) {
     using Fq = typename Curve::Fq;
     hipStream_t s = (hipStream_t)s_;
     if (n == 0) {
@@ -1032,7 +1039,7 @@
         sync((stream_t)s);
         return;
     }
-    msm_prepare_table<Curve>(ws_, scalars, n, off, nullptr, 0, 0, c, stride, s_);
+    msm_prepare_table<Curve>(ws_, scalars, n, off, nullptr, 0, 0, c, stride, s_, digits);
     MsmWorkspace &S = *ws_;
     float ms = 0;
     auto t_begin = std::chrono::steady_clock::now();
@@ -1121,8 +1128,23 @@
     __syncthreads();
 }
 template <class Fr>
+__device__ __forceinline__ void part_load(const Fr *__restrict__ s1, uint32_t n1, const Fr *__restrict__ s2, uint32_t g, uint32_t (&raw)[Fr::N + 1]) {
+    static_assert(Fr::N == 8, "a scalar is read as two 16-byte words");
+    const uint4 *src = reinterpret_cast<const uint4 *>(g < n1 ? s1 + g : s2 + (g - n1));
+    const uint4 a = src[0], b = src[1];
+    raw[0] = a.x; raw[1] = a.y; raw[2] = a.z; raw[3] = a.w; raw[4] = b.x; raw[5] = b.y; raw[6] = b.z; raw[7] = b.w; raw[Fr::N] = 0;
+}
+template <class Fr>
+__global__ void k_canonical_scalars(const Fr *__restrict__ s1, uint32_t n1, const Fr *__restrict__ s2, uint32_t n2, Fr *__restrict__ out) {
+    const uint32_t g = blockIdx.x * blockDim.x + threadIdx.x;
+    if (g >= n1 + n2) return;
+    Fr r;
+    (g < n1 ? s1[g] : s2[g - n1]).to_raw(r.l);
+    out[g] = r;
+}
+template <class Fr>
 __global__ void __launch_bounds__(PART_THREADS) k_part_hist(const Fr *__restrict__ s1, uint32_t n1, const Fr *__restrict__ s2, uint32_t n2, TableLayout L, uint32_t nbin,
-                                                            uint32_t *__restrict__ canon, uint32_t *__restrict__ hist) {
+                                                            uint32_t *__restrict__ hist) {
     __shared__ uint32_t sh[PART_NBIN_MAX];
     for (uint32_t b = threadIdx.x; b < nbin; b += PART_THREADS) sh[b] = 0;
     __syncthreads();
@@ -1133,21 +1155,17 @@
             const uint32_t g = tile * PART_TILE + q * PART_THREADS + threadIdx.x;
             if (g >= n) continue;
             uint32_t d[PART_MAXW], raw[Fr::N + 1];
-            (g < n1 ? s1[g] : s2[g - n1]).to_raw(raw);
-            raw[Fr::N] = 0;
+            part_load<Fr>(s1, n1, s2, g, raw);
             part_digits<Fr::N>(raw, L, d);
 #pragma unroll
             for (int w = 0; w < PART_MAXW; w++) if (d[w] != PART_NONE) atomicAdd(&sh[(d[w] & 0x7fffffffu) >> PART_FINE_BITS], 1u);
-            static_assert(Fr::N == 8, "the canonical scalar is stored as two 16-byte words");
-            uint4 *dst = reinterpret_cast<uint4 *>(canon + (size_t)g * Fr::N);
-            dst[0] = make_uint4(raw[0], raw[1], raw[2], raw[3]); dst[1] = make_uint4(raw[4], raw[5], raw[6], raw[7]);
         }
     __syncthreads();
     for (uint32_t b = threadIdx.x; b < nbin; b += PART_THREADS) hist[(size_t)b * gridDim.x + blockIdx.x] = sh[b];
     if (blockIdx.x == 0 && threadIdx.x == 0) hist[(size_t)nbin * gridDim.x] = 0;
 }
-template <int NW>
-__global__ void __launch_bounds__(PART_THREADS) k_part_scatter(const uint32_t *__restrict__ canon, uint32_t n, uint32_t n1, TableLayout L, uint32_t off1, uint32_t off2, uint32_t stride,
+template <class Fr>
+__global__ void __launch_bounds__(PART_THREADS) k_part_scatter(const Fr *__restrict__ s1, const Fr *__restrict__ s2, uint32_t n, uint32_t n1, TableLayout L, uint32_t off1, uint32_t off2, uint32_t stride,
                                                                uint32_t nbin, const uint32_t *__restrict__ offs, uint32_t *__restrict__ out_val, uint16_t *__restrict__ out_key) {
     __shared__ uint32_t cursor[PART_NBIN_MAX], cnt[PART_NBIN_MAX], fill[PART_NBIN_MAX], st_val[PART_STAGE], st_key[PART_STAGE];
     __shared__ uint32_t wave_sums[PART_THREADS / 64], total;
@@ -1162,11 +1180,9 @@
         for (int q = 0; q < PART_SPT; q++) {
             const uint32_t g = tile * PART_TILE + q * PART_THREADS + threadIdx.x;
             if (g < n) {
-                uint32_t raw[NW + 1];
-                const uint4 *src = reinterpret_cast<const uint4 *>(canon + (size_t)g * NW);
-                const uint4 a = src[0], b = src[1];
-                raw[0] = a.x; raw[1] = a.y; raw[2] = a.z; raw[3] = a.w; raw[4] = b.x; raw[5] = b.y; raw[6] = b.z; raw[7] = b.w; raw[NW] = 0;
-                part_digits<NW>(raw, L, d[q]);
+                uint32_t raw[Fr::N + 1];
+                part_load<Fr>(s1, n1, s2, g, raw);
+                part_digits<Fr::N>(raw, L, d[q]);
             } else {
 #pragma unroll
                 for (int w = 0; w < PART_MAXW; w++) d[q][w] = PART_NONE;
@@ -1260,23 +1276,31 @@
     }
 }
 template <class Fr>
-static void partition_buckets(MsmWorkspace &S, const Fr *scal1, size_t n1, size_t off1, const Fr *scal2, size_t n2, size_t off2, const TableLayout &L, size_t stride, uint32_t cap, hipStream_t s) {
+static void partition_buckets(MsmWorkspace &S, const Fr *scal1, size_t n1, size_t off1, const Fr *scal2, size_t n2, size_t off2, const TableLayout &L, size_t stride, uint32_t cap, bool stored_digits,
+                              hipStream_t s) {
     const int B = L.c_hi - 1;
     const uint32_t nbin = 1u << (B - PART_FINE_BITS), G = PART_GRID;
     const size_t n = n1 + n2, nb = (size_t)1 << B, nh = (size_t)nbin * G + 1;
-    S.canon.grow(n * Fr::N);
+    if (!stored_digits) {
+        S.canon.grow(n * Fr::N);
+        Fr *canon = reinterpret_cast<Fr *>(S.canon.p);
+        hipLaunchKernelGGL((k_canonical_scalars<Fr>), dim3((unsigned)((n + 255) / 256)), dim3(256), 0, s, scal1, (uint32_t)n1, scal2, (uint32_t)n2, canon);
+        HIP_LAUNCH_CHECK();
+        scal1 = canon; scal2 = canon + n1;
+    }
+    if (((uintptr_t)scal1 | (uintptr_t)scal2) & 15) throw GpuError("msm_table: scalar arrays must be 16-byte aligned");
     grow_together({nh, nh}, S.part_hist, S.part_offs);
 #ifdef ZKAES_MEASURE
     for (int rep = (knockin() & 1) ? 0 : 1; rep < 2; rep++)
 #endif
     {
-    hipLaunchKernelGGL((k_part_hist<Fr>), dim3(G), dim3(PART_THREADS), 0, s, scal1, (uint32_t)n1, scal2, (uint32_t)n2, L, nbin, S.canon, S.part_hist);
+    hipLaunchKernelGGL((k_part_hist<Fr>), dim3(G), dim3(PART_THREADS), 0, s, scal1, (uint32_t)n1, scal2, (uint32_t)n2, L, nbin, S.part_hist);
     HIP_LAUNCH_CHECK();
     size_t tb = 0;
     HIP_CHECK(rocprim::exclusive_scan(nullptr, tb, S.part_hist.p, S.part_offs.p, 0u, nh, rocprim::plus<uint32_t>(), s));
     S.tmp.grow(tb);
     HIP_CHECK(rocprim::exclusive_scan(S.tmp.p, tb, S.part_hist.p, S.part_offs.p, 0u, nh, rocprim::plus<uint32_t>(), s));
-    hipLaunchKernelGGL((k_part_scatter<Fr::N>), dim3(G), dim3(PART_THREADS), 0, s, (const uint32_t *)S.canon, (uint32_t)n, (uint32_t)n1, L, (uint32_t)off1, (uint32_t)off2, (uint32_t)stride, nbin,
+    hipLaunchKernelGGL((k_part_scatter<Fr>), dim3(G), dim3(PART_THREADS), 0, s, scal1, scal2, (uint32_t)n, (uint32_t)n1, L, (uint32_t)off1, (uint32_t)off2, (uint32_t)stride, nbin,
                        (const uint32_t *)S.part_offs, S.vals_a, (uint16_t *)S.keys_a.p);
     HIP_LAUNCH_CHECK();
     hipLaunchKernelGGL(k_part_fine, dim3(nbin), dim3(PART_FINE_THREADS), 0, s, (const uint32_t *)S.part_offs, G, (const uint32_t *)S.vals_a, (const uint16_t *)S.keys_a.p, S.vals_b, S.start, S.end);
@@ -1288,7 +1312,7 @@
 
 template <class Curve>
 void msm_prepare_table(MsmWorkspace *ws_, const typename Curve::Fr *scal1, size_t n1, size_t off1, const typename Curve::Fr *scal2, size_t n2, size_t off2, int c, size_t stride,
-                       stream_t s_) {
+                       stream_t s_, Digits digits) {
     using Fr = typename Curve::Fr;
     hipStream_t s = (hipStream_t)s_;
     if (!ws_) throw GpuError("msm: null workspace");
@@ -1309,11 +1333,12 @@
     ensure_scratch(S, pairs, nb, cap);
     const int B = L.c_hi - 1;
     if (B > PART_FINE_BITS && (1u << (B - PART_FINE_BITS)) <= PART_NBIN_MAX && nwin <= PART_MAXW && pairs >= ((size_t)1 << 16)) {
-        partition_buckets<Fr>(S, scal1, n1, off1, scal2, n2, off2, L, stride, cap, s);
+        partition_buckets<Fr>(S, scal1, n1, off1, scal2, n2, off2, L, stride, cap, digits == Digits::stored, s);
         return;
     }
-    if (n1) { hipLaunchKernelGGL((k_digits_table<Fr>), dim3((unsigned)((n1 + 255) / 256)), dim3(256), 0, s, scal1, (uint32_t)n1, 0u, (uint32_t)n, (uint32_t)off1, L, (uint32_t)stride, S.keys_a, S.vals_a); HIP_LAUNCH_CHECK(); }
-    if (n2) { hipLaunchKernelGGL((k_digits_table<Fr>), dim3((unsigned)((n2 + 255) / 256)), dim3(256), 0, s, scal2, (uint32_t)n2, (uint32_t)n1, (uint32_t)n, (uint32_t)off2, L, (uint32_t)stride, S.keys_a, S.vals_a); HIP_LAUNCH_CHECK(); }
+    const auto digits_kernel = digits == Digits::stored ? k_digits_table<Fr, true> : k_digits_table<Fr, false>;
+    if (n1) { hipLaunchKernelGGL(digits_kernel, dim3((unsigned)((n1 + 255) / 256)), dim3(256), 0, s, scal1, (uint32_t)n1, 0u, (uint32_t)n, (uint32_t)off1, L, (uint32_t)stride, S.keys_a, S.vals_a); HIP_LAUNCH_CHECK(); }
+    if (n2) { hipLaunchKernelGGL(digits_kernel, dim3((unsigned)((n2 + 255) / 256)), dim3(256), 0, s, scal2, (uint32_t)n2, (uint32_t)n1, (uint32_t)n, (uint32_t)off2, L, (uint32_t)stride, S.keys_a, S.vals_a); HIP_LAUNCH_CHECK(); }
     prepare_buckets<typename Curve::FqP>(S, pairs, L.c_hi - 1, 1, L.c_hi - 1, cap, s);
 }
 template <class Curve>
@@ -1323,17 +1348,18 @@
     return msm_finish<Curve>(ws_, tables, s_);
 }
 template <class Curve>
-XYZZ<typename Curve::Fq> msm_table(MsmWorkspace *ws_, const Niels28<typename Curve::FqP> *tables, size_t stride, size_t off, int c, const typename Curve::Fr *scalars, size_t n, stream_t s_) {
+XYZZ<typename Curve::Fq> msm_table(MsmWorkspace *ws_, const Niels28<typename Curve::FqP> *tables, size_t stride, size_t off, int c, const typename Curve::Fr *scalars, size_t n, stream_t s_,
+                                   Digits digits) {
     if (n == 0) return XYZZ<typename Curve::Fq>::inf();
-    msm_prepare_table<Curve>(ws_, scalars, n, off, nullptr, 0, 0, c, stride, s_);
+    msm_prepare_table<Curve>(ws_, scalars, n, off, nullptr, 0, 0, c, stride, s_, digits);
     return msm_finish<Curve>(ws_, tables, s_);
 }
 
 template <class Fr>
-__global__ void k_power_scalars(Fr beta, uint64_t from, uint32_t count, Fr *__restrict__ out) {
+__global__ void k_power_scalars(Fr beta, uint64_t from, uint32_t count, Fr scale, Fr *__restrict__ out) {
     uint32_t i = blockIdx.x * blockDim.x + threadIdx.x;
     if (i >= count) return;
-    out[i] = beta.pow_u64(from + i);
+    out[i] = beta.pow_u64(from + i) * scale;
 }
 template <class Fq, class Fr>
 __global__ void __launch_bounds__(64) k_fixed_base(const Affine<Fq> *__restrict__ table, const Fr *__restrict__ scalars, uint32_t count, Affine<Fq> *__restrict__ out) {
@@ -1369,7 +1395,8 @@
 }
 
 template <class Curve>
-void fixed_base_powers(Affine<typename Curve::Fq> *out, const Affine<typename Curve::Fq> &base, const typename Curve::Fr &beta, size_t from, size_t count, stream_t s_) {
+void fixed_base_powers(Affine<typename Curve::Fq> *out, const Affine<typename Curve::Fq> &base, const typename Curve::Fr &beta, size_t from, size_t count, stream_t s_,
+                       const typename Curve::Fr *scale) {
     using Fq = typename Curve::Fq;
     using Fr = typename Curve::Fr;
     hipStream_t s = (hipStream_t)s_;
@@ -1379,7 +1406,7 @@
     DevPtr<Fr> d_sc(CH);
     for (size_t off = 0; off < count; off += CH) {
         uint32_t m = (uint32_t)((count - off) < CH ? (count - off) : CH);
-        hipLaunchKernelGGL((k_power_scalars<Fr>), dim3((m + 255) / 256), dim3(256), 0, s, beta, (uint64_t)(from + off), m, d_sc.get());
+        hipLaunchKernelGGL((k_power_scalars<Fr>), dim3((m + 255) / 256), dim3(256), 0, s, beta, (uint64_t)(from + off), m, scale ? *scale : Fr::one(), d_sc.get());
         HIP_LAUNCH_CHECK();
         hipLaunchKernelGGL((k_fixed_base<Fq, Fr>), dim3((m + 63) / 64), dim3(64), 0, s, (const Affine<Fq> *)d_table.get(), (const Fr *)d_sc.get(), m, out + off);
         HIP_LAUNCH_CHECK();
@@ -1533,11 +1560,11 @@
 }
 template XYZZ<Fq377> msm_finish<Bls377>(MsmWorkspace *, const Niels28<Fq377P> *, stream_t);
 template void msm_finish2<Bls377>(MsmWorkspace *, const Niels28<Fq377P> *, const Niels28<Fq377P> *, XYZZ<Fq377> *, stream_t);
-template XYZZ<Fq377> msm<Bls377>(MsmWorkspace *, const Niels28<Fq377P> *, const Fr377 *, size_t, stream_t);
-template XYZZ<Fq377> msm_table<Bls377>(MsmWorkspace *, const Niels28<Fq377P> *, size_t, size_t, int, const Fr377 *, size_t, stream_t);
+template XYZZ<Fq377> msm<Bls377>(MsmWorkspace *, const Niels28<Fq377P> *, const Fr377 *, size_t, stream_t, Digits);
+template XYZZ<Fq377> msm_table<Bls377>(MsmWorkspace *, const Niels28<Fq377P> *, size_t, size_t, int, const Fr377 *, size_t, stream_t, Digits);
 template bool class_sum<Bls377>(MsmWorkspace *, const Niels28<Fq377P> *, const int8_t *, size_t, XYZZ<Fq377> *, stream_t);
 
-template void msm_table_sum_device<Bls377>(MsmWorkspace *, const Niels28<Fq377P> *, size_t, size_t, int, const Fr377 *, size_t, XYZZ<Fq377> *, stream_t);
+template void msm_table_sum_device<Bls377>(MsmWorkspace *, const Niels28<Fq377P> *, size_t, size_t, int, const Fr377 *, size_t, XYZZ<Fq377> *, stream_t, Digits);
 template XYZZ<Fq377> msm_fold_points_device<Bls377>(const XYZZ<Fq377> *, int, stream_t);
 template XYZZ<Fq381> msm_fold_points_device<Bls381>(const XYZZ<Fq381> *, int, stream_t);
 template void msm_sharded_plan<Bls377>(size_t, int *, int *);
@@ -1546,8 +1573,8 @@
 template void msm_window_sums_device<Bls381>(MsmWorkspace *, const Affine28<Fq381P> *, const Fr381 *, size_t, size_t, XYZZ<Fq381> *, stream_t);
 template XYZZ<Fq377> msm_fold_window_sums_device<Bls377>(const XYZZ<Fq377> *, int, size_t, stream_t);
 template XYZZ<Fq381> msm_fold_window_sums_device<Bls381>(const XYZZ<Fq381> *, int, size_t, stream_t);
-template void msm_prepare_table<Bls377>(MsmWorkspace *, const Fr377 *, size_t, size_t, const Fr377 *, size_t, size_t, int, size_t, stream_t);
-template void msm_prepare_table<Bls381>(MsmWorkspace *, const Fr381 *, size_t, size_t, const Fr381 *, size_t, size_t, int, size_t, stream_t);
+template void msm_prepare_table<Bls377>(MsmWorkspace *, const Fr377 *, size_t, size_t, const Fr377 *, size_t, size_t, int, size_t, stream_t, Digits);
+template void msm_prepare_table<Bls381>(MsmWorkspace *, const Fr381 *, size_t, size_t, const Fr381 *, size_t, size_t, int, size_t, stream_t, Digits);
 template XYZZ<Fq377> msm_table<Bls377>(MsmWorkspace *, const Affine28<Fq377P> *, size_t, size_t, int, const Fr377 *, size_t, stream_t);
 template XYZZ<Fq381> msm_table<Bls381>(MsmWorkspace *, const Affine28<Fq381P> *, size_t, size_t, int, const Fr381 *, size_t, stream_t);
 template void convert_bases<Bls377>(Affine28<Fq377P> *, const Affine<Fq377> *, size_t, stream_t);
@@ -1558,16 +1585,16 @@
 template void build_window_tables<Bls381>(Affine<Fq381> *, size_t, int, stream_t);
 template int table_windows<Bls377>(int);
 template int table_windows<Bls381>(int);
-template void msm_prepare<Bls377>(MsmWorkspace *, const Fr377 *, size_t, const Fr377 *, size_t, size_t, stream_t, int);
-template void msm_prepare<Bls381>(MsmWorkspace *, const Fr381 *, size_t, const Fr381 *, size_t, size_t, stream_t, int);
+template void msm_prepare<Bls377>(MsmWorkspace *, const Fr377 *, size_t, const Fr377 *, size_t, size_t, stream_t, int, Digits);
+template void msm_prepare<Bls381>(MsmWorkspace *, const Fr381 *, size_t, const Fr381 *, size_t, size_t, stream_t, int, Digits);
 template XYZZ<Fq377> msm_finish<Bls377>(MsmWorkspace *, const Affine28<Fq377P> *, stream_t);
 template XYZZ<Fq381> msm_finish<Bls381>(MsmWorkspace *, const Affine28<Fq381P> *, stream_t);
 template XYZZ<Fq377> msm<Bls377>(MsmWorkspace *, const Affine28<Fq377P> *, const Fr377 *, size_t, stream_t);
 template XYZZ<Fq381> msm<Bls381>(MsmWorkspace *, const Affine28<Fq381P> *, const Fr381 *, size_t, stream_t);
 template void fixed_base_scalars<Bls377>(Affine<Fq377> *, const Affine<Fq377> &, const Fr377 *, size_t, stream_t);
 template bool class_sum<Bls377>(MsmWorkspace *, const Affine28<Fq377P> *, const int8_t *, size_t, XYZZ<Fq377> *, stream_t);
-template void fixed_base_powers<Bls377>(Affine<Fq377> *, const Affine<Fq377> &, const Fr377 &, size_t, size_t, stream_t);
-template void fixed_base_powers<Bls381>(Affine<Fq381> *, const Affine<Fq381> &, const Fr381 &, size_t, size_t, stream_t);
-
-}
-}
+template void fixed_base_powers<Bls377>(Affine<Fq377> *, const Affine<Fq377> &, const Fr377 &, size_t, size_t, stream_t, const Fr377 *);
+template void fixed_base_powers<Bls381>(Affine<Fq381> *, const Affine<Fq381> &, const Fr381 &, size_t, size_t, stream_t, const Fr381 *);
+
+}
+}
diff --git a/aes_zero_knowledge_proof_circuit_amd/csrc/marlin.cpp b/aes_zero_knowledge_proof_circuit_amd/csrc/marlin.cpp
--- a/aes_zero_knowledge_proof_circuit_amd/csrc/marlin.cpp
+++ b/aes_zero_knowledge_proof_circuit_amd/csrc/marlin.cpp
@@ -108,7 +108,8 @@
         DevPtr<G1A> stage[2];
         stage[0].alloc(S->stride);
         if (n_tab > 1) stage[1].alloc(S->stride);
-        gpu::fixed_base_powers<Bls377>(stage[0], S->g, S->beta, 0, S->stride, stream);
+        const Fr r_inv = gpu::montgomery_r_inverse<Fr>();
+        gpu::fixed_base_powers<Bls377>(stage[0], S->g, S->beta, 0, S->stride, stream, &r_inv);
         S->d_points.alloc(n_tab * S->stride);
         srs_convert(S->d_points, stage[0], S->stride, stream);
         for (size_t j = 1; j < n_tab; j++) {
@@ -238,6 +239,7 @@
     std::shared_ptr<UniversalSrs> srs;
     std::shared_ptr<LagrangeSrs> lag;
     SrsPoint *d_powers = nullptr, *d_shifted = nullptr;
+    static constexpr gpu::Digits SRS_DIGITS = gpu::Digits::stored;
     size_t srs_stride = 0;
 #ifndef ZKAES_TABLE_MIN_N
 #define ZKAES_TABLE_MIN_N 100000
@@ -302,8 +304,8 @@
         if (len == 0) return XYZZ<Fq377>::inf();
         size_t avail = shifted ? (bounds[1] + 1) : (supported_degree + 1);
         if (off + len > avail) throw std::runtime_error("KZG10: polynomial degree exceeds the committer key");
-        if (table_ok(cx, len)) return gpu::msm_table<Bls377>(ln.ws, d_powers, srs_stride, (shifted ? lowest_shift : 0) + off, table_c, scalars, len, ln.stream);
-        return gpu::msm<Bls377>(ln.ws, (shifted ? d_shifted : d_powers) + off, scalars, len, ln.stream);
+        if (table_ok(cx, len)) return gpu::msm_table<Bls377>(ln.ws, d_powers, srs_stride, (shifted ? lowest_shift : 0) + off, table_c, scalars, len, ln.stream, SRS_DIGITS);
+        return gpu::msm<Bls377>(ln.ws, (shifted ? d_shifted : d_powers) + off, scalars, len, ln.stream, SRS_DIGITS);
     }
     struct Labeled { int idx; long bound; bool hiding; KzgRand rand, shifted_rand; Commitment comm; };
     static void draw_rand(Labeled &lp, ChaChaRng &zk) {
@@ -329,8 +331,8 @@
         const size_t off = bounded ? (max_degree - (size_t)lp.bound) - lowest_shift : 0;
         if (len > supported_degree + 1 || (bounded && off + len > bounds[1] + 1)) throw std::runtime_error("KZG10: polynomial degree exceeds the committer key");
         if (len) {
-            if (table_ok(cx, len)) gpu::msm_prepare_table<Bls377>(ln.ws, coeffs, len, 0, nullptr, 0, 0, table_c, srs_stride, ln.stream);
-            else gpu::msm_prepare<Bls377>(ln.ws, coeffs, len, nullptr, 0, 0, ln.stream);
+            if (table_ok(cx, len)) gpu::msm_prepare_table<Bls377>(ln.ws, coeffs, len, 0, nullptr, 0, 0, table_c, srs_stride, ln.stream, SRS_DIGITS);
+            else gpu::msm_prepare<Bls377>(ln.ws, coeffs, len, nullptr, 0, 0, ln.stream, 0, SRS_DIGITS);
         }
         XYZZ<Fq377> c12[2] = {XYZZ<Fq377>::inf(), XYZZ<Fq377>::inf()}, h12[2] = {XYZZ<Fq377>::inf(), XYZZ<Fq377>::inf()};
         hide(h12[0], lp.rand);
@@ -345,8 +347,8 @@
     }
     void msm_opening_prepare(ProverContext &cx, Lane &ln, const F *wit, size_t wlen, const F *swit, size_t slen, size_t shift_off) {
         if (wlen > supported_degree + 1 || shift_off + slen > bounds[1] + 1) throw std::runtime_error("KZG10: polynomial degree exceeds the committer key");
-        if (table_ok(cx, wlen + slen)) gpu::msm_prepare_table<Bls377>(ln.ws, wit, wlen, 0, swit, slen, lowest_shift + shift_off, table_c, srs_stride, ln.stream);
-        else gpu::msm_prepare<Bls377>(ln.ws, wit, wlen, swit, slen, lowest_shift + shift_off, ln.stream);
+        if (table_ok(cx, wlen + slen)) gpu::msm_prepare_table<Bls377>(ln.ws, wit, wlen, 0, swit, slen, lowest_shift + shift_off, table_c, srs_stride, ln.stream, SRS_DIGITS);
+        else gpu::msm_prepare<Bls377>(ln.ws, wit, wlen, swit, slen, lowest_shift + shift_off, ln.stream, 0, SRS_DIGITS);
     }
     XYZZ<Fq377> msm_opening_finish(Lane &ln) { return gpu::msm_finish<Bls377>(ln.ws, d_powers, ln.stream); }
     bool use_lanes = true;
@@ -874,7 +876,7 @@
     std::lock_guard<std::mutex> busy(cx.in_use);
     if (n_local > cx.acc.n) throw std::runtime_error("msm_powers_partial_device: more scalars than a prover context holds");
     if (n_local) gpu::h2d(cx.acc.p, scalars, n_local * sizeof(F), cx.stream);
-    gpu::msm_table_sum_device<Bls377>(cx.msm_ws, impl->d_powers, impl->srs_stride, offset, impl->table_c, cx.acc.p, n_local, (XYZZ<Fq377> *)dev_out, cx.stream);
+    gpu::msm_table_sum_device<Bls377>(cx.msm_ws, impl->d_powers, impl->srs_stride, offset, impl->table_c, cx.acc.p, n_local, (XYZZ<Fq377> *)dev_out, cx.stream, ProvingKeyImpl::SRS_DIGITS);
 }
 Proof ProvingKey::prove_aes(const uint8_t *message, size_t len, const uint8_t key[16], const uint8_t *zk_seed) {
     if (impl->circuit.kind != CIRCUIT_AES) throw std::invalid_argument("proving key was not synthesized for the AES circuit");
```
